# TalShor/SciLMM

Hardware: NVIDIA B200
Metric: reml_iter_time (lower is better)
Workload: dtype f64

## Files before the change

### include/scilmm_b200.h

```cpp
#ifndef SCILMM_B200_H
#define SCILMM_B200_H

#include <stdint.h>

#ifdef __cplusplus
extern "C" {
#endif

#define SLMM_OK 0
#define SLMM_ERR_INVALID 1
#define SLMM_ERR_CUDA 2
#define SLMM_ERR_NOT_POSDEF 3
#define SLMM_ERR_INTERNAL 4

#define SLMM_ORDER_NATURAL 0
#define SLMM_ORDER_GIVEN 1
#define SLMM_ORDER_METIS 2
#define SLMM_ORDER_MINDEG 3
#define SLMM_ORDER_METIS_FAST 4

typedef struct slmm_chol slmm_chol_t;
typedef struct slmm_matset slmm_matset_t;

const char* slmm_last_error(void);
int slmm_version(void);
int slmm_device_count(int* out);

int slmm_matset_create(int32_t n, int32_t K, slmm_matset_t** out);
int slmm_matset_destroy(slmm_matset_t* ms);
int slmm_matset_upload(slmm_matset_t* ms, int32_t k, const int32_t* h_indptr, const int32_t* h_indices,
                       const double* h_data);
int slmm_matset_bind_device(slmm_matset_t* ms, int32_t k, const int32_t* d_indptr, const int32_t* d_indices,
                            const double* d_data, int64_t nnz, int32_t same_as);
int slmm_matset_set_row_range(slmm_matset_t* ms, int32_t row_begin, int32_t row_end);
int slmm_matset_symmetry_hash(slmm_matset_t* ms, int32_t k, uint64_t* h_out2);
int slmm_matset_set_symmetric(slmm_matset_t* ms, int32_t k, int32_t flag);
int slmm_upload_h2d(void* d_dst, const void* h_src, int64_t nbytes, int32_t threads);
int slmm_upload_h2d_2d(void* d_dst, int64_t dst_pitch, const void* h_src, int64_t src_pitch, int64_t width_bytes,
                       int64_t rows);
int slmm_matset_nnz(const slmm_matset_t* ms, int32_t k, int64_t* out);
int slmm_matset_values(const slmm_matset_t* ms, int32_t k, const double** d_data_out);

int slmm_he_moments(slmm_matset_t* ms, const double* d_y, int32_t row_begin, int32_t row_end, double* d_out);
int slmm_he_moments_host(slmm_matset_t* ms, const double* h_y, double* h_out);

int slmm_spmm(slmm_matset_t* ms, int32_t k, const double* d_X, int32_t ncols, double* d_out);
int slmm_spmm_coldot(slmm_matset_t* ms, int32_t k, const double* d_X, int32_t ncols, int32_t row_begin,
                     int32_t row_end, double* d_out);

int slmm_spmm_coldot_multi(slmm_matset_t* ms, int32_t nk, const int32_t* ks, const double* d_X, int32_t ncols,
                           int32_t store_from, double* d_store, int32_t row_begin, int32_t row_end, double* d_dots);
int slmm_quadform_multi(slmm_matset_t* ms, int32_t nk, const int32_t* ks, const double* d_X, int32_t ncols,
                        int32_t row_begin, int32_t row_end, double* d_dots);
int slmm_quadform_gram_multi(slmm_matset_t* ms, int32_t nk, const int32_t* ks, const double* d_X, int32_t ncols,
                             const double* d_XB, int32_t nb, int32_t row_begin, int32_t row_end, double* d_dots,
                             double* d_gram_half);
int slmm_matset_validate(slmm_matset_t* ms, int32_t k, int32_t* flags_out);
int slmm_device_arrays_equal_i32(const int32_t* d_a, const int32_t* d_b, int64_t count, int32_t* out);
int slmm_matset_is_symmetric(slmm_matset_t* ms, int32_t k, int32_t* out);
int slmm_matset_pattern_id(const slmm_matset_t* ms, int32_t k, int32_t* out);

int slmm_matset_build_tiles(slmm_matset_t* ms, int32_t k, const int32_t* d_perm, const int32_t* d_iperm);
int slmm_matset_tile_stats(const slmm_matset_t* ms, int32_t k, int64_t* out4);
int slmm_matset_tile_cta_profile(const slmm_matset_t* ms, int32_t k, int64_t* out, int32_t ncta);
int slmm_quadform_tiled(slmm_matset_t* ms, int32_t nk, const int32_t* ks, const double* d_X, int32_t ncols, int32_t nb,
                        double* d_dots, double* d_gram_half);
int slmm_device_csr_is_symmetric(const int32_t* d_indptr, const int32_t* d_indices, const double* d_data, int32_t n,
                                 int32_t* out);
int slmm_device_pattern_subset(const int32_t* d_indptr_a, const int32_t* d_indices_a, const int32_t* d_indptr_b,
                               const int32_t* d_indices_b, int32_t n, int32_t* out);

int slmm_chol_analyze(int32_t n, const int32_t* h_indptr, const int32_t* h_indices, int32_t ordering,
                      const int32_t* h_user_perm, slmm_chol_t** out);
int slmm_chol_destroy(slmm_chol_t* h);
int slmm_chol_stats(const slmm_chol_t* h, int64_t* i_out, double* d_out);
int slmm_chol_perm(const slmm_chol_t* h, int32_t* h_perm);
int slmm_chol_device_perm(const slmm_chol_t* h, const int32_t** d_perm, const int32_t** d_iperm);

int slmm_chol_register_pattern(slmm_chol_t* h, const int32_t* h_indptr, const int32_t* h_indices, int32_t* map_id);
int slmm_chol_register_pattern_tri(slmm_chol_t* h, const int32_t* h_indptr, const int32_t* h_indices, int32_t tri,
                                   int32_t* map_id);
int slmm_chol_register_pattern_device(slmm_chol_t* h, const int32_t* d_indptr, const int32_t* d_indices, int64_t nnz,
                                      int32_t tri, int32_t* map_id);
int slmm_chol_add_values(slmm_chol_t* h, int32_t map_id, const double* d_values, double sigma, int32_t first);
int slmm_chol_add_values2(slmm_chol_t* h, int32_t map_id, const double* d_values0, double sigma0,
                          const double* d_values1, double sigma1, int32_t first);
int slmm_chol_factorize(slmm_chol_t* h, int32_t* fail_col);
int slmm_chol_logdet(slmm_chol_t* h, double* h_out);
int slmm_chol_solve(slmm_chol_t* h, double* d_B, int32_t nrhs, int32_t mode);
int slmm_chol_lmul(slmm_chol_t* h, const double* d_Z, double* d_out, int32_t nrhs);
int slmm_probe_normals(double* d_out, int64_t n, int32_t ncols, int32_t col_begin, uint64_t seed, uint64_t stream);
int slmm_chol_export_L(slmm_chol_t* h, int64_t* h_colptr, int32_t* h_rowidx, double* h_values);

int slmm_chol_aux_begin(slmm_chol_t* h);
int slmm_chol_aux_end(slmm_chol_t* h);
int slmm_chol_aux_join(slmm_chol_t* h);
int slmm_chol_copy_panels(slmm_chol_t* h, double* host_out);
int slmm_launch_count(int64_t* out, int32_t reset);
int slmm_chol_set_profiling(slmm_chol_t* h, int32_t on);
int slmm_chol_get_profile(const slmm_chol_t* h, double* ms6, double* flops6, int64_t* n6);
int slmm_chol_get_profile_ex(const slmm_chol_t* h, int32_t nkinds, double* ms, double* flops, int64_t* n);
int slmm_chol_set_timeline(slmm_chol_t* h, int32_t on);
int slmm_chol_get_timeline(slmm_chol_t* h, int32_t max_n, int32_t* n_out, float* ms, int32_t* stream);
int slmm_chol_get_launch_timeline(slmm_chol_t* h, int32_t max_n, int32_t* n_out, float* end_ms, int32_t* stream,
                                  int32_t* kind, int32_t* grid, double* flops);
int slmm_chol_get_launch_profile(const slmm_chol_t* h, int64_t max_n, int64_t* n_out, float* ms, double* flops,
                                 int32_t* kind, int32_t* grid);

typedef struct slmm_symbolic slmm_symbolic_t;
int slmm_symbolic_create(int32_t n, const int32_t* h_indptr, const int32_t* h_indices, int32_t ordering,
                         const int32_t* h_user_perm, slmm_symbolic_t** out);
int slmm_symbolic_destroy(slmm_symbolic_t* s);
int slmm_symbolic_stats(const slmm_symbolic_t* s, int64_t* i_out, double* d_out);
int slmm_symbolic_arrays(const slmm_symbolic_t* s, int32_t* perm, int32_t* parent, int32_t* colcount,
                         int32_t* sn_first, int32_t* sn_nrow, int32_t* sn_parent, int64_t* sn_rowptr,
                         int64_t* sn_lptr, int32_t* rows, int32_t* rel, int32_t* level_ptr, int32_t* level_sn);
int slmm_symbolic_entry_map(const slmm_symbolic_t* s, const int32_t* h_indptr, const int32_t* h_indices,
                            int64_t* h_target);
int slmm_symbolic_entry_map_tri(const slmm_symbolic_t* s, const int32_t* h_indptr, const int32_t* h_indices,
                                int32_t tri, int64_t* h_target);

typedef struct slmm_ibd slmm_ibd_t;
int slmm_ibd_build(int32_t n, const int32_t* h_rel_indptr, const int32_t* h_rel_indices, slmm_ibd_t** out);
int slmm_ibd_sizes(const slmm_ibd_t* h, int64_t* nnz_L, int64_t* nnz_A, int32_t* nlevels);
int slmm_ibd_copy_L(const slmm_ibd_t* h, int32_t* h_indptr, int32_t* h_indices, double* h_data);
int slmm_ibd_copy_DF(const slmm_ibd_t* h, double* h_D, double* h_F);
int slmm_ibd_copy_A(const slmm_ibd_t* h, int32_t* h_indptr, int32_t* h_indices, double* h_data);
int slmm_ibd_destroy(slmm_ibd_t* h);

int slmm_gemm_selftest(int32_t M, int32_t N, int32_t K, const double* d_A, const double* d_B, double* d_C,
                       int32_t lower, int32_t reps, float* ms_out);

int slmm_gemm_selftest_ex(int32_t M, int32_t N, int32_t K, const double* d_A, int64_t lda, const double* d_B, int64_t ldb,
                          double* d_C, int64_t ldc, int32_t flags, int32_t copies);

#ifdef __cplusplus
}
#endif
#endif
```

### scilmm_b200/_lib.py

```python
import ctypes as C
import os

_HERE = os.path.dirname(os.path.abspath(__file__))
LIB_PATH = os.path.join(_HERE, "libscilmm_b200.so")

i32, i64, f64 = C.c_int32, C.c_int64, C.c_double
vp = C.c_void_p
pp = C.POINTER(C.c_void_p)


class SlmmError(RuntimeError):
    def __init__(self, code, msg):
        RuntimeError.__init__(self, "scilmm_b200 error %d: %s" % (code, msg))
        self.code = code


class NotPositiveDefiniteError(SlmmError):

    def __init__(self, code, msg, column=-1):
        SlmmError.__init__(self, code, msg)
        self.column = column


SIGNATURES = {
    "slmm_last_error": (C.c_char_p, []),
    "slmm_version": (C.c_int, []),
    "slmm_device_count": (C.c_int, [C.POINTER(C.c_int)]),
    "slmm_matset_create": (C.c_int, [i32, i32, pp]),
    "slmm_matset_destroy": (C.c_int, [vp]),
    "slmm_matset_upload": (C.c_int, [vp, i32, vp, vp, vp]),
    "slmm_matset_bind_device": (C.c_int, [vp, i32, vp, vp, vp, i64, i32]),
    "slmm_matset_build_tiles": (C.c_int, [vp, i32, vp, vp]),
    "slmm_matset_tile_stats": (C.c_int, [vp, i32, vp]),
    "slmm_matset_tile_cta_profile": (C.c_int, [vp, i32, vp, i32]),
    "slmm_quadform_tiled": (C.c_int, [vp, i32, vp, vp, i32, i32, vp, vp]),
    "slmm_chol_device_perm": (C.c_int, [vp, pp, pp]),
    "slmm_matset_set_row_range": (C.c_int, [vp, i32, i32]),
    "slmm_matset_symmetry_hash": (C.c_int, [vp, i32, vp]),
    "slmm_matset_set_symmetric": (C.c_int, [vp, i32, i32]),
    "slmm_upload_h2d": (C.c_int, [vp, vp, i64, i32]),
    "slmm_upload_h2d_2d": (C.c_int, [vp, i64, vp, i64, i64, i64]),
    "slmm_matset_nnz": (C.c_int, [vp, i32, C.POINTER(i64)]),
    "slmm_matset_values": (C.c_int, [vp, i32, pp]),
    "slmm_he_moments": (C.c_int, [vp, vp, i32, i32, vp]),
    "slmm_he_moments_host": (C.c_int, [vp, vp, vp]),
    "slmm_spmm": (C.c_int, [vp, i32, vp, i32, vp]),
    "slmm_spmm_coldot": (C.c_int, [vp, i32, vp, i32, i32, i32, vp]),
    "slmm_spmm_coldot_multi": (C.c_int, [vp, i32, vp, vp, i32, i32, vp, i32, i32, vp]),
    "slmm_matset_pattern_id": (C.c_int, [vp, i32, C.POINTER(i32)]),
    "slmm_quadform_multi": (C.c_int, [vp, i32, vp, vp, i32, i32, i32, vp]),
    "slmm_matset_is_symmetric": (C.c_int, [vp, i32, C.POINTER(i32)]),
    "slmm_matset_validate": (C.c_int, [vp, i32, C.POINTER(i32)]),
    "slmm_device_arrays_equal_i32": (C.c_int, [vp, vp, i64, C.POINTER(i32)]),
    "slmm_quadform_gram_multi": (C.c_int, [vp, i32, vp, vp, i32, vp, i32, i32, i32, vp, vp]),
    "slmm_chol_analyze": (C.c_int, [i32, vp, vp, i32, vp, pp]),
    "slmm_chol_destroy": (C.c_int, [vp]),
    "slmm_chol_stats": (C.c_int, [vp, vp, vp]),
    "slmm_chol_perm": (C.c_int, [vp, vp]),
    "slmm_chol_register_pattern": (C.c_int, [vp, vp, vp, C.POINTER(i32)]),
    "slmm_chol_register_pattern_tri": (C.c_int, [vp, vp, vp, i32, C.POINTER(i32)]),
    "slmm_chol_register_pattern_device": (C.c_int, [vp, vp, vp, i64, i32, C.POINTER(i32)]),
    "slmm_device_csr_is_symmetric": (C.c_int, [vp, vp, vp, i32, C.POINTER(i32)]),
    "slmm_device_pattern_subset": (C.c_int, [vp, vp, vp, vp, i32, C.POINTER(i32)]),
    "slmm_symbolic_entry_map_tri": (C.c_int, [vp, vp, vp, i32, vp]),
    "slmm_chol_add_values": (C.c_int, [vp, i32, vp, f64, i32]),
    "slmm_chol_add_values2": (C.c_int, [vp, i32, vp, f64, vp, f64, i32]),
    "slmm_chol_factorize": (C.c_int, [vp, C.POINTER(i32)]),
    "slmm_chol_logdet": (C.c_int, [vp, C.POINTER(f64)]),
    "slmm_chol_solve": (C.c_int, [vp, vp, i32, i32]),
    "slmm_chol_lmul": (C.c_int, [vp, vp, vp, i32]),
    "slmm_probe_normals": (C.c_int, [vp, i64, i32, i32, C.c_uint64, C.c_uint64]),
    "slmm_chol_export_L": (C.c_int, [vp, vp, vp, vp]),
    "slmm_chol_copy_panels": (C.c_int, [vp, vp]),
    "slmm_chol_aux_begin": (C.c_int, [vp]),
    "slmm_chol_aux_end": (C.c_int, [vp]),
    "slmm_chol_aux_join": (C.c_int, [vp]),
    "slmm_launch_count": (C.c_int, [C.POINTER(i64), i32]),
    "slmm_chol_set_profiling": (C.c_int, [vp, i32]),
    "slmm_chol_set_timeline": (C.c_int, [vp, i32]),
    "slmm_chol_get_timeline": (C.c_int, [vp, i32, C.POINTER(i32), vp, vp]),
    "slmm_chol_get_profile_ex": (C.c_int, [vp, i32, vp, vp, vp]),
    "slmm_chol_get_launch_timeline": (C.c_int, [vp, i32, C.POINTER(i32), vp, vp, vp, vp, vp]),
    "slmm_chol_get_profile": (C.c_int, [vp, vp, vp, vp]),
    "slmm_chol_get_launch_profile": (C.c_int, [vp, i64, C.POINTER(i64), vp, vp, vp, vp]),
    "slmm_symbolic_create": (C.c_int, [i32, vp, vp, i32, vp, pp]),
    "slmm_symbolic_destroy": (C.c_int, [vp]),
    "slmm_symbolic_stats": (C.c_int, [vp, vp, vp]),
    "slmm_symbolic_arrays": (C.c_int, [vp] + [vp] * 12),
    "slmm_symbolic_entry_map": (C.c_int, [vp, vp, vp, vp]),
    "slmm_ibd_build": (C.c_int, [i32, vp, vp, pp]),
    "slmm_ibd_sizes": (C.c_int, [vp, C.POINTER(i64), C.POINTER(i64), C.POINTER(i32)]),
    "slmm_ibd_copy_L": (C.c_int, [vp, vp, vp, vp]),
    "slmm_ibd_copy_DF": (C.c_int, [vp, vp, vp]),
    "slmm_ibd_copy_A": (C.c_int, [vp, vp, vp, vp]),
    "slmm_ibd_destroy": (C.c_int, [vp]),
    "slmm_gemm_selftest_ex": (C.c_int, [i32, i32, i32, vp, i64, vp, i64, vp, i64, i32, i32]),
    "slmm_gemm_selftest": (C.c_int, [i32, i32, i32, vp, vp, vp, i32, i32, C.POINTER(C.c_float)]),
}

_lib = None


def lib():
    global _lib
    if _lib is None:
        if not os.path.exists(LIB_PATH):
            raise ImportError("%s is missing: run `python -c 'import __graft_entry__ as g; g.build()'` "
                              "(nvcc, sm_100a). There is no CPU fallback." % LIB_PATH)
        h = C.CDLL(LIB_PATH)
        for name, (res, args) in SIGNATURES.items():
            fn = getattr(h, name)
            fn.restype = res
            fn.argtypes = args
        _lib = h
    return _lib


def check(code, column=None):
    if code == 0:
        return
    msg = lib().slmm_last_error().decode("utf-8", "replace")
    if code == 3:
        raise NotPositiveDefiniteError(code, msg, -1 if column is None else column)
    raise SlmmError(code, msg)


def np_ptr(a):
    return a.ctypes.data_as(C.c_void_p)
```

### scilmm_b200/csrc/build.py

```python
import os
import subprocess
import sys

HERE = os.path.dirname(os.path.abspath(__file__))
PKG = os.path.dirname(HERE)
LIB = os.path.join(PKG, "libscilmm_b200.so")
CUDA_HOME = os.environ.get("CUDA_HOME", "/usr/local/cuda")
NVCC = os.path.join(CUDA_HOME, "bin", "nvcc")
METIS = os.path.join(CUDA_HOME, "lib64", "libmetis_static.a")
SOURCES_CU = ["chol.cu", "sparse_ops.cu", "ibd.cu", "quadform_tiled.cu"]
SOURCES_CPP = ["symbolic.cpp"]
HEADERS = ["common.h", "dense_tiles.cuh", "potrf_block.cuh", "symbolic.h", "skinny_ops.cuh", "matset.h", "dense_tiles_tma.cuh"]


def _stale():
    if not os.path.exists(LIB):
        return True
    t = os.path.getmtime(LIB)
    for f in SOURCES_CU + SOURCES_CPP + HEADERS + ["build.py"]:
        if os.path.getmtime(os.path.join(HERE, f)) > t:
            return True
    return False


def build(force=False, verbose=False):
    if not force and not _stale():
        return LIB
    if not os.path.exists(NVCC):
        raise RuntimeError("nvcc not found at %s" % NVCC)
    objs = []
    for src in SOURCES_CPP:
        obj = os.path.join(HERE, src.replace(".cpp", ".o"))
        cmd = ["g++", "-O2", "-fPIC", "-std=c++17", "-c", os.path.join(HERE, src), "-o", obj]
        subprocess.check_call(cmd)
        objs.append(obj)
    cmd = [NVCC, "-gencode", "arch=compute_100a,code=sm_100a", "-lineinfo", "-O3", "-std=c++17",
           "-Xcompiler", "-fPIC", "-shared"]
    if verbose:
        cmd += ["-Xptxas", "-v"]
    cmd += [os.path.join(HERE, s) for s in SOURCES_CU] + objs + [METIS, "-o", LIB]
    out = subprocess.run(cmd, stdout=subprocess.PIPE, stderr=subprocess.STDOUT, text=True)
    if verbose or out.returncode != 0:
        sys.stderr.write(out.stdout)
    if out.returncode != 0:
        raise RuntimeError("nvcc failed")
    return LIB


if __name__ == "__main__":
    print(build(force="--force" in sys.argv, verbose="-v" in sys.argv))
```

### scilmm_b200/csrc/chol.cu

```cuda
#include <algorithm>
#include <cmath>
#include <cstring>
#include <map>
#include <memory>
#include <vector>

#include "common.h"
#include "dense_tiles.cuh"
#include "dense_tiles_tma.cuh"
#include "potrf_block.cuh"
#include "skinny_ops.cuh"
#include "symbolic.h"

namespace slmm {

static thread_local std::string g_last_error;
void set_last_error(const std::string& msg) { g_last_error = msg; }
const std::string& last_error() { return g_last_error; }
int64_t g_launch_count = 0;

constexpr int NBO = 1024;

struct PullItem { int32_t p, c0, c1, e0, e1; };
struct PullEntry { int64_t rel_off, src_off; int32_t rsc, ta, tb, pad; };

struct DevSym {
  const int32_t *sn_first, *sn_nrow, *rows, *rel, *child_ptr, *child_idx;
  const int64_t *sn_rowptr, *sn_lptr, *sn_uptr;
};

__global__ void scatter_axpy_kernel(const int64_t* __restrict__ map, const double* __restrict__ vals, double sigma,
                                    double* __restrict__ Lx, int64_t nnz) {
  int64_t e = blockIdx.x * (int64_t)blockDim.x + threadIdx.x;
  const int64_t stride = (int64_t)gridDim.x * blockDim.x;
  for (; e < nnz; e += stride) {
    const int64_t tgt = map[e];
    if (tgt >= 0) Lx[tgt] = __dadd_rn(Lx[tgt], __dmul_rn(sigma, vals[e]));
  }
}

__global__ void scatter_axpy2_kernel(const int64_t* __restrict__ map, const double* __restrict__ v0, double s0,
                                     const double* __restrict__ v1, double s1, double* __restrict__ Lx, int64_t nnz) {
  int64_t e = blockIdx.x * (int64_t)blockDim.x + threadIdx.x;
  const int64_t stride = (int64_t)gridDim.x * blockDim.x;
  for (; e < nnz; e += stride) {
    const int64_t tgt = map[e];
    if (tgt >= 0) Lx[tgt] = __dadd_rn(__dadd_rn(Lx[tgt], __dmul_rn(s0, v0[e])), __dmul_rn(s1, v1[e]));
  }
}

__device__ __forceinline__ int lower_bound_dev(const int32_t* a, int n, int v) {
  int lo = 0, hi = n;
  while (lo < hi) { int mid = (lo + hi) >> 1; if (a[mid] < v) lo = mid + 1; else hi = mid; }
  return lo;
}

template <int TPI>
__global__ void __launch_bounds__(TPI < 128 ? 128 : TPI) extend_add_kernel(const PullItem* __restrict__ items, int nitems,
                                                                         const PullEntry* __restrict__ entries,
                                                                         DevSym S, double* __restrict__ Lx,
                                                                         const double* __restrict__ arena_child,
                                                                         double* __restrict__ arena_parent) {
  constexpr int GROUPS = (TPI < 128 ? 128 : TPI) / TPI;
  const int w = blockIdx.x * GROUPS + threadIdx.x / TPI, lane = threadIdx.x % TPI;
  if (w >= nitems) return;
  const PullItem it = items[w];
  const int p = it.p;
  const int nsp = S.sn_first[p + 1] - S.sn_first[p], msp = S.sn_nrow[p], rsp = msp - nsp;
  double* panel = Lx + S.sn_lptr[p];
  double* Up = arena_parent + S.sn_uptr[p];
  for (int q = it.e0; q < it.e1; q++) {
    const PullEntry en = entries[q];
    const int rsc = en.rsc;
    const int32_t* __restrict__ relc = S.rel + en.rel_off;
    const double* Uc = arena_child + en.src_off;
    for (int tt = en.ta; tt < en.tb; tt++) {
      const int pc = relc[tt];
      const double* __restrict__ src = Uc + (int64_t)tt * rsc;
      double* dst = pc < nsp ? panel + (int64_t)pc * ((msp + 1) & ~1) : Up + (int64_t)(pc - nsp) * rsp - nsp;
      int u = tt + lane;
      for (; u + 3 * TPI < rsc; u += 4 * TPI) {
        const int r0 = relc[u], r1 = relc[u + TPI], r2 = relc[u + 2 * TPI], r3 = relc[u + 3 * TPI];
        const double v0 = src[u], v1 = src[u + TPI], v2 = src[u + 2 * TPI], v3 = src[u + 3 * TPI];
        const double d0 = dst[r0], d1 = dst[r1], d2 = dst[r2], d3 = dst[r3];
        dst[r0] = d0 + v0; dst[r1] = d1 + v1; dst[r2] = d2 + v2; dst[r3] = d3 + v3;
      }
      for (; u < rsc; u += TPI) dst[relc[u]] += src[u];
    }
    if (TPI >= 128) __syncthreads(); else __syncwarp();
  }
}

__global__ void vec_pull_kernel(const PullItem* __restrict__ items, int nitems, const PullEntry* __restrict__ entries,
                                DevSym S, double* __restrict__ X, const double* __restrict__ arena_child,
                                double* __restrict__ arena_parent, const int64_t* __restrict__ vptr, int nrhs) {
  const int w = (blockIdx.x * blockDim.x + threadIdx.x) >> 5, lane = threadIdx.x & 31;
  if (w >= nitems) return;
  const PullItem it = items[w];
  const int p = it.p;
  const int fp = S.sn_first[p], nsp = S.sn_first[p + 1] - fp;
  double* Vp = arena_parent + vptr[p];
  for (int q = it.e0; q < it.e1; q++) {
    const PullEntry en = entries[q];
    const int32_t* relc = S.rel + en.rel_off;
    const double* Vc = arena_child + en.src_off;
    for (int tt = en.ta; tt < en.tb; tt++) {
      const int pr = relc[tt];
      const double* src = Vc + (int64_t)tt * nrhs;
      double* dst = pr < nsp ? X + (int64_t)(fp + pr) * nrhs : Vp + (int64_t)(pr - nsp) * nrhs;
      for (int j = lane; j < nrhs; j += 32) dst[j] += src[j];
    }
  }
}

__global__ void gather_rows_kernel(const double* __restrict__ src, double* __restrict__ dst,
                                   const int32_t* __restrict__ perm, int n, int nrhs, int scatter) {
  const int64_t total = (int64_t)n * nrhs;
  for (int64_t q = blockIdx.x * (int64_t)blockDim.x + threadIdx.x; q < total; q += (int64_t)gridDim.x * blockDim.x) {
    const int i = (int)(q / nrhs), j = (int)(q % nrhs);
    const int64_t o = (int64_t)perm[i] * nrhs + j;
    if (scatter) dst[o] = src[q]; else dst[q] = src[o];
  }
}

__global__ void __launch_bounds__(256) entry_map_kernel(const int32_t* __restrict__ ap, const int32_t* __restrict__ ai,
                                                        int n, const int32_t* __restrict__ iperm,
                                                        const int32_t* __restrict__ col2sn, DevSym S, int tri,
                                                        int64_t* __restrict__ target, int* __restrict__ bad) {
  const int lane = threadIdx.x & 31;
  const int warps = (gridDim.x * blockDim.x) >> 5;
  for (int r = (blockIdx.x * blockDim.x + threadIdx.x) >> 5; r < n; r += warps) {
    const int pr = iperm[r];
    const int b = ap[r], e = ap[r + 1];
    for (int p = b + lane; p < e; p += 32) {
      const int c = ai[p];
      const int pc = iperm[c];
      int ir = pr, ic = pc;
      int64_t out = -1;
      bool take = true;
      if (tri == 0) take = ic <= ir;
      else {
        take = !((tri > 0 && c < r) || (tri < 0 && c > r));
        if (ic > ir) { ir = pc; ic = pr; }
      }
      if (take) {
        const int s = col2sn[ic];
        const int ms = S.sn_nrow[s];
        const int32_t* rows = S.rows + S.sn_rowptr[s];
        const int pos = lower_bound_dev(rows, ms, ir);
        if (pos < ms && rows[pos] == ir) out = S.sn_lptr[s] + (int64_t)(ic - S.sn_first[s]) * ((ms + 1) & ~1) + pos;
        else *bad = 1;
      }
      target[p] = out;
    }
  }
}

__device__ __forceinline__ void philox4x32_10(uint32_t c0, uint32_t c1, uint32_t c2, uint32_t c3, uint32_t k0,
                                              uint32_t k1, uint32_t out[4]) {
#pragma unroll
  for (int r = 0; r < 10; r++) {
    const uint32_t hi0 = __umulhi(0xD2511F53u, c0), lo0 = 0xD2511F53u * c0;
    const uint32_t hi1 = __umulhi(0xCD9E8D57u, c2), lo1 = 0xCD9E8D57u * c2;
    const uint32_t n0 = hi1 ^ c1 ^ k0, n2 = hi0 ^ c3 ^ k1;
    c0 = n0; c1 = lo1; c2 = n2; c3 = lo0;
    k0 += 0x9E3779B9u; k1 += 0xBB67AE85u;
  }
  out[0] = c0; out[1] = c1; out[2] = c2; out[3] = c3;
}

__global__ void __launch_bounds__(256) probe_normals_kernel(double* __restrict__ out, int64_t n, int ncols, int col_begin,
                                                            uint64_t seed, uint64_t stream) {
  const int64_t total = n * ncols;
  for (int64_t q = blockIdx.x * (int64_t)blockDim.x + threadIdx.x; q < total; q += (int64_t)gridDim.x * blockDim.x) {
    const int64_t i = q / ncols;
    const int c = (int)(q - i * ncols) + col_begin;
    uint32_t x[4];
    philox4x32_10((uint32_t)i, (uint32_t)c, (uint32_t)stream, (uint32_t)(stream >> 32) ^ (uint32_t)(i >> 32),
                  (uint32_t)seed, (uint32_t)(seed >> 32), x);
    const uint64_t a = (((uint64_t)x[0] << 32) | x[1]) >> 11, b = (((uint64_t)x[2] << 32) | x[3]) >> 11;
    const double u1 = ((double)a + 0.5) * 0x1.0p-53, u2 = ((double)b + 0.5) * 0x1.0p-53;
    out[q] = sqrt(-2.0 * log(u1)) * cospi(2.0 * u2);
  }
}

struct WBlock { int64_t off; int32_t n, pad; };

__global__ void init_identity_kernel(const WBlock* __restrict__ blocks, double* __restrict__ W) {
  const WBlock b = blocks[blockIdx.x];
  double* w = W + b.off;
  const int64_t total = (int64_t)b.n * b.n;
  for (int64_t q = threadIdx.x; q < total; q += blockDim.x) w[q] = (q % b.n == q / b.n) ? 1.0 : 0.0;
}

__global__ void logdet_kernel(const double* __restrict__ Lx, const int32_t* __restrict__ col2sn,
                              const int32_t* __restrict__ sn_first, const int32_t* __restrict__ sn_nrow,
                              const int64_t* __restrict__ sn_lptr, int n, double* __restrict__ partial) {
  __shared__ double sh[256];
  double acc = 0.0;
  for (int j = blockIdx.x * blockDim.x + threadIdx.x; j < n; j += gridDim.x * blockDim.x) {
    const int s = col2sn[j], c = j - sn_first[s];
    acc += log(Lx[sn_lptr[s] + (int64_t)c * ((sn_nrow[s] + 1) & ~1) + c]);
  }
  sh[threadIdx.x] = acc;
  __syncthreads();
  for (int o = 128; o > 0; o >>= 1) {
    if (threadIdx.x < o) sh[threadIdx.x] += sh[threadIdx.x + o];
    __syncthreads();
  }
  if (threadIdx.x == 0) partial[blockIdx.x] = sh[0];
}

struct Launch {
  enum Kind { POTRF, GEMM_BIG, GEMM_SMALL, PULL_MAT, PULL_VEC, PULL_MAT_BIG, INIT_W, REDUCE, EV_RECORD, EV_WAIT,
              SKINNY_F1, SKINNY_F2 ,
              GEMM_TMA  } kind;
  int64_t off;
  int32_t count;
  int32_t grid;
  int32_t child_parity;
  double flops;
  int64_t tile_off;
  int32_t stream;
  int64_t aux_off = 0;
};

static CUtensorMap encode_tmap(const double* base, uint64_t rows, uint64_t cols, uint64_t ld) {
  typedef CUresult (*EncodeFn)(CUtensorMap*, CUtensorMapDataType, cuuint32_t, void*, const cuuint64_t*, const cuuint64_t*,
                               const cuuint32_t*, const cuuint32_t*, CUtensorMapInterleave, CUtensorMapSwizzle,
                               CUtensorMapL2promotion, CUtensorMapFloatOOBfill);
  static EncodeFn fn = nullptr;
  if (!fn) {
    void* p = nullptr;
    cudaDriverEntryPointQueryResult q;
    CUDA_OK(cudaGetDriverEntryPoint("cuTensorMapEncodeTiled", &p, cudaEnableDefault, &q));
    if (!p || q != cudaDriverEntryPointSuccess) throw std::runtime_error("cuTensorMapEncodeTiled is not available");
    fn = (EncodeFn)p;
  }
  CUtensorMap m;
  const cuuint64_t gdim[2] = {rows, cols};
  const cuuint64_t gstride[1] = {ld * sizeof(double)};
  const cuuint32_t box[2] = {16, (cuuint32_t)TMA_KS};
  const cuuint32_t estr[2] = {1, 1};
  const CUresult rc = fn(&m, CU_TENSOR_MAP_DATA_TYPE_FLOAT64, 2, (void*)base, gdim, gstride, box, estr, CU_TENSOR_MAP_INTERLEAVE_NONE,
                         CU_TENSOR_MAP_SWIZZLE_128B, CU_TENSOR_MAP_L2_PROMOTION_L2_128B, CU_TENSOR_MAP_FLOAT_OOB_FILL_NONE);
  if (rc != CUDA_SUCCESS) throw std::runtime_error("cuTensorMapEncodeTiled failed (" + std::to_string((int)rc) + ")");
  return m;
}

constexpr int BIG_STAGES = 4, SMALL_STAGES = 4;
constexpr int BIG_SMEM = BIG_STAGES * 16 * (128 + 4) * 2 * 8 + 2 * BIG_STAGES * 8;
constexpr int SMALL_SMEM = SMALL_STAGES * 16 * (64 + 4) * 2 * 8 + 2 * SMALL_STAGES * 8;
constexpr int BIG_THREADS = 32 * (2 * 4 + NPW), SMALL_THREADS = 32 * (2 * 2 + NPW);

struct Schedule {
  std::vector<Launch> launches;
  std::vector<GemmOp> gemm;
  std::vector<PotrfOp> potrf;
  std::vector<PullItem> pull;
  std::vector<PullEntry> pull_entries;
  PullEntry* d_pull_entries = nullptr;
  std::vector<ReduceOp> reduce;
  std::vector<CUtensorMap> tmaps;
  CUtensorMap* d_tmaps = nullptr;
  std::vector<int32_t> tile_op;
  int32_t* d_tile_op = nullptr;
  int nevents = 0;
  int64_t ws_size = 0;
  int64_t ws2_size = 0;
  double* d_ws = nullptr;
  double* d_ws2 = nullptr;
  ReduceOp* d_reduce = nullptr;
  GemmOp* d_gemm = nullptr;
  PotrfOp* d_potrf = nullptr;
  PullItem* d_pull = nullptr;
  double flops = 0;
  cudaGraphExec_t gexec[2] = {nullptr, nullptr};
  bool graph_failed = false;
  void upload() {
    if (ws_size > 0 || ws2_size > 0) {
      d_ws = dev_alloc<double>(ws_size);
      d_ws2 = dev_alloc<double>(ws2_size);
      for (GemmOp& op : gemm) {
        if (op.flags & GF_WS) { op.C = d_ws + (int64_t)(intptr_t)op.C; op.flags &= ~GF_WS; }
        if (op.flags & GF_WS2) { op.C = d_ws2 + (int64_t)(intptr_t)op.C; op.flags &= ~GF_WS2; }
      }
      for (ReduceOp& r : reduce) {
        r.ws = ((r.flags & GF_WS2) ? d_ws2 : d_ws) + (int64_t)(intptr_t)r.ws;
        r.flags &= ~GF_WS2;
      }
    }
    d_reduce = dev_upload(reduce.data(), reduce.size());
    d_gemm = dev_upload(gemm.data(), gemm.size());
    d_potrf = dev_upload(potrf.data(), potrf.size());
    d_pull = dev_upload(pull.data(), pull.size());
    d_tile_op = dev_upload(tile_op.data(), tile_op.size());
    d_tmaps = dev_upload(tmaps.data(), tmaps.size());
    d_pull_entries = dev_upload(pull_entries.data(), pull_entries.size());
  }
  void release() {
    for (int q = 0; q < 2; q++) if (gexec[q]) { cudaGraphExecDestroy(gexec[q]); gexec[q] = nullptr; }
    dev_free(d_gemm); dev_free(d_potrf); dev_free(d_pull); dev_free(d_ws); dev_free(d_ws2); dev_free(d_reduce); dev_free(d_tile_op); dev_free(d_pull_entries);
    d_ws2 = nullptr;
    dev_free(d_tmaps); d_tmaps = nullptr;
    d_tile_op = nullptr; d_pull_entries = nullptr;
    d_gemm = nullptr; d_potrf = nullptr; d_pull = nullptr; d_ws = nullptr; d_reduce = nullptr;
  }
  size_t device_bytes() const {
    return gemm.size() * sizeof(GemmOp) + potrf.size() * sizeof(PotrfOp) + pull.size() * sizeof(PullItem) +
           reduce.size() * sizeof(ReduceOp) + (size_t)(ws_size + ws2_size) * 8 + tile_op.size() * 4 + pull_entries.size() * sizeof(PullEntry);
  }
};

struct PhaseBuilder {
  std::vector<GemmOp> big, small, sk1, sk2;
  std::vector<GemmOp> tma;
  int skinny_mt = 0;
  int ws_id = 0;
  std::vector<PotrfOp> potrf;
  std::vector<ReduceOp> reduces;
  int64_t ws_used = 0;
  bool allow_split = true;
  static bool tma_ok(const GemmOp& op) {
    return op.a_si == 1 && op.b_sj == 1 && op.a_kidx == nullptr && !(op.flags & GF_TRIL_B) &&
           (op.a_sk % 2) == 0 && (op.b_sk % 2) == 0 && op.a_sk > 0 && op.b_sk > 0 && op.K >= 64;
  }
  void push(const GemmOp& op, bool small_tiles) {
    const bool tma_splits_inplace = op.C == op.A && op.N + (int)(((uintptr_t)op.B >> 3) & 1) > 128;
    if (small_tiles) small.push_back(op);
    else if (tma_ok(op) && !tma_splits_inplace) tma.push_back(op);
    else big.push_back(op);
  }
  template <typename Push>
  void split_k(const GemmOp& op, int S, int kc, Push push) {
    const int64_t mn = (int64_t)op.M * op.N;
    ReduceOp r;
    memset(&r, 0, sizeof(r));
    r.C = op.C; r.c_si = op.c_si; r.c_sj = op.c_sj; r.M = op.M; r.N = op.N; r.S = S;
    r.flags = (op.flags & (GF_ACCUM | GF_NEG)) | (ws_id ? GF_WS2 : 0);
    r.ws = (const double*)(intptr_t)ws_used;
    reduces.push_back(r);
    for (int c = 0; c < S; c++) {
      GemmOp part = op;
      const int k0 = c * kc;
      part.K = std::min(kc, op.K - k0);
      if (op.a_kidx) part.a_kidx = op.a_kidx + k0; else part.A = op.A + (int64_t)k0 * op.a_sk;
      part.B = op.B + (int64_t)k0 * op.b_sk;
      part.C = (double*)(intptr_t)(ws_used + (int64_t)c * mn);
      part.c_si = 1; part.c_sj = op.M;
      part.flags = (ws_id ? GF_WS2 : GF_WS) | (op.flags & GF_TRIL_B);
      part.pad = k0;
      push(part);
    }
    ws_used += (int64_t)S * mn;
  }
  bool add_skinny(const GemmOp& op) {
    if (skinny_mt <= 0 || op.M > skinny_mt || op.a_si != 1 || op.c_si != 1 || (op.flags & (GF_LOWER | GF_BIGTILE))) return false;
    const bool f1 = op.b_sj == 1 && op.a_kidx == nullptr;
    if (!f1 && op.b_sk != 1) return false;
    if (!f1 && (op.flags & GF_TRIL_B)) return false;
    std::vector<GemmOp>& dst = f1 ? sk1 : sk2;
    const int cols = f1 ? SK_F1_COLS : SK_F2_COLS, kmin = 64;
    const int64_t nj = (op.N + cols - 1) / cols;
    int S = 1;
    const int64_t target = f1 ? 148 * 8 : 148 * 4;
    const bool can_split = allow_split && op.C != op.A;
    if (can_split && nj < target) S = (int)std::min<int64_t>((target + nj - 1) / nj, std::max(1, op.K / kmin));
    if (!f1 && skinny_mt < 8) S = std::max(S, (op.K + SK_F2_KMAX - 1) / SK_F2_KMAX);
    if (S > 1 && !can_split) return false;
    int kc = op.K;
    if (S > 1) {
      kc = (((op.K + S - 1) / S) + 15) / 16 * 16;
      if (!f1 && skinny_mt < 8) kc = std::min(kc, SK_F2_KMAX);
      S = (op.K + kc - 1) / kc;
    }
    if (S <= 1) { GemmOp o = op; o.pad = 0; dst.push_back(o); }
    else split_k(op, S, kc, [&](const GemmOp& part) { dst.push_back(part); });
    return true;
  }
  void add(GemmOp op) {
    if (op.M <= 0 || op.N <= 0 || op.K <= 0) return;
    if (add_skinny(op)) return;
    const bool lower = op.flags & GF_LOWER;
    const int64_t tb = (int64_t)((op.M + 127) / 128) * ((op.N + 127) / 128);
    const int64_t ts = (int64_t)((op.M + 63) / 64) * ((op.N + 63) / 64);
    const bool force_big = op.flags & GF_BIGTILE;
    op.flags &= ~GF_BIGTILE;
    const bool small_tiles = !force_big && (!(op.M > 64 && op.N > 64) || (!lower && tb < 40 && op.K >= 128) ||
                                            (lower && tb <= 64));
    const int64_t tiles = small_tiles ? ts : tb;
    if (allow_split && !lower && (op.flags & GF_TRIL_B) && op.K >= 4096 && op.C != op.A && !small_tiles) {
      const int kc = 2048;
      const int S = (op.K + kc - 1) / kc;
      split_k(op, S, kc, [&](GemmOp part) { part.flags = (ws_id ? GF_WS2 : GF_WS) | GF_TRIL_B; push(part, false); });
      return;
    }
    if (allow_split && !lower && !(op.flags & GF_TRIL_B) && tiles <= 148 && op.K >= 256 && op.C != op.A) {
      int S = (int)std::min<int64_t>(std::min<int64_t>(64, op.K / 64), std::max<int64_t>(1, 148 / tiles));
      const int kc = S > 0 ? (((op.K + S - 1) / S) + 15) / 16 * 16 : op.K;
      S = (op.K + kc - 1) / kc;
      if (S >= 2) {
        op.flags &= ~GF_TRIL_B;
        split_k(op, S, kc, [&](GemmOp part) { part.pad = 0; part.flags = ws_id ? GF_WS2 : GF_WS; push(part, small_tiles); });
        return;
      }
    }
    push(op, small_tiles);
  }
  void flush(Schedule& sch, int stream = 0) {
    const size_t first_launch = sch.launches.size();
    if (!potrf.empty()) {
      double pf = 0;
      for (const PotrfOp& o : potrf) pf += 2.0 * o.nb * o.nb * o.nb / 3.0;
      sch.launches.push_back({Launch::POTRF, (int64_t)sch.potrf.size(), (int32_t)potrf.size(), (int32_t)potrf.size(), 0, pf});
      sch.potrf.insert(sch.potrf.end(), potrf.begin(), potrf.end());
    }
    for (int pass = 0; pass < 3; pass++) {
      std::vector<GemmOp>& v = pass == 0 ? tma : pass == 1 ? big : small;
      if (v.empty()) continue;
      const int T = pass == 2 ? 64 : 128;
      int64_t tiles = 0;
      double lf = 0;
      for (GemmOp& op : v) {
        int em = 0, en = 0;
        if (pass == 0) {
          em = (int)(((uintptr_t)op.A >> 3) & 1);
          en = (int)(((uintptr_t)op.B >> 3) & 1);
          op.pad = em | (en << 1);
        }
        op.tiles_m = (op.M + em + T - 1) / T;
        op.tiles_n = (op.N + en + T - 1) / T;
        op.tile_start = (int32_t)tiles;
        tiles += (int64_t)op.tiles_m * op.tiles_n;
        double f = 2.0 * op.M * op.N * op.K;
        if (op.flags & GF_TRIL_B) f = (double)op.M * op.N * op.K;
        if (op.flags & GF_LOWER) {
          const double nn = std::min(op.M, op.N);
          f = 2.0 * op.K * ((double)op.M * op.N - nn * (nn - 1) / 2.0);
        }
        sch.flops += f;
        lf += f;
      }
      if (tiles > 2000000000LL) throw std::runtime_error("too many tiles in one phase");
      const int64_t tile_off = (int64_t)sch.tile_op.size();
      sch.tile_op.resize(tile_off + tiles);
      for (size_t q = 0; q < v.size(); q++)
        std::fill(sch.tile_op.begin() + tile_off + v[q].tile_start,
                  sch.tile_op.begin() + tile_off + v[q].tile_start + (int64_t)v[q].tiles_m * v[q].tiles_n, (int32_t)q);
      if (pass == 0) {
        for (GemmOp& op : v) {
          const int sa = op.pad & 1, sb = (op.pad >> 1) & 1;
          sch.tmaps.push_back(encode_tmap(op.A - sa, (uint64_t)op.M + sa, (uint64_t)op.K, (uint64_t)op.a_sk));
          sch.tmaps.push_back(encode_tmap(op.B - sb, (uint64_t)op.N + sb, (uint64_t)op.K, (uint64_t)op.b_sk));
        }
      }
      Launch L{pass == 0 ? Launch::GEMM_TMA : pass == 1 ? Launch::GEMM_BIG : Launch::GEMM_SMALL, (int64_t)sch.gemm.size(),
               (int32_t)v.size(), (int32_t)tiles, 0, lf, tile_off};
      if (pass == 0) L.aux_off = (int64_t)sch.tmaps.size() - 2 * (int64_t)v.size();
      sch.launches.push_back(L);
      sch.gemm.insert(sch.gemm.end(), v.begin(), v.end());
    }
    for (int pass = 0; pass < 2; pass++) {
      std::vector<GemmOp>& v = pass == 0 ? sk1 : sk2;
      if (v.empty()) continue;
      const int T = pass == 0 ? SK_F1_COLS : SK_F2_COLS;
      int64_t tiles = 0;
      double lf = 0;
      for (GemmOp& op : v) {
        op.tiles_m = 1;
        op.tiles_n = (op.N + T - 1) / T;
        op.tile_start = (int32_t)tiles;
        tiles += op.tiles_n;
        const double f = (op.flags & GF_TRIL_B) ? (double)op.M * op.N * op.K : 2.0 * op.M * op.N * op.K;
        sch.flops += f;
        lf += f;
      }
      if (tiles > 2000000000LL) throw std::runtime_error("too many tiles in one phase");
      const int64_t tile_off = (int64_t)sch.tile_op.size();
      sch.tile_op.resize(tile_off + tiles);
      for (size_t q = 0; q < v.size(); q++)
        std::fill(sch.tile_op.begin() + tile_off + v[q].tile_start,
                  sch.tile_op.begin() + tile_off + v[q].tile_start + v[q].tiles_n, (int32_t)q);
      sch.launches.push_back({pass == 0 ? Launch::SKINNY_F1 : Launch::SKINNY_F2, (int64_t)sch.gemm.size(),
                              (int32_t)v.size(), (int32_t)tiles, skinny_mt, lf, tile_off});
      sch.gemm.insert(sch.gemm.end(), v.begin(), v.end());
    }
    if (!reduces.empty()) {
      int64_t blocks = 0;
      for (ReduceOp& r : reduces) {
        r.block_start = (int32_t)blocks;
        blocks += ((int64_t)r.M * r.N + 255) / 256;
      }
      sch.launches.push_back({Launch::REDUCE, (int64_t)sch.reduce.size(), (int32_t)reduces.size(), (int32_t)blocks, 0, 0.0});
      sch.reduce.insert(sch.reduce.end(), reduces.begin(), reduces.end());
      if (ws_id) sch.ws2_size = std::max(sch.ws2_size, ws_used); else sch.ws_size = std::max(sch.ws_size, ws_used);
    }
    for (size_t q = first_launch; q < sch.launches.size(); q++) sch.launches[q].stream = stream;
    big.clear(); small.clear(); tma.clear(); sk1.clear(); sk2.clear(); potrf.clear(); reduces.clear();
    ws_used = 0;
  }
  bool empty() const { return big.empty() && small.empty() && tma.empty() && sk1.empty() && sk2.empty() && potrf.empty(); }
};

static GemmOp make_op(double* C, int64_t c_si, int64_t c_sj, const double* A, int64_t a_si, int64_t a_sk,
                      const double* B, int64_t b_sj, int64_t b_sk, int M, int N, int K, int flags,
                      const int32_t* kidx = nullptr) {
  GemmOp op;
  memset(&op, 0, sizeof(op));
  op.C = C; op.A = A; op.B = B; op.a_kidx = kidx;
  op.c_si = c_si; op.c_sj = c_sj; op.a_si = a_si; op.a_sk = a_sk; op.b_sj = b_sj; op.b_sk = b_sk;
  op.M = M; op.N = N; op.K = K; op.flags = flags;
  return op;
}

struct SolvePlan {
  int nrhs = 0;
  double *X = nullptr, *X2 = nullptr;
  double* arena[2] = {nullptr, nullptr};
  int64_t* d_vptr = nullptr;
  Schedule fwd, bwd, lmul;
  size_t bytes = 0;
  void release() {
    dev_free(X); dev_free(X2); dev_free(arena[0]); dev_free(arena[1]); dev_free(d_vptr);
    fwd.release(); bwd.release(); lmul.release();
  }
};

struct EntryMap { int64_t* d_map = nullptr; int64_t nnz = 0; };

}

using namespace slmm;

struct slmm_chol {
  Symbolic S;
  int32_t *d_sn_first = nullptr, *d_sn_nrow = nullptr, *d_rows = nullptr, *d_rel = nullptr, *d_child_ptr = nullptr,
          *d_child_idx = nullptr, *d_col2sn = nullptr, *d_perm = nullptr, *d_iperm = nullptr;
  int64_t *d_sn_rowptr = nullptr, *d_sn_lptr = nullptr, *d_sn_uptr = nullptr;
  std::vector<int64_t> uptr, invptr;
  std::vector<int64_t> wptr;
  std::vector<WBlock> wblocks;
  WBlock* d_wblocks = nullptr;
  double* Lx = nullptr;
  double* inv = nullptr;
  double* W = nullptr;
  double* wscratch = nullptr;
  std::vector<int64_t> wscratch_off;
  double* arena[2] = {nullptr, nullptr};
  int64_t arena_size[2] = {0, 0};
  int* d_info = nullptr;
  double* d_partial = nullptr;
  Schedule fact;
  std::vector<EntryMap> maps;
  std::map<int, std::unique_ptr<SolvePlan>> plans;
  cudaStream_t s_main = nullptr, s_bulk = nullptr;
  cudaStream_t s_aux = nullptr;
  cudaStream_t cur = nullptr;
  cudaEvent_t ev_aux = nullptr;
  cudaEvent_t ev_fork = nullptr, ev_join = nullptr;
  std::vector<cudaEvent_t> events;
  bool factored = false;
  bool profiling = false;
  bool timeline = false;
  std::vector<cudaEvent_t> tl_events;
  std::vector<cudaEvent_t> tl_launch;
  int tl_count = 0;
  double prof_ms[16] = {};
  double prof_flops[16] = {};
  int64_t prof_n[16] = {};
  std::vector<float> prof_launch_ms;
  std::vector<double> prof_launch_flops;
  std::vector<int32_t> prof_launch_kind, prof_launch_grid;
  size_t bytes = 0;
  int64_t exported_nnz = 0;

  DevSym devsym() const {
    return DevSym{d_sn_first, d_sn_nrow, d_rows, d_rel, d_child_ptr, d_child_idx, d_sn_rowptr, d_sn_lptr, d_sn_uptr};
  }
};

namespace slmm {

static void init_kernel_attributes() {
  static bool done = false;
  if (done) return;
  CUDA_OK(cudaFuncSetAttribute(gemm_tiles_kernel<128, 128, 2, 4, BIG_STAGES>, cudaFuncAttributeMaxDynamicSharedMemorySize, BIG_SMEM));
  CUDA_OK(cudaFuncSetAttribute(gemm_tiles_kernel<64, 64, 2, 2, SMALL_STAGES>, cudaFuncAttributeMaxDynamicSharedMemorySize, SMALL_SMEM));
  CUDA_OK(cudaFuncSetAttribute(potrf_inv_kernel_v4, cudaFuncAttributeMaxDynamicSharedMemorySize, POTRF4_SMEM));
  CUDA_OK(cudaFuncSetAttribute(gemm_tiles_tma_kernel, cudaFuncAttributeMaxDynamicSharedMemorySize, TMA_SMEM));
#define SKD_ATTR(NMT)                                                                                                         \
  CUDA_OK(cudaFuncSetAttribute(skinny_f2_dmma_kernel<NMT>, cudaFuncAttributeMaxDynamicSharedMemorySize, SkDmma<NMT>::SMEM));   \
  CUDA_OK(cudaFuncSetAttribute(skinny_f1_dmma_kernel<NMT>, cudaFuncAttributeMaxDynamicSharedMemorySize, SkDmma<NMT>::F1_SMEM));
  SKD_ATTR(1) SKD_ATTR(2) SKD_ATTR(4)
#undef SKD_ATTR
  done = true;
}

static void launch_one(slmm_chol* h, const Schedule& sch, const Launch& L, const DevSym& ds, double* X,
                       double* const* vec_arena, const int64_t* d_vptr, int nrhs, cudaStream_t st) {
  switch (L.kind) {
    case Launch::POTRF:
      potrf_inv_kernel_v4<<<L.grid, 256, POTRF4_SMEM, st>>>(sch.d_potrf + L.off, h->d_info);
      break;
    case Launch::GEMM_BIG:
      gemm_tiles_kernel<128, 128, 2, 4, BIG_STAGES><<<L.grid, BIG_THREADS, BIG_SMEM, st>>>(sch.d_gemm + L.off, sch.d_tile_op + L.tile_off);
      break;
    case Launch::GEMM_TMA:
      gemm_tiles_tma_kernel<<<L.grid, TMA_THREADS, TMA_SMEM, st>>>(sch.d_gemm + L.off, sch.d_tile_op + L.tile_off, sch.d_tmaps + L.aux_off);
      break;
    case Launch::GEMM_SMALL:
      gemm_tiles_kernel<64, 64, 2, 2, SMALL_STAGES><<<L.grid, SMALL_THREADS, SMALL_SMEM, st>>>(sch.d_gemm + L.off, sch.d_tile_op + L.tile_off);
      break;
    case Launch::PULL_MAT:
      extend_add_kernel<32><<<(L.count + 3) / 4, 128, 0, st>>>(sch.d_pull + L.off, L.count, sch.d_pull_entries, ds, h->Lx,
                                                               h->arena[L.child_parity], h->arena[L.child_parity ^ 1]);
      break;
    case Launch::PULL_MAT_BIG:
      extend_add_kernel<256><<<L.count, 256, 0, st>>>(sch.d_pull + L.off, L.count, sch.d_pull_entries, ds, h->Lx,
                                                      h->arena[L.child_parity], h->arena[L.child_parity ^ 1]);
      break;
    case Launch::PULL_VEC:
      vec_pull_kernel<<<(L.count + 3) / 4, 128, 0, st>>>(sch.d_pull + L.off, L.count, sch.d_pull_entries, ds, X,
                                                         vec_arena[L.child_parity], vec_arena[L.child_parity ^ 1], d_vptr, nrhs);
      break;
    case Launch::REDUCE:
      splitk_reduce_kernel<<<L.grid, 256, 0, st>>>(sch.d_reduce + L.off, L.count);
      break;
    case Launch::SKINNY_F1:
    case Launch::SKINNY_F2: {
      const GemmOp* ops = sch.d_gemm + L.off;
      const int32_t* top = sch.d_tile_op + L.tile_off;
      const bool f1 = L.kind == Launch::SKINNY_F1;
#define SKD_CASE(NMT)                                                                          \
  if (f1) skinny_f1_dmma_kernel<NMT><<<L.grid, 256, SkDmma<NMT>::F1_SMEM, st>>>(ops, top);  \
  else skinny_f2_dmma_kernel<NMT><<<L.grid, 256, SkDmma<NMT>::SMEM, st>>>(ops, top);
#define SK_CASE(MT)                                                                        \
  if (f1) skinny_f1_kernel<MT><<<L.grid, SK_F1_COLS, 0, st>>>(ops, top);                   \
  else skinny_f2_kernel<MT><<<L.grid, 256, SK_F2_KMAX * MT * sizeof(double), st>>>(ops, top);
      switch (L.child_parity) {
        case 1: SK_CASE(1) break;
        case 2: SK_CASE(2) break;
        case 4: SK_CASE(4) break;
        case 8: SKD_CASE(1) break;
        case 16: SKD_CASE(2) break;
        default: SKD_CASE(4) break;
      }
#undef SK_CASE
#undef SKD_CASE
      break;
    }
    case Launch::INIT_W:
      init_identity_kernel<<<L.count, 256, 0, st>>>(h->d_wblocks, h->W);
      break;
    default:
      break;
  }
}

static bool is_kernel(const Launch& L) { return L.kind != Launch::EV_RECORD && L.kind != Launch::EV_WAIT; }

static void issue_schedule(slmm_chol* h, const Schedule& sch, double* X, double* const* vec_arena,
                           const int64_t* d_vptr, int nrhs, bool two, cudaStream_t one,
                           std::vector<cudaEvent_t>* per_launch = nullptr) {
  const DevSym ds = h->devsym();
  size_t nk = 0;
  for (const Launch& L : sch.launches) {
    cudaStream_t st = two ? (L.stream ? h->s_bulk : h->s_main) : one;
    if (L.kind == Launch::EV_RECORD) { if (two) CUDA_OK(cudaEventRecord(h->events[L.count], st)); continue; }
    if (L.kind == Launch::EV_WAIT) { if (two) CUDA_OK(cudaStreamWaitEvent(st, h->events[L.count], 0)); continue; }
    launch_one(h, sch, L, ds, X, vec_arena, d_vptr, nrhs, st);
    if (per_launch) {
      if (nk >= per_launch->size()) { cudaEvent_t e; CUDA_OK(cudaEventCreate(&e)); per_launch->push_back(e); }
      CUDA_OK(cudaEventRecord((*per_launch)[nk], st));
    }
    nk++;
  }
}

static cudaGraphExec_t capture_schedule(slmm_chol* h, const Schedule& sch, double* X, double* const* vec_arena,
                                        const int64_t* d_vptr, int nrhs, bool two) {
  cudaStream_t origin = h->s_main;
  cudaGraph_t graph = nullptr;
  cudaGraphExec_t exec = nullptr;
  CUDA_OK(cudaStreamBeginCapture(origin, cudaStreamCaptureModeRelaxed));
  try {
    if (two) {
      CUDA_OK(cudaEventRecord(h->ev_fork, origin));
      CUDA_OK(cudaStreamWaitEvent(h->s_bulk, h->ev_fork, 0));
    }
    issue_schedule(h, sch, X, vec_arena, d_vptr, nrhs, two, origin);
    if (two) {
      CUDA_OK(cudaEventRecord(h->ev_join, h->s_bulk));
      CUDA_OK(cudaStreamWaitEvent(origin, h->ev_join, 0));
    }
    CUDA_OK(cudaGetLastError());
  } catch (...) {
    cudaStreamEndCapture(origin, &graph);
    if (graph) cudaGraphDestroy(graph);
    cudaGetLastError();
    throw;
  }
  CUDA_OK(cudaStreamEndCapture(origin, &graph));
  const cudaError_t e = cudaGraphInstantiate(&exec, graph, 0);
  cudaGraphDestroy(graph);
  CUDA_OK(e);
  return exec;
}

static void run_schedule(slmm_chol* h, Schedule& sch, double* X, double* const* vec_arena, const int64_t* d_vptr,
                         int nrhs) {
  int64_t nk = 0;
  for (const Launch& L : sch.launches) nk += is_kernel(L) ? 1 : 0;
  if (nk == 0) return;
  if (!h->profiling) {
    const bool two = sch.nevents > 0 && h->s_main != nullptr && h->cur == nullptr;
    while ((int)h->events.size() < sch.nevents) {
      cudaEvent_t e;
      CUDA_OK(cudaEventCreateWithFlags(&e, cudaEventDisableTiming));
      h->events.push_back(e);
    }
    const int gi = two ? 0 : 1;
    if (h->timeline && two) {
      while ((int)h->tl_events.size() < sch.nevents + 2) {
        cudaEvent_t e;
        CUDA_OK(cudaEventCreate(&e));
        h->tl_events.push_back(e);
      }
      std::vector<cudaEvent_t> saved = h->events;
      for (int q = 0; q < sch.nevents; q++) h->events[q] = h->tl_events[q + 2];
      CUDA_OK(cudaEventRecord(h->tl_events[0], 0));
      CUDA_OK(cudaStreamWaitEvent(h->s_main, h->tl_events[0], 0));
      CUDA_OK(cudaStreamWaitEvent(h->s_bulk, h->tl_events[0], 0));
      issue_schedule(h, sch, X, vec_arena, d_vptr, nrhs, true, nullptr, &h->tl_launch);
      CUDA_OK(cudaEventRecord(h->ev_join, h->s_bulk));
      CUDA_OK(cudaStreamWaitEvent(h->s_main, h->ev_join, 0));
      CUDA_OK(cudaEventRecord(h->tl_events[1], h->s_main));
      CUDA_OK(cudaStreamWaitEvent(0, h->tl_events[1], 0));
      CUDA_OK(cudaEventSynchronize(h->tl_events[1]));
      h->events = saved;
      h->tl_count = sch.nevents + 2;
      g_launch_count += nk;
      return;
    }
    const bool use_graph = !two && h->s_main != nullptr && !sch.graph_failed;
    if (use_graph && sch.gexec[gi] == nullptr) {
      try {
        sch.gexec[gi] = capture_schedule(h, sch, X, vec_arena, d_vptr, nrhs, two);
      } catch (const std::exception&) {
        sch.graph_failed = true;
        sch.gexec[gi] = nullptr;
      }
    }
    cudaGraphExec_t exec = (use_graph && !sch.graph_failed) ? sch.gexec[gi] : nullptr;
    if (exec != nullptr && h->cur != nullptr) {
      CUDA_OK(cudaGraphLaunch(exec, h->cur));
    } else if (exec != nullptr || two) {
      CUDA_OK(cudaEventRecord(h->ev_fork, 0));
      CUDA_OK(cudaStreamWaitEvent(h->s_main, h->ev_fork, 0));
      if (exec != nullptr) {
        CUDA_OK(cudaGraphLaunch(exec, h->s_main));
      } else {
        CUDA_OK(cudaStreamWaitEvent(h->s_bulk, h->ev_fork, 0));
        issue_schedule(h, sch, X, vec_arena, d_vptr, nrhs, true, nullptr);
        CUDA_OK(cudaEventRecord(h->ev_join, h->s_bulk));
        CUDA_OK(cudaStreamWaitEvent(h->s_main, h->ev_join, 0));
      }
      CUDA_OK(cudaEventRecord(h->ev_join, h->s_main));
      CUDA_OK(cudaStreamWaitEvent(0, h->ev_join, 0));
    } else {
      issue_schedule(h, sch, X, vec_arena, d_vptr, nrhs, false, h->cur);
    }
  } else {
    const DevSym ds = h->devsym();
    cudaStream_t st = h->cur;
    std::vector<const Launch*> ks;
    for (const Launch& L : sch.launches) if (is_kernel(L)) ks.push_back(&L);
    const size_t nl = ks.size();
    std::vector<cudaEvent_t> ev(nl + 1);
    for (auto& e : ev) CUDA_OK(cudaEventCreate(&e));
    CUDA_OK(cudaEventRecord(ev[0], st));
    for (size_t i = 0; i < nl; i++) {
      launch_one(h, sch, *ks[i], ds, X, vec_arena, d_vptr, nrhs, st);
      CUDA_OK(cudaEventRecord(ev[i + 1], st));
    }
    CUDA_OK(cudaEventSynchronize(ev[nl]));
    for (size_t i = 0; i < nl; i++) {
      float ms = 0;
      CUDA_OK(cudaEventElapsedTime(&ms, ev[i], ev[i + 1]));
      const int k = (int)ks[i]->kind;
      h->prof_ms[k] += ms;
      h->prof_flops[k] += ks[i]->flops;
      h->prof_n[k] += 1;
      h->prof_launch_ms.push_back(ms);
      h->prof_launch_flops.push_back(ks[i]->flops);
      h->prof_launch_kind.push_back(k);
      h->prof_launch_grid.push_back((ks[i]->kind <= Launch::GEMM_SMALL || ks[i]->kind >= Launch::SKINNY_F1) ? ks[i]->grid : ks[i]->count);
    }
    for (auto& e : ev) cudaEventDestroy(e);
  }
  g_launch_count += nk;
  CUDA_OK(cudaGetLastError());
}

static void add_pull_items(Schedule& sch, const Symbolic& S, const std::vector<int64_t>& src_ptr, int level,
                           int lo_kind, Launch::Kind kind, int chunk, int min_rows = 0, int max_rows = 1 << 30) {
  const int64_t off = (int64_t)sch.pull.size();
  std::vector<std::vector<PullEntry>> per_item;
  for (int q = S.level_ptr[level]; q < S.level_ptr[level + 1]; q++) {
    const int p = S.level_sn[q];
    if (S.child_ptr[p + 1] == S.child_ptr[p]) continue;
    const int ns = S.sn_first[p + 1] - S.sn_first[p], ms = S.sn_nrow[p];
    if (ms < min_rows || ms >= max_rows) continue;
    const int a = lo_kind == 1 ? ns : 0, b = lo_kind == 0 ? ns : ms;
    std::vector<int> starts;
    for (int c0 = a; c0 < b;) {
      int c1 = std::min(b, c0 + chunk);
      if (c0 < ns && c1 > ns) c1 = ns;
      starts.push_back(c0);
      c0 = c1;
    }
    if (starts.empty()) continue;
    starts.push_back(b);
    const int nit = (int)starts.size() - 1;
    per_item.assign(nit, std::vector<PullEntry>());
    for (int cq = S.child_ptr[p]; cq < S.child_ptr[p + 1]; cq++) {
      const int c = S.child_idx[cq];
      const int nsc = S.sn_first[c + 1] - S.sn_first[c], rsc = S.sn_nrow[c] - nsc;
      if (rsc == 0) continue;
      const int64_t rel_off = S.sn_rowptr[c] + nsc;
      const int32_t* relc = S.rel.data() + rel_off;
      int t = (int)(std::lower_bound(relc, relc + rsc, a) - relc);
      int item = 0;
      while (t < rsc && relc[t] < b) {
        while (starts[item + 1] <= relc[t]) item++;
        int tb = t;
        while (tb < rsc && relc[tb] < starts[item + 1]) tb++;
        per_item[item].push_back({rel_off, src_ptr[c], rsc, t, tb, 0});
        t = tb;
      }
    }
    for (int i = 0; i < nit; i++) {
      if (per_item[i].empty()) continue;
      const int32_t e0 = (int32_t)sch.pull_entries.size();
      sch.pull_entries.insert(sch.pull_entries.end(), per_item[i].begin(), per_item[i].end());
      sch.pull.push_back({p, starts[i], starts[i + 1], e0, (int32_t)sch.pull_entries.size()});
    }
  }
  const int cnt = (int)(sch.pull.size() - off);
  if (cnt > 0) sch.launches.push_back({kind, off, cnt, 0, (level + 1) & 1, 0.0});
}

struct OuterBlock { int o0, nbo, ldw; double* winv; };
static int num_outer(int ns) { return (ns + NBO - 1) / NBO; }
static OuterBlock outer_block(const slmm_chol* h, int s, int ob) {
  const Symbolic& S = h->S;
  const int ns = S.sn_first[s + 1] - S.sn_first[s];
  OuterBlock b;
  b.o0 = ob * NBO;
  b.nbo = std::min(ns, b.o0 + NBO) - b.o0;
  if (b.nbo <= NBI) {
    b.winv = h->inv + h->invptr[s] + (int64_t)(b.o0 / NBI) * NBI * NBI;
    b.ldw = NBI;
  } else {
    int64_t off = h->wptr[s];
    for (int q = 0; q < ob; q++) off += (int64_t)NBO * NBO;
    b.winv = h->W + off;
    b.ldw = b.nbo;
  }
  return b;
}

struct FStep {
  enum Kind { POTRF, TRSM, UPD, WINV1, WINV2, CPANEL, OUTER, SCHUR } kind;
  int a, b;
};

static void build_factor_schedule(slmm_chol* h) {
  const Symbolic& S = h->S;
  Schedule& sch = h->fact;
  PhaseBuilder pb, pb_rest, pb_unrest;
  pb_rest.allow_split = pb_unrest.allow_split = false;
  int last_bulk_ev = -1, unrest_ev = -1;
  std::vector<std::vector<FStep>> prog;
  for (int d = S.nlevels - 1; d >= 0; d--) {
    add_pull_items(sch, S, h->uptr, d, 0, Launch::PULL_MAT, 8, 0, 512);
    add_pull_items(sch, S, h->uptr, d, 0, Launch::PULL_MAT_BIG, 4, 512);
    const int nl = S.level_ptr[d + 1] - S.level_ptr[d];
    prog.assign(nl, std::vector<FStep>());
    size_t max_steps = 0;
    for (int q = 0; q < nl; q++) {
      const int s = S.level_sn[S.level_ptr[d] + q];
      const int ns = S.sn_first[s + 1] - S.sn_first[s], ms = S.sn_nrow[s], rs = ms - ns;
      std::vector<FStep>& pr = prog[q];
      if (ns <= NBO) {
        const int nib = (ns + NBI - 1) / NBI;
        for (int ib = 0; ib < nib; ib++) {
          pr.push_back({FStep::POTRF, ib, 0});
          pr.push_back({FStep::TRSM, ib, 0});
          if (ib + 1 < nib) pr.push_back({FStep::UPD, ib, 0});
        }
        if (rs > 0) pr.push_back({FStep::SCHUR, 0, 0});
      } else {
        for (int ob = 0; ob < num_outer(ns); ob++) {
          const int o0 = ob * NBO, o1 = std::min(ns, o0 + NBO), w = o1 - o0;
          for (int c0 = o0; c0 < o1; c0 += NBI) {
            const int ib = c0 / NBI;
            pr.push_back({FStep::POTRF, ib, 0});
            if (std::min(o1, c0 + NBI) < o1) { pr.push_back({FStep::TRSM, ib, 0}); pr.push_back({FStep::UPD, ib, 0}); }
          }
          for (int m = NBI; m < w; m *= 2) { pr.push_back({FStep::WINV1, ob, m}); pr.push_back({FStep::WINV2, ob, m}); }
          if (ms > o1)
            for (int j = (w + 127) / 128 - 1; j >= 0; j--) pr.push_back({FStep::CPANEL, ob, j});
          if (o1 < ns) pr.push_back({FStep::OUTER, ob, 0});
          else if (rs > 0) pr.push_back({FStep::SCHUR, 0, 0});
        }
      }
      max_steps = std::max(max_steps, pr.size());
    }
    for (size_t ph = 0; ph < max_steps; ph++) {
      bool outer_done = false, needs_below = false;
      for (int q = 0; q < nl; q++) {
        if (ph >= prog[q].size()) continue;
        const FStep st = prog[q][ph];
        if (st.kind == FStep::CPANEL || st.kind == FStep::SCHUR) needs_below = true;
        const int s = S.level_sn[S.level_ptr[d] + q];
        const int f = S.sn_first[s], ns = S.sn_first[s + 1] - f, ms = S.sn_nrow[s], rs = ms - ns;
        const bool wide = ns > NBO;
        double* P = h->Lx + S.sn_lptr[s];
        const int64_t ld = panel_ld(ms);
        if (st.kind == FStep::POTRF || st.kind == FStep::TRSM || st.kind == FStep::UPD) {
          const int ib = st.a, c0 = ib * NBI, c1 = std::min(ns, c0 + NBI), nb = c1 - c0;
          const int ob = c0 / NBO, ob0 = ob * NBO, ob_end = std::min(ns, ob0 + NBO);
          double* inv = h->inv + h->invptr[s] + (int64_t)ib * NBI * NBI;
          int64_t inv_ld = NBI;
          if (wide) {
            const OuterBlock wb = outer_block(h, s, ob);
            if (wb.nbo > NBI) { inv = wb.winv + (c0 - ob0) + (int64_t)(c0 - ob0) * wb.ldw; inv_ld = wb.ldw; }
          }
          const int row_end = wide ? ob_end : ms;
          if (st.kind == FStep::POTRF) {
            pb.potrf.push_back({P + c0 + c0 * ld, inv, (int32_t)ld, nb, f + c0, (int32_t)inv_ld});
            sch.flops += (double)nb * nb * nb / 3.0;
          } else if (st.kind == FStep::TRSM) {
            pb.add(make_op(P + c1 + c0 * ld, 1, ld, P + c1 + c0 * ld, 1, ld, inv, 1, inv_ld, row_end - c1, nb, nb, 0));
          } else {
            pb.add(make_op(P + c1 + c1 * ld, 1, ld, P + c1 + c0 * ld, 1, ld, P + c1 + c0 * ld, 1, ld, row_end - c1,
                           ob_end - c1, nb, GF_LOWER | GF_ACCUM | GF_NEG));
          }
        } else if (st.kind == FStep::WINV1 || st.kind == FStep::WINV2) {
          const OuterBlock wb = outer_block(h, s, st.a);
          const int m = st.b, o0 = wb.o0;
          double* T = h->wscratch + h->wscratch_off[s];
          int pair = 0;
          for (int lo = 0; lo + m < wb.nbo; lo += 2 * m, pair++) {
            const int m2 = std::min(m, wb.nbo - lo - m);
            double* Tp = T + (int64_t)pair * m * m;
            double* Ainv = wb.winv + lo + (int64_t)lo * wb.ldw;
            double* Binv = wb.winv + (lo + m) + (int64_t)(lo + m) * wb.ldw;
            double* X21 = wb.winv + (lo + m) + (int64_t)lo * wb.ldw;
            if (st.kind == FStep::WINV1)
              pb.add(make_op(Tp, 1, m2, P + (o0 + lo + m) + (int64_t)(o0 + lo) * ld, 1, ld, Ainv, wb.ldw, 1, m2, m, m, 0));
            else
              pb.add(make_op(X21, 1, wb.ldw, Binv, 1, wb.ldw, Tp, m2, 1, m2, m, m2, GF_NEG));
          }
        } else if (st.kind == FStep::CPANEL) {
          const OuterBlock wb = outer_block(h, s, st.a);
          const int o0 = wb.o0, o1 = o0 + wb.nbo, j0 = 128 * st.b, nj = std::min(128, wb.nbo - j0);
          const int K = std::min(wb.nbo, j0 + 128);
          pb.add(make_op(P + o1 + (int64_t)(o0 + j0) * ld, 1, ld, P + o1 + (int64_t)o0 * ld, 1, ld, wb.winv + j0, 1, wb.ldw,
                         ms - o1, nj, K, GF_BIGTILE));
        } else if (st.kind == FStep::OUTER) {
          const int ob0 = st.a * NBO, c1 = std::min(ns, ob0 + NBO);
          outer_done = true;
          const int nx = std::min(ns, c1 + NBO);
          const bool split = (ns - nx) >= NBO;
          const int ncols = split ? nx - c1 : ns - c1;
          const int below = ms - c1 - ncols;
          pb.add(make_op(P + c1 + c1 * ld, 1, ld, P + c1 + ob0 * ld, 1, ld, P + c1 + ob0 * ld, 1, ld, ncols,
                         ncols, c1 - ob0, GF_LOWER | GF_ACCUM | GF_NEG));
          if (below > 0)
            pb_unrest.add(make_op(P + (c1 + ncols) + c1 * ld, 1, ld, P + (c1 + ncols) + ob0 * ld, 1, ld, P + c1 + ob0 * ld, 1, ld,
                                  below, ncols, c1 - ob0, GF_ACCUM | GF_NEG));
          if (split)
            pb_rest.add(make_op(P + nx + nx * ld, 1, ld, P + nx + ob0 * ld, 1, ld, P + nx + ob0 * ld, 1, ld, ms - nx,
                                ns - nx, c1 - ob0, GF_LOWER | GF_ACCUM | GF_NEG));
        } else {
          double* U = h->arena[d & 1] + h->uptr[s];
          pb.add(make_op(U, 1, rs, P + ns, 1, ld, P + ns, 1, ld, rs, rs, ns, GF_LOWER | GF_NEG));
        }
      }
      const bool side = !pb_rest.empty() || !pb_unrest.empty();
      int ev_panel = -1;
      if (side) {
        ev_panel = sch.nevents++;
        sch.launches.push_back({Launch::EV_RECORD, 0, ev_panel, 0, 0, 0.0, 0, 0});
      }
      if (outer_done && last_bulk_ev >= 0) {
        sch.launches.push_back({Launch::EV_WAIT, 0, last_bulk_ev, 0, 0, 0.0, 0, 0});
        last_bulk_ev = -1;
      }
      if (needs_below && unrest_ev >= 0) {
        sch.launches.push_back({Launch::EV_WAIT, 0, unrest_ev, 0, 0, 0.0, 0, 0});
        unrest_ev = -1;
      }
      pb.flush(sch, 0);
      if (side) {
        sch.launches.push_back({Launch::EV_WAIT, 0, ev_panel, 0, 0, 0.0, 0, 1});
        if (!pb_unrest.empty()) {
          pb_unrest.flush(sch, 1);
          unrest_ev = sch.nevents++;
          sch.launches.push_back({Launch::EV_RECORD, 0, unrest_ev, 0, 0, 0.0, 0, 1});
          last_bulk_ev = unrest_ev;
        }
        if (!pb_rest.empty()) {
          pb_rest.flush(sch, 1);
          last_bulk_ev = sch.nevents++;
          sch.launches.push_back({Launch::EV_RECORD, 0, last_bulk_ev, 0, 0, 0.0, 0, 1});
        }
      }
    }
    if (last_bulk_ev >= 0) sch.launches.push_back({Launch::EV_WAIT, 0, last_bulk_ev, 0, 0, 0.0, 0, 0});
    last_bulk_ev = unrest_ev = -1;
    add_pull_items(sch, S, h->uptr, d, 1, Launch::PULL_MAT, 8, 0, 512);
    add_pull_items(sch, S, h->uptr, d, 1, Launch::PULL_MAT_BIG, 4, 512);
  }
  if (!h->wblocks.empty()) {
    sch.launches.push_back({Launch::INIT_W, 0, (int32_t)h->wblocks.size(), (int32_t)h->wblocks.size(), 0, 0.0});
    for (int t = 0; t < NBO / NBI; t++) {
      for (int half = 0; half < 2; half++) {
        for (int s2 = 0; s2 < S.nsuper; s2++) {
          const int ns = S.sn_first[s2 + 1] - S.sn_first[s2];
          if (ns <= NBI || ns > NBO) continue;
          double* P = h->Lx + S.sn_lptr[s2];
          const int64_t ldp = panel_ld(S.sn_nrow[s2]);
          for (int ob = 0; ob < num_outer(ns); ob++) {
            const OuterBlock b = outer_block(h, s2, ob);
            if (b.nbo <= NBI || t * NBI >= b.nbo) continue;
            const int r0 = t * NBI, nbt = std::min(NBI, b.nbo - r0), ncols = std::min(b.nbo, r0 + NBI);
            double* inv64 = h->inv + h->invptr[s2] + (int64_t)((b.o0 + r0) / NBI) * NBI * NBI;
            if (half == 0) {
              pb.add(make_op(b.winv + r0, 1, b.ldw, inv64, 1, NBI, b.winv + r0, b.ldw, 1, nbt, ncols, nbt, 0));
            } else if (r0 + nbt < b.nbo) {
              pb.add(make_op(b.winv + r0 + nbt, 1, b.ldw, P + (b.o0 + r0 + nbt) + (int64_t)(b.o0 + r0) * ldp, 1, ldp,
                             b.winv + r0, b.ldw, 1, b.nbo - r0 - nbt, ncols, nbt, GF_ACCUM | GF_NEG));
            }
          }
        }
        pb.flush(sch);
      }
    }
  }
  sch.upload();
}

static SolvePlan* get_plan(slmm_chol* h, int nrhs) {
  const int key = nrhs * 2 + (h->cur != nullptr ? 1 : 0);
  auto it = h->plans.find(key);
  if (it != h->plans.end()) return it->second.get();
  if (h->plans.size() >= 6) {
    CUDA_OK(cudaDeviceSynchronize());
    for (auto& kv : h->plans) kv.second->release();
    h->plans.clear();
  }
  const Symbolic& S = h->S;
  std::unique_ptr<SolvePlan> pl(new SolvePlan());
  pl->nrhs = nrhs;
  const int n = S.n;
  pl->X = dev_alloc<double>((size_t)n * nrhs);
  pl->X2 = dev_alloc<double>((size_t)n * nrhs);
  std::vector<int64_t> vptr(S.nsuper, 0);
  int64_t asz[2] = {0, 0};
  for (int d = 0; d < S.nlevels; d++) {
    int64_t off = 0;
    for (int q = S.level_ptr[d]; q < S.level_ptr[d + 1]; q++) {
      const int s = S.level_sn[q];
      vptr[s] = off;
      off += (int64_t)(S.sn_nrow[s] - (S.sn_first[s + 1] - S.sn_first[s])) * nrhs;
    }
    asz[d & 1] = std::max(asz[d & 1], off);
  }
  pl->arena[0] = dev_alloc<double>(asz[0]);
  pl->arena[1] = dev_alloc<double>(asz[1]);
  pl->d_vptr = dev_upload(vptr.data(), vptr.size());
  pl->bytes = ((size_t)2 * n * nrhs + asz[0] + asz[1]) * 8;
  const int64_t R = nrhs;
  PhaseBuilder pb, pb_rest;
  pb_rest.ws_id = 1;
  if (nrhs <= 32) pb.skinny_mt = nrhs <= 1 ? 1 : nrhs <= 2 ? 2 : nrhs <= 4 ? 4 : nrhs <= 8 ? 8 : nrhs <= 16 ? 16 : 32;
  const bool lookahead = nrhs >= 64;
  int last_bulk_ev = -1;
  auto flush_pair = [&](Schedule& sch, bool updated) {
    int ev_diag = -1;
    if (!pb_rest.empty()) {
      ev_diag = sch.nevents++;
      sch.launches.push_back({Launch::EV_RECORD, 0, ev_diag, 0, 0, 0.0, 0, 0});
    }
    if (updated && last_bulk_ev >= 0) {
      sch.launches.push_back({Launch::EV_WAIT, 0, last_bulk_ev, 0, 0, 0.0, 0, 0});
      last_bulk_ev = -1;
    }
    pb.flush(sch, 0);
    if (ev_diag >= 0) {
      sch.launches.push_back({Launch::EV_WAIT, 0, ev_diag, 0, 0, 0.0, 0, 1});
      pb_rest.flush(sch, 1);
      last_bulk_ev = sch.nevents++;
      sch.launches.push_back({Launch::EV_RECORD, 0, last_bulk_ev, 0, 0, 0.0, 0, 1});
    }
  };
  for (int d = S.nlevels - 1; d >= 0; d--) {
    add_pull_items(pl->fwd, S, vptr, d, 0, Launch::PULL_VEC, 4);
    int max_nob = 0;
    for (int q = S.level_ptr[d]; q < S.level_ptr[d + 1]; q++) {
      const int s = S.level_sn[q];
      max_nob = std::max(max_nob, num_outer(S.sn_first[s + 1] - S.sn_first[s]));
    }
    for (int ph = 0; ph < 2 * max_nob + 1; ph++) {
      bool updated = false;
      for (int q = S.level_ptr[d]; q < S.level_ptr[d + 1]; q++) {
        const int s = S.level_sn[q];
        const int f = S.sn_first[s], ns = S.sn_first[s + 1] - f, ms = S.sn_nrow[s], rs = ms - ns;
        const int nob = num_outer(ns);
        double* P = h->Lx + S.sn_lptr[s];
        const int64_t ld = panel_ld(ms);
        double* Xs = pl->X + (int64_t)f * R;
        double* Ys = pl->X2 + (int64_t)f * R;
        if (ph == 2 * nob) {
          if (rs > 0)
            pb.add(make_op(pl->arena[d & 1] + vptr[s], 1, R, Ys, 1, R, P + ns, 1, ld, nrhs, rs, ns, GF_NEG));
          continue;
        }
        if (ph > 2 * nob) continue;
        const OuterBlock b = outer_block(h, s, ph / 2);
        const int o1 = b.o0 + b.nbo;
        if (ph % 2 == 0) {
          pb.add(make_op(Ys + (int64_t)b.o0 * R, 1, R, Xs + (int64_t)b.o0 * R, 1, R, b.winv, 1, b.ldw, nrhs, b.nbo,
                         b.nbo, 0));
        } else if (o1 < ns) {
          updated = true;
          const int nx = std::min(ns, o1 + NBO);
          const bool split = lookahead && (ns - nx) >= NBO;
          pb.add(make_op(Xs + (int64_t)o1 * R, 1, R, Ys + (int64_t)b.o0 * R, 1, R, P + o1 + (int64_t)b.o0 * ld, 1, ld,
                         nrhs, (split ? nx : ns) - o1, b.nbo, GF_ACCUM | GF_NEG));
          if (split)
            pb_rest.add(make_op(Xs + (int64_t)nx * R, 1, R, Ys + (int64_t)b.o0 * R, 1, R, P + nx + (int64_t)b.o0 * ld, 1, ld,
                                nrhs, ns - nx, b.nbo, GF_ACCUM | GF_NEG));
        }
      }
      flush_pair(pl->fwd, updated);
    }
    if (last_bulk_ev >= 0) { pl->fwd.launches.push_back({Launch::EV_WAIT, 0, last_bulk_ev, 0, 0, 0.0, 0, 0}); last_bulk_ev = -1; }
    add_pull_items(pl->fwd, S, vptr, d, 1, Launch::PULL_VEC, 4);
  }
  for (int d = 0; d < S.nlevels; d++) {
    int max_nob = 0;
    for (int q = S.level_ptr[d]; q < S.level_ptr[d + 1]; q++) {
      const int s = S.level_sn[q];
      max_nob = std::max(max_nob, num_outer(S.sn_first[s + 1] - S.sn_first[s]));
    }
    for (int ph = 0; ph < 2 * max_nob + 1; ph++) {
      bool updated = false;
      for (int q = S.level_ptr[d]; q < S.level_ptr[d + 1]; q++) {
        const int s = S.level_sn[q];
        const int f = S.sn_first[s], ns = S.sn_first[s + 1] - f, ms = S.sn_nrow[s], rs = ms - ns;
        const int nob = num_outer(ns);
        double* P = h->Lx + S.sn_lptr[s];
        const int64_t ld = panel_ld(ms);
        double* Xs = pl->X + (int64_t)f * R;
        double* Ys = pl->X2 + (int64_t)f * R;
        if (ph == 0) {
          if (rs > 0)
            pb.add(make_op(Ys, 1, R, pl->X, 1, R, P + ns, ld, 1, nrhs, ns, rs, GF_ACCUM | GF_NEG,
                           h->d_rows + S.sn_rowptr[s] + ns));
          continue;
        }
        const int step = ph - 1, r = step / 2;
        if (r >= nob) continue;
        const OuterBlock b = outer_block(h, s, nob - 1 - r);
        if (step % 2 == 0) {
          pb.add(make_op(Xs + (int64_t)b.o0 * R, 1, R, Ys + (int64_t)b.o0 * R, 1, R, b.winv, b.ldw, 1, nrhs, b.nbo,
                         b.nbo, 0));
        } else if (b.o0 > 0) {
          updated = true;
          const int p0 = b.o0 - NBO;
          const bool split = lookahead && p0 >= NBO;
          const int lo = split ? p0 : 0;
          pb.add(make_op(Ys + (int64_t)lo * R, 1, R, Xs + (int64_t)b.o0 * R, 1, R, P + b.o0 + (int64_t)lo * ld, ld, 1, nrhs,
                         b.o0 - lo, b.nbo, GF_ACCUM | GF_NEG));
          if (split)
            pb_rest.add(make_op(Ys, 1, R, Xs + (int64_t)b.o0 * R, 1, R, P + b.o0, ld, 1, nrhs, p0, b.nbo,
                                GF_ACCUM | GF_NEG));
        }
      }
      flush_pair(pl->bwd, updated);
    }
    if (last_bulk_ev >= 0) { pl->bwd.launches.push_back({Launch::EV_WAIT, 0, last_bulk_ev, 0, 0, 0.0, 0, 0}); last_bulk_ev = -1; }
  }
  for (int d = S.nlevels - 1; d >= 0; d--) {
    for (int q = S.level_ptr[d]; q < S.level_ptr[d + 1]; q++) {
      const int s = S.level_sn[q];
      const int f = S.sn_first[s], ns = S.sn_first[s + 1] - f, ms = S.sn_nrow[s], rs = ms - ns;
      double* P = h->Lx + S.sn_lptr[s];
      const int64_t ld = panel_ld(ms);
      pb.add(make_op(pl->X2 + (int64_t)f * R, 1, R, pl->X + (int64_t)f * R, 1, R, P, 1, ld, nrhs, ns, ns, GF_TRIL_B));
      if (rs > 0)
        pb.add(make_op(pl->arena[d & 1] + vptr[s], 1, R, pl->X + (int64_t)f * R, 1, R, P + ns, 1, ld, nrhs, rs, ns, 0));
    }
    pb.flush(pl->lmul);
    add_pull_items(pl->lmul, S, vptr, d, 2, Launch::PULL_VEC, 4);
  }
  pl->fwd.upload();
  pl->bwd.upload();
  pl->lmul.upload();
  pl->bytes += pl->fwd.device_bytes() + pl->bwd.device_bytes() + pl->lmul.device_bytes();
  SolvePlan* raw = pl.get();
  h->plans[key] = std::move(pl);
  return raw;
}

}

template <typename T>
static void copy_out(T* dst, const std::vector<T>& v) { if (dst && !v.empty()) memcpy(dst, v.data(), v.size() * sizeof(T)); }

extern "C" {

const char* slmm_last_error(void) { return slmm::last_error().c_str(); }
int slmm_version(void) { return 100; }
int slmm_device_count(int* out) {
  int c = 0;
  cudaError_t e = cudaGetDeviceCount(&c);
  if (e != cudaSuccess) { c = 0; cudaGetLastError(); }
  *out = c;
  return SLMM_OK;
}

int slmm_chol_analyze(int32_t n, const int32_t* indptr, const int32_t* indices, int32_t ordering,
                      const int32_t* user_perm, slmm_chol_t** out) {
  SLMM_TRY
  if (n <= 0 || !indptr || !indices || !out) throw std::invalid_argument("slmm_chol_analyze: bad arguments");
  std::unique_ptr<slmm_chol> h(new slmm_chol());
  SymbolicOptions opt;
  opt.ordering = ordering;
  analyze(n, indptr, indices, user_perm, opt, h->S);
  const Symbolic& S = h->S;
  init_kernel_attributes();
  h->uptr.assign(S.nsuper, 0);
  h->invptr.assign(S.nsuper + 1, 0);
  for (int d = 0; d < S.nlevels; d++) {
    int64_t off = 0;
    for (int q = S.level_ptr[d]; q < S.level_ptr[d + 1]; q++) {
      const int s = S.level_sn[q];
      const int64_t rs = S.sn_nrow[s] - (S.sn_first[s + 1] - S.sn_first[s]);
      h->uptr[s] = off;
      off += rs * rs;
    }
    h->arena_size[d & 1] = std::max(h->arena_size[d & 1], off);
  }
  h->exported_nnz = 0;
  h->wptr.assign(S.nsuper + 1, 0);
  h->wscratch_off.assign(S.nsuper, 0);
  int64_t wscratch_total = 0;
  for (int s = 0; s < S.nsuper; s++) {
    const int64_t ns = S.sn_first[s + 1] - S.sn_first[s], ms = S.sn_nrow[s];
    h->invptr[s + 1] = h->invptr[s] + ((ns + NBI - 1) / NBI) * NBI * NBI;
    h->exported_nnz += ns * ms - ns * (ns - 1) / 2;
    int64_t w = 0;
    for (int ob = 0; ob < num_outer((int)ns); ob++) {
      const int nbo = (int)std::min<int64_t>(ns, (int64_t)(ob + 1) * NBO) - ob * NBO;
      if (nbo > NBI) {
        if (ns <= NBO) h->wblocks.push_back({h->wptr[s] + w, nbo, 0});
        w += ((int64_t)nbo * nbo + 1) & ~(int64_t)1;
      }
    }
    h->wptr[s + 1] = h->wptr[s] + w;
    h->wscratch_off[s] = wscratch_total;
    if (ns > NBO) wscratch_total += (int64_t)(NBO / 2) * (NBO / 2);
  }
  h->d_sn_first = dev_upload(S.sn_first.data(), S.sn_first.size());
  h->d_sn_nrow = dev_upload(S.sn_nrow.data(), S.sn_nrow.size());
  h->d_rows = dev_upload(S.rows.data(), S.rows.size());
  h->d_rel = dev_upload(S.rel.data(), S.rel.size());
  h->d_child_ptr = dev_upload(S.child_ptr.data(), S.child_ptr.size());
  h->d_child_idx = dev_upload(S.child_idx.data(), S.child_idx.size());
  h->d_col2sn = dev_upload(S.col2sn.data(), S.col2sn.size());
  h->d_perm = dev_upload(S.perm.data(), S.perm.size());
  h->d_iperm = dev_upload(S.iperm.data(), S.iperm.size());
  h->d_sn_rowptr = dev_upload(S.sn_rowptr.data(), S.sn_rowptr.size());
  h->d_sn_lptr = dev_upload(S.sn_lptr.data(), S.sn_lptr.size());
  h->d_sn_uptr = dev_upload(h->uptr.data(), h->uptr.size());
  h->Lx = dev_alloc<double>(S.lsize);
  h->inv = dev_alloc<double>(h->invptr[S.nsuper]);
  h->W = dev_alloc<double>(h->wptr[S.nsuper]);
  CUDA_OK(cudaMemset(h->W, 0, std::max<int64_t>(1, h->wptr[S.nsuper]) * sizeof(double)));
  h->wscratch = dev_alloc<double>(wscratch_total);
  h->d_wblocks = dev_upload(h->wblocks.data(), h->wblocks.size());
  h->arena[0] = dev_alloc<double>(h->arena_size[0]);
  h->arena[1] = dev_alloc<double>(h->arena_size[1]);
  h->d_info = dev_alloc<int>(1);
  h->d_partial = dev_alloc<double>(1024);
  {
    int least = 0, greatest = 0;
    CUDA_OK(cudaDeviceGetStreamPriorityRange(&least, &greatest));
    CUDA_OK(cudaStreamCreateWithPriority(&h->s_main, cudaStreamNonBlocking, greatest));
    CUDA_OK(cudaStreamCreateWithPriority(&h->s_bulk, cudaStreamNonBlocking, least));
    CUDA_OK(cudaStreamCreateWithPriority(&h->s_aux, cudaStreamNonBlocking, least));
    CUDA_OK(cudaEventCreateWithFlags(&h->ev_aux, cudaEventDisableTiming));
    CUDA_OK(cudaEventCreateWithFlags(&h->ev_fork, cudaEventDisableTiming));
    CUDA_OK(cudaEventCreateWithFlags(&h->ev_join, cudaEventDisableTiming));
  }
  CUDA_OK(cudaMemset(h->Lx, 0, S.lsize * sizeof(double)));
  build_factor_schedule(h.get());
  h->bytes = (S.lsize + h->invptr[S.nsuper] + h->wptr[S.nsuper] + h->arena_size[0] + h->arena_size[1]) * 8 +
             (S.rows.size() * 2 + S.sn_first.size() * 8) * 4 + h->fact.device_bytes();
  CUDA_OK(cudaDeviceSynchronize());
  *out = h.release();
  return SLMM_OK;
  SLMM_CATCH
}

int slmm_chol_destroy(slmm_chol_t* h) {
  if (!h) return SLMM_OK;
  dev_free(h->d_sn_first); dev_free(h->d_sn_nrow); dev_free(h->d_rows); dev_free(h->d_rel);
  dev_free(h->d_child_ptr); dev_free(h->d_child_idx); dev_free(h->d_col2sn); dev_free(h->d_perm); dev_free(h->d_iperm);
  dev_free(h->d_sn_rowptr); dev_free(h->d_sn_lptr); dev_free(h->d_sn_uptr);
  dev_free(h->Lx); dev_free(h->inv); dev_free(h->W); dev_free(h->wscratch); dev_free(h->d_wblocks); dev_free(h->arena[0]); dev_free(h->arena[1]);
  dev_free(h->d_info); dev_free(h->d_partial);
  for (cudaEvent_t e : h->events) cudaEventDestroy(e);
  for (cudaEvent_t e : h->tl_events) cudaEventDestroy(e);
  for (cudaEvent_t e : h->tl_launch) cudaEventDestroy(e);
  if (h->ev_fork) cudaEventDestroy(h->ev_fork);
  if (h->ev_join) cudaEventDestroy(h->ev_join);
  if (h->s_main) cudaStreamDestroy(h->s_main);
  if (h->s_bulk) cudaStreamDestroy(h->s_bulk);
  if (h->s_aux) cudaStreamDestroy(h->s_aux);
  if (h->ev_aux) cudaEventDestroy(h->ev_aux);
  h->fact.release();
  for (auto& m : h->maps) dev_free(m.d_map);
  for (auto& kv : h->plans) kv.second->release();
  delete h;
  return SLMM_OK;
}

int slmm_chol_stats(const slmm_chol_t* h, int64_t* i, double* d) {
  SLMM_TRY
  if (!h) throw std::invalid_argument("null handle");
  const Symbolic& S = h->S;
  if (i) {
    i[0] = S.n; i[1] = S.nsuper; i[2] = S.nlevels; i[3] = S.nnzL; i[4] = S.lsize; i[5] = h->exported_nnz;
    i[6] = S.max_front_rows; i[7] = S.max_super_cols; i[8] = S.ncomponents;
    i[9] = (int64_t)h->fact.launches.size();
    size_t b = h->bytes;
    for (auto& kv : h->plans) b += kv.second->bytes;
    for (auto& m : h->maps) b += m.nnz * 8;
    i[10] = (int64_t)b;
  }
  if (d) { d[0] = S.flops; d[1] = S.t_order; d[2] = S.t_symbolic; d[3] = h->fact.flops; }
  return SLMM_OK;
  SLMM_CATCH
}

int slmm_chol_perm(const slmm_chol_t* h, int32_t* perm) {
  SLMM_TRY
  if (!h || !perm) throw std::invalid_argument("null argument");
  memcpy(perm, h->S.perm.data(), sizeof(int32_t) * h->S.n);
  return SLMM_OK;
  SLMM_CATCH
}

int slmm_chol_device_perm(const slmm_chol_t* h, const int32_t** d_perm, const int32_t** d_iperm) {
  if (!h || !d_perm || !d_iperm) return SLMM_ERR_INVALID;
  *d_perm = h->d_perm;
  *d_iperm = h->d_iperm;
  return SLMM_OK;
}

int slmm_chol_register_pattern_tri(slmm_chol_t* h, const int32_t* indptr, const int32_t* indices, int32_t tri,
                                   int32_t* map_id) {
  SLMM_TRY
  if (!h || !indptr || !indices || !map_id) throw std::invalid_argument("null argument");
  const int64_t nnz = indptr[h->S.n];
  std::vector<int64_t> tgt(nnz);
  entry_map(h->S, indptr, indices, tgt.data(), tri);
  EntryMap m;
  m.nnz = nnz;
  m.d_map = dev_upload(tgt.data(), tgt.size());
  CUDA_OK(cudaDeviceSynchronize());
  h->maps.push_back(m);
  *map_id = (int32_t)h->maps.size() - 1;
  return SLMM_OK;
  SLMM_CATCH
}

int slmm_chol_register_pattern(slmm_chol_t* h, const int32_t* indptr, const int32_t* indices, int32_t* map_id) {
  return slmm_chol_register_pattern_tri(h, indptr, indices, 0, map_id);
}

int slmm_chol_register_pattern_device(slmm_chol_t* h, const int32_t* d_indptr, const int32_t* d_indices, int64_t nnz,
                                      int32_t tri, int32_t* map_id) {
  SLMM_TRY
  if (!h || !d_indptr || !d_indices || !map_id || nnz < 0) throw std::invalid_argument("bad arguments");
  EntryMap m;
  m.nnz = nnz;
  m.d_map = dev_alloc<int64_t>((size_t)nnz);
  int* d_bad = dev_alloc<int>(1);
  CUDA_OK(cudaMemsetAsync(d_bad, 0, sizeof(int), 0));
  const int n = h->S.n;
  entry_map_kernel<<<std::max(1, std::min(148 * 8, (n + 7) / 8)), 256>>>(d_indptr, d_indices, n, h->d_iperm, h->d_col2sn,
                                                                       h->devsym(), tri, m.d_map, d_bad);
  g_launch_count++;
  int bad = 0;
  const cudaError_t e = cudaMemcpy(&bad, d_bad, sizeof(int), cudaMemcpyDeviceToHost);
  dev_free(d_bad);
  if (e != cudaSuccess || bad) {
    dev_free(m.d_map);
    CUDA_OK(e);
    throw std::invalid_argument("matrix entry outside the analysed pattern");
  }
  h->maps.push_back(m);
  *map_id = (int32_t)h->maps.size() - 1;
  return SLMM_OK;
  SLMM_CATCH
}

int slmm_chol_add_values(slmm_chol_t* h, int32_t map_id, const double* d_values, double sigma, int32_t first) {
  SLMM_TRY
  if (!h || map_id < 0 || map_id >= (int)h->maps.size()) throw std::invalid_argument("bad map id");
  if (first) CUDA_OK(cudaMemsetAsync(h->Lx, 0, h->S.lsize * sizeof(double), 0));
  const EntryMap& m = h->maps[map_id];
  if (m.nnz > 0) {
    const int grid = (int)std::min<int64_t>((m.nnz + 255) / 256, 148 * 16);
    scatter_axpy_kernel<<<grid, 256>>>(m.d_map, d_values, sigma, h->Lx, m.nnz);
    g_launch_count++;
  }
  CUDA_OK(cudaGetLastError());
  h->factored = false;
  return SLMM_OK;
  SLMM_CATCH
}

int slmm_chol_add_values2(slmm_chol_t* h, int32_t map_id, const double* d_values0, double sigma0,
                          const double* d_values1, double sigma1, int32_t first) {
  SLMM_TRY
  if (!h || map_id < 0 || map_id >= (int)h->maps.size() || !d_values0 || !d_values1) throw std::invalid_argument("bad arguments");
  if (first) CUDA_OK(cudaMemsetAsync(h->Lx, 0, h->S.lsize * sizeof(double), 0));
  const EntryMap& m = h->maps[map_id];
  if (m.nnz > 0) {
    const int grid = (int)std::min<int64_t>((m.nnz + 255) / 256, 148 * 16);
    scatter_axpy2_kernel<<<grid, 256>>>(m.d_map, d_values0, sigma0, d_values1, sigma1, h->Lx, m.nnz);
    g_launch_count++;
  }
  CUDA_OK(cudaGetLastError());
  h->factored = false;
  return SLMM_OK;
  SLMM_CATCH
}

int slmm_chol_factorize(slmm_chol_t* h, int32_t* fail_col) {
  SLMM_TRY
  if (!h) throw std::invalid_argument("null handle");
  const int big = 0x7fffffff;
  CUDA_OK(cudaMemcpyAsync(h->d_info, &big, sizeof(int), cudaMemcpyHostToDevice, 0));
  run_schedule(h, h->fact, nullptr, nullptr, nullptr, 0);
  int info = 0;
  CUDA_OK(cudaMemcpy(&info, h->d_info, sizeof(int), cudaMemcpyDeviceToHost));
  if (info != big) {
    if (fail_col) *fail_col = info - 1;
    set_last_error("matrix is not positive definite (non-positive pivot at permuted column " + std::to_string(info - 1) + ")");
    return SLMM_ERR_NOT_POSDEF;
  }
  if (fail_col) *fail_col = -1;
  h->factored = true;
  return SLMM_OK;
  SLMM_CATCH
}

int slmm_chol_logdet(slmm_chol_t* h, double* out) {
  SLMM_TRY
  if (!h || !out) throw std::invalid_argument("null argument");
  if (!h->factored) throw std::invalid_argument("factorize first");
  const int grid = std::min(1024, (h->S.n + 255) / 256);
  logdet_kernel<<<grid, 256>>>(h->Lx, h->d_col2sn, h->d_sn_first, h->d_sn_nrow, h->d_sn_lptr, h->S.n, h->d_partial);
  g_launch_count++;
  std::vector<double> part(grid);
  CUDA_OK(cudaMemcpy(part.data(), h->d_partial, grid * sizeof(double), cudaMemcpyDeviceToHost));
  double s = 0;
  for (double v : part) s += v;
  *out = 2.0 * s;
  return SLMM_OK;
  SLMM_CATCH
}

int slmm_chol_solve(slmm_chol_t* h, double* d_B, int32_t nrhs, int32_t mode) {
  SLMM_TRY
  if (!h || !d_B || nrhs <= 0) throw std::invalid_argument("bad arguments");
  if (!h->factored) throw std::invalid_argument("factorize first");
  SolvePlan* pl = get_plan(h, nrhs);
  const int n = h->S.n;
  const int64_t total = (int64_t)n * nrhs;
  const int grid = (int)std::min<int64_t>((total + 255) / 256, 148 * 32);
  gather_rows_kernel<<<grid, 256, 0, h->cur>>>(d_B, mode == 2 ? pl->X2 : pl->X, h->d_perm, n, nrhs, 0);
  if (mode == 0 || mode == 1) run_schedule(h, pl->fwd, pl->X, pl->arena, pl->d_vptr, nrhs);
  if (mode == 0 || mode == 2) run_schedule(h, pl->bwd, pl->X, pl->arena, pl->d_vptr, nrhs);
  gather_rows_kernel<<<grid, 256, 0, h->cur>>>(mode == 1 ? pl->X2 : pl->X, d_B, h->d_perm, n, nrhs, 1);
  g_launch_count += 2;
  CUDA_OK(cudaGetLastError());
  return SLMM_OK;
  SLMM_CATCH
}

int slmm_chol_lmul(slmm_chol_t* h, const double* d_Z, double* d_out, int32_t nrhs) {
  SLMM_TRY
  if (!h || !d_Z || !d_out || nrhs <= 0) throw std::invalid_argument("bad arguments");
  if (!h->factored) throw std::invalid_argument("factorize first");
  SolvePlan* pl = get_plan(h, nrhs);
  const int n = h->S.n;
  const int64_t total = (int64_t)n * nrhs;
  CUDA_OK(cudaMemcpyAsync(pl->X, d_Z, total * sizeof(double), cudaMemcpyDeviceToDevice, h->cur));
  run_schedule(h, pl->lmul, pl->X2, pl->arena, pl->d_vptr, nrhs);
  const int grid = (int)std::min<int64_t>((total + 255) / 256, 148 * 32);
  gather_rows_kernel<<<grid, 256, 0, h->cur>>>(pl->X2, d_out, h->d_perm, n, nrhs, 1);
  g_launch_count++;
  CUDA_OK(cudaGetLastError());
  return SLMM_OK;
  SLMM_CATCH
}

int slmm_probe_normals(double* d_out, int64_t n, int32_t ncols, int32_t col_begin, uint64_t seed, uint64_t stream) {
  SLMM_TRY
  if (!d_out || n <= 0 || ncols <= 0 || col_begin < 0) throw std::invalid_argument("bad arguments");
  const int64_t total = n * ncols;
  const int grid = (int)std::min<int64_t>((total + 255) / 256, 148 * 16);
  probe_normals_kernel<<<grid, 256>>>(d_out, n, ncols, col_begin, seed, stream);
  g_launch_count++;
  CUDA_OK(cudaGetLastError());
  return SLMM_OK;
  SLMM_CATCH
}

int slmm_chol_export_L(slmm_chol_t* h, int64_t* colptr, int32_t* rowidx, double* values) {
  SLMM_TRY
  if (!h || !colptr || !rowidx || !values) throw std::invalid_argument("null argument");
  if (!h->factored) throw std::invalid_argument("factorize first");
  const Symbolic& S = h->S;
  std::vector<double> Lh(S.lsize);
  CUDA_OK(cudaMemcpy(Lh.data(), h->Lx, S.lsize * sizeof(double), cudaMemcpyDeviceToHost));
  int64_t q = 0;
  for (int s = 0; s < S.nsuper; s++) {
    const int f = S.sn_first[s], ns = S.sn_first[s + 1] - f, ms = S.sn_nrow[s];
    const int32_t* rows = S.rows.data() + S.sn_rowptr[s];
    const double* P = Lh.data() + S.sn_lptr[s];
    for (int c = 0; c < ns; c++) {
      colptr[f + c] = q;
      for (int r = c; r < ms; r++) { rowidx[q] = rows[r]; values[q] = P[r + (int64_t)c * panel_ld(ms)]; q++; }
    }
  }
  colptr[S.n] = q;
  return SLMM_OK;
  SLMM_CATCH
}

int slmm_chol_aux_begin(slmm_chol_t* h) {
  SLMM_TRY
  if (!h || !h->s_aux) throw std::invalid_argument("null handle");
  if (h->cur != nullptr) throw std::invalid_argument("auxiliary section already open");
  CUDA_OK(cudaEventRecord(h->ev_aux, 0));
  CUDA_OK(cudaStreamWaitEvent(h->s_aux, h->ev_aux, 0));
  h->cur = h->s_aux;
  return SLMM_OK;
  SLMM_CATCH
}

int slmm_chol_aux_end(slmm_chol_t* h) {
  if (!h) return SLMM_ERR_INVALID;
  h->cur = nullptr;
  return SLMM_OK;
}

int slmm_chol_aux_join(slmm_chol_t* h) {
  SLMM_TRY
  if (!h || !h->s_aux) throw std::invalid_argument("null handle");
  CUDA_OK(cudaEventRecord(h->ev_aux, h->s_aux));
  CUDA_OK(cudaStreamWaitEvent(0, h->ev_aux, 0));
  return SLMM_OK;
  SLMM_CATCH
}

int slmm_chol_copy_panels(slmm_chol_t* h, double* host_out) {
  SLMM_TRY
  if (!h || !host_out) throw std::invalid_argument("null argument");
  CUDA_OK(cudaMemcpy(host_out, h->Lx, h->S.lsize * sizeof(double), cudaMemcpyDeviceToHost));
  return SLMM_OK;
  SLMM_CATCH
}

int slmm_launch_count(int64_t* out, int32_t reset) {
  if (out) *out = g_launch_count;
  if (reset) g_launch_count = 0;
  return SLMM_OK;
}

int slmm_chol_set_profiling(slmm_chol_t* h, int32_t on) {
  if (!h) return SLMM_ERR_INVALID;
  h->profiling = on != 0;
  for (int k = 0; k < 16; k++) { h->prof_ms[k] = 0; h->prof_flops[k] = 0; h->prof_n[k] = 0; }
  h->prof_launch_ms.clear(); h->prof_launch_flops.clear(); h->prof_launch_kind.clear(); h->prof_launch_grid.clear();
  return SLMM_OK;
}

int slmm_chol_set_timeline(slmm_chol_t* h, int32_t on) {
  if (!h) return SLMM_ERR_INVALID;
  h->timeline = on != 0;
  return SLMM_OK;
}

int slmm_chol_get_timeline(slmm_chol_t* h, int32_t max_n, int32_t* n_out, float* ms, int32_t* stream) {
  SLMM_TRY
  if (!h || !n_out) throw std::invalid_argument("null argument");
  const int n = h->tl_count;
  *n_out = n;
  if (ms) {
    std::vector<int> rec_stream(std::max(0, n - 2), 0);
    for (const Launch& L : h->fact.launches)
      if (L.kind == Launch::EV_RECORD && L.count + 2 < n) rec_stream[L.count] = L.stream;
    for (int q = 0; q < n && q < max_n; q++) {
      float v = 0.f;
      if (q > 0) CUDA_OK(cudaEventElapsedTime(&v, h->tl_events[0], h->tl_events[q]));
      ms[q] = v;
      if (stream) stream[q] = q >= 2 ? rec_stream[q - 2] : 0;
    }
  }
  return SLMM_OK;
  SLMM_CATCH
}

int slmm_chol_get_launch_timeline(slmm_chol_t* h, int32_t max_n, int32_t* n_out, float* end_ms, int32_t* stream,
                                  int32_t* kind, int32_t* grid, double* flops) {
  SLMM_TRY
  if (!h || !n_out) throw std::invalid_argument("null argument");
  std::vector<const Launch*> ks;
  for (const Launch& L : h->fact.launches) if (is_kernel(L)) ks.push_back(&L);
  const int n = (int)std::min(ks.size(), h->tl_launch.size());
  *n_out = n;
  for (int q = 0; q < n && q < max_n; q++) {
    if (end_ms) { float v = 0.f; CUDA_OK(cudaEventElapsedTime(&v, h->tl_events[0], h->tl_launch[q])); end_ms[q] = v; }
    if (stream) stream[q] = ks[q]->stream;
    if (kind) kind[q] = (int)ks[q]->kind;
    if (grid) grid[q] = (ks[q]->kind <= Launch::GEMM_SMALL || ks[q]->kind >= Launch::SKINNY_F1) ? ks[q]->grid : ks[q]->count;
    if (flops) flops[q] = ks[q]->flops;
  }
  return SLMM_OK;
  SLMM_CATCH
}

int slmm_chol_get_profile(const slmm_chol_t* h, double* ms6, double* flops6, int64_t* n6) {
  if (!h || !ms6 || !flops6 || !n6) return SLMM_ERR_INVALID;
  for (int k = 0; k < 6; k++) { ms6[k] = h->prof_ms[k]; flops6[k] = h->prof_flops[k]; n6[k] = h->prof_n[k]; }
  return SLMM_OK;
}

int slmm_chol_get_profile_ex(const slmm_chol_t* h, int32_t nkinds, double* ms, double* flops, int64_t* n) {
  if (!h || !ms || !flops || !n || nkinds < 0 || nkinds > 16) return SLMM_ERR_INVALID;
  for (int k = 0; k < nkinds; k++) { ms[k] = h->prof_ms[k]; flops[k] = h->prof_flops[k]; n[k] = h->prof_n[k]; }
  return SLMM_OK;
}

int slmm_chol_get_launch_profile(const slmm_chol_t* h, int64_t max_n, int64_t* n_out, float* ms, double* flops,
                                 int32_t* kind, int32_t* grid) {
  if (!h || !n_out) return SLMM_ERR_INVALID;
  const int64_t n = (int64_t)h->prof_launch_ms.size();
  *n_out = n;
  for (int64_t i = 0; i < n && i < max_n; i++) {
    if (ms) ms[i] = h->prof_launch_ms[i];
    if (flops) flops[i] = h->prof_launch_flops[i];
    if (kind) kind[i] = h->prof_launch_kind[i];
    if (grid) grid[i] = h->prof_launch_grid[i];
  }
  return SLMM_OK;
}

struct slmm_symbolic { Symbolic S; };

int slmm_symbolic_create(int32_t n, const int32_t* indptr, const int32_t* indices, int32_t ordering,
                         const int32_t* user_perm, slmm_symbolic_t** out) {
  SLMM_TRY
  if (n <= 0 || !indptr || !indices || !out) throw std::invalid_argument("slmm_symbolic_create: bad arguments");
  std::unique_ptr<slmm_symbolic> h(new slmm_symbolic());
  SymbolicOptions opt;
  opt.ordering = ordering;
  analyze(n, indptr, indices, user_perm, opt, h->S);
  *out = h.release();
  return SLMM_OK;
  SLMM_CATCH
}

int slmm_symbolic_destroy(slmm_symbolic_t* s) { delete s; return SLMM_OK; }

int slmm_symbolic_stats(const slmm_symbolic_t* h, int64_t* i, double* d) {
  SLMM_TRY
  if (!h) throw std::invalid_argument("null handle");
  const Symbolic& S = h->S;
  if (i) {
    int64_t exported = 0;
    for (int s = 0; s < S.nsuper; s++) {
      const int64_t ns = S.sn_first[s + 1] - S.sn_first[s], ms = S.sn_nrow[s];
      exported += ns * ms - ns * (ns - 1) / 2;
    }
    i[0] = S.n; i[1] = S.nsuper; i[2] = S.nlevels; i[3] = S.nnzL; i[4] = S.lsize; i[5] = exported;
    i[6] = S.max_front_rows; i[7] = S.max_super_cols; i[8] = S.ncomponents; i[9] = (int64_t)S.rows.size();
  }
  if (d) { d[0] = S.flops; d[1] = S.t_order; d[2] = S.t_symbolic; d[3] = 0; }
  return SLMM_OK;
  SLMM_CATCH
}

int slmm_symbolic_arrays(const slmm_symbolic_t* h, int32_t* perm, int32_t* parent, int32_t* colcount,
                         int32_t* sn_first, int32_t* sn_nrow, int32_t* sn_parent, int64_t* sn_rowptr,
                         int64_t* sn_lptr, int32_t* rows, int32_t* rel, int32_t* level_ptr, int32_t* level_sn) {
  SLMM_TRY
  if (!h) throw std::invalid_argument("null handle");
  const Symbolic& S = h->S;
  copy_out(perm, S.perm); copy_out(parent, S.parent); copy_out(colcount, S.colcount);
  copy_out(sn_first, S.sn_first); copy_out(sn_nrow, S.sn_nrow); copy_out(sn_parent, S.sn_parent);
  copy_out(sn_rowptr, S.sn_rowptr); copy_out(sn_lptr, S.sn_lptr); copy_out(rows, S.rows); copy_out(rel, S.rel);
  copy_out(level_ptr, S.level_ptr); copy_out(level_sn, S.level_sn);
  return SLMM_OK;
  SLMM_CATCH
}

int slmm_symbolic_entry_map_tri(const slmm_symbolic_t* h, const int32_t* indptr, const int32_t* indices, int32_t tri,
                                int64_t* target) {
  SLMM_TRY
  if (!h || !indptr || !indices || !target) throw std::invalid_argument("null argument");
  entry_map(h->S, indptr, indices, target, tri);
  return SLMM_OK;
  SLMM_CATCH
}

int slmm_symbolic_entry_map(const slmm_symbolic_t* h, const int32_t* indptr, const int32_t* indices, int64_t* target) {
  SLMM_TRY
  if (!h || !indptr || !indices || !target) throw std::invalid_argument("null argument");
  entry_map(h->S, indptr, indices, target);
  return SLMM_OK;
  SLMM_CATCH
}

int slmm_gemm_selftest_ex(int32_t M, int32_t N, int32_t K, const double* d_A, int64_t lda, const double* d_B, int64_t ldb,
                          double* d_C, int64_t ldc, int32_t flags, int32_t copies) {
  SLMM_TRY
  init_kernel_attributes();
  Schedule sch;
  PhaseBuilder pb;
  pb.allow_split = false;
  for (int c = 0; c < copies; c++)
    pb.add(make_op(d_C + (int64_t)c * ldc * N, 1, ldc, d_A, 1, lda, d_B, 1, ldb, M, N, K, flags & (GF_LOWER | GF_ACCUM | GF_NEG)));
  pb.flush(sch);
  sch.upload();
  slmm_chol dummy;
  run_schedule(&dummy, sch, nullptr, nullptr, nullptr, 0);
  CUDA_OK(cudaDeviceSynchronize());
  sch.release();
  return SLMM_OK;
  SLMM_CATCH
}

int slmm_gemm_selftest(int32_t M, int32_t N, int32_t K, const double* d_A, const double* d_B, double* d_C,
                       int32_t lower, int32_t reps, float* ms_out) {
  SLMM_TRY
  init_kernel_attributes();
  Schedule sch;
  PhaseBuilder pb;
  pb.add(make_op(d_C, 1, M, d_A, 1, M, d_B, 1, N, M, N, K, lower ? GF_LOWER : 0));
  pb.flush(sch);
  sch.upload();
  cudaEvent_t e0, e1;
  CUDA_OK(cudaEventCreate(&e0));
  CUDA_OK(cudaEventCreate(&e1));
  slmm_chol dummy;
  run_schedule(&dummy, sch, nullptr, nullptr, nullptr, 0);
  CUDA_OK(cudaEventRecord(e0, 0));
  for (int r = 0; r < reps; r++) run_schedule(&dummy, sch, nullptr, nullptr, nullptr, 0);
  CUDA_OK(cudaEventRecord(e1, 0));
  CUDA_OK(cudaEventSynchronize(e1));
  float ms = 0;
  CUDA_OK(cudaEventElapsedTime(&ms, e0, e1));
  if (ms_out) *ms_out = reps > 0 ? ms / reps : 0.f;
  cudaEventDestroy(e0);
  cudaEventDestroy(e1);
  sch.release();
  return SLMM_OK;
  SLMM_CATCH
}

}
```

### scilmm_b200/csrc/dense_tiles.cuh

```cuda
#pragma once
#include <cuda_runtime.h>

#include <cstdint>

namespace slmm {

constexpr int NBI = 64;

enum GemmFlags { GF_LOWER = 1, GF_ACCUM = 2, GF_NEG = 4, GF_WS = 8 ,
                 GF_BIGTILE = 16 ,
                 GF_TRIL_B = 32 ,
                 GF_WS2 = 64  };

struct GemmOp {
  double* C;
  const double* A;
  const double* B;
  const int32_t* a_kidx;
  int64_t c_si, c_sj, a_si, a_sk, b_sj, b_sk;
  int32_t M, N, K;
  int32_t flags;
  int32_t tile_start, tiles_m, tiles_n, pad;
};

struct ReduceOp {
  double* C;
  const double* ws;
  int64_t c_si, c_sj;
  int32_t M, N, S, flags;
  int32_t block_start, pad;
};

struct PotrfOp {
  double* blk;
  double* inv;
  int32_t ld, nb;
  int32_t colbase;
  int32_t inv_ld;
};

__device__ __forceinline__ void dmma884(double& c0, double& c1, double a, double b) {
  asm volatile("mma.sync.aligned.m8n8k4.row.col.f64.f64.f64.f64 {%0,%1}, {%2}, {%3}, {%0,%1};\n"
               : "+d"(c0), "+d"(c1)
               : "d"(a), "d"(b));
}

__device__ __forceinline__ void cp_async8(double* smem_dst, const double* gsrc, int src_bytes) {
  const unsigned d = (unsigned)__cvta_generic_to_shared(smem_dst);
  asm volatile("cp.async.ca.shared.global [%0], [%1], 8, %2;\n" ::"r"(d), "l"(gsrc), "r"(src_bytes) : "memory");
}
__device__ __forceinline__ void mbar_init(uint64_t* bar, int count) {
  asm volatile("mbarrier.init.shared::cta.b64 [%0], %1;\n" ::"r"((unsigned)__cvta_generic_to_shared(bar)), "r"(count) : "memory");
}
__device__ __forceinline__ void mbar_arrive(uint64_t* bar) {
  asm volatile("{\n.reg .b64 st;\nmbarrier.arrive.shared::cta.b64 st, [%0];\n}\n" ::"r"((unsigned)__cvta_generic_to_shared(bar)) : "memory");
}
__device__ __forceinline__ void mbar_cp_async_arrive(uint64_t* bar) {
  asm volatile("cp.async.mbarrier.arrive.noinc.shared::cta.b64 [%0];\n" ::"r"((unsigned)__cvta_generic_to_shared(bar)) : "memory");
}
__device__ __forceinline__ void mbar_wait(uint64_t* bar, int parity) {
  const unsigned a = (unsigned)__cvta_generic_to_shared(bar);
  unsigned done = 0;
  while (!done) {
    asm volatile("{\n.reg .pred p;\nmbarrier.try_wait.parity.shared::cta.b64 p, [%1], %2;\nselp.u32 %0, 1, 0, p;\n}\n"
                 : "=r"(done) : "r"(a), "r"(parity) : "memory");
  }
}

constexpr int NPW = 4;

template <int REGS>
__device__ __forceinline__ void reg_dealloc() { asm volatile("setmaxnreg.dec.sync.aligned.u32 %0;\n" ::"n"(REGS)); }
template <int REGS>
__device__ __forceinline__ void reg_alloc() { asm volatile("setmaxnreg.inc.sync.aligned.u32 %0;\n" ::"n"(REGS)); }

template <int T, int LD>
__device__ __noinline__ void produce_operand(double* __restrict__ sm, const double* __restrict__ base, int64_t s_i,
                                                int64_t s_k, const int32_t* __restrict__ kidx, bool kcontig, int rem,
                                                int k0, int K, int pw, int lane) {
  constexpr int KS = 16;
  if (!kcontig) {
    const int64_t lane_off = (int64_t)lane * s_i, chunk = 32 * s_i;
#pragma unroll
    for (int kq = 0; kq < KS / NPW; kq++) {
      const int k = pw * (KS / NPW) + kq;
      const bool kok = k0 + k < K;
      int64_t gk = k0 + k;
      if (kidx != nullptr) gk = kok ? kidx[k0 + k] : 0;
      const double* src = base + gk * s_k + lane_off;
      double* dst = sm + k * LD + lane;
#pragma unroll
      for (int c = 0; c < T / 32; c++) {
        const bool ok = kok && (lane + 32 * c < rem);
        cp_async8(dst + 32 * c, ok ? src + c * chunk : base, ok ? 8 : 0);
      }
    }
  } else {
    const int k = lane & 15, r = lane >> 4;
    const bool kok = k0 + k < K;
    const double* src = base + (k0 + k);
    double* dst = sm + k * LD;
#pragma unroll
    for (int c = 0; c < T / 2 / NPW; c++) {
      const int i = 2 * (pw * (T / 2 / NPW) + c) + r;
      const bool ok = kok && i < rem;
      cp_async8(dst + i, ok ? src + (int64_t)i * s_i : base, ok ? 8 : 0);
    }
  }
}

template <int TM, int TN, int NWM, int NWN, int STAGES>
__global__ void __launch_bounds__(32 * (NWM * NWN + NPW), 1) gemm_tiles_kernel(const GemmOp* __restrict__ ops,
                                                                                const int32_t* __restrict__ tile_op) {
  constexpr int NCW = NWM * NWN;
  constexpr int KS = 16;
  constexpr int WM = TM / NWM, WN = TN / NWN;
  constexpr int MI = WM / 8, NI = WN / 8;
  constexpr int LDA = TM + 4, LDB = TN + 4;
  constexpr bool REBALANCE = (NCW == 8);
  static_assert(TM % 32 == 0 && TN % 32 == 0 && NCW % 4 == 0, "producer mapping / warpgroup layout");
  extern __shared__ double smem[];
  double* As = smem;
  double* Bs = smem + STAGES * KS * LDA;
  uint64_t* full_bar = reinterpret_cast<uint64_t*>(Bs + STAGES * KS * LDB);
  uint64_t* empty_bar = full_bar + STAGES;

  const int tile = blockIdx.x;
  const GemmOp& op = ops[tile_op[tile]];
  const int local = tile - op.tile_start;
  const int tiles_m = op.tiles_m;
  const int tm0 = (local % tiles_m) * TM, tn0 = (local / tiles_m) * TN;
  const int flags = op.flags;
  if ((flags & GF_LOWER) && tm0 + TM <= tn0) return;

  const int tid = threadIdx.x, lane = tid & 31, warp = tid >> 5;
  const int M = op.M, N = op.N;
  const int K = (flags & GF_TRIL_B) ? min(op.K, max(0, tn0 + TN - op.pad)) : op.K;
  const int nslab = (K + KS - 1) / KS;
  if (tid == 0) {
    for (int s = 0; s < STAGES; s++) { mbar_init(full_bar + s, 32 * NPW); mbar_init(empty_bar + s, NCW); }
    asm volatile("fence.mbarrier_init.release.cluster;\n" ::: "memory");
  }
  __syncthreads();

  if (warp >= NCW) {
    if (REBALANCE) reg_dealloc<56>();
    const int pw = warp - NCW;
    const int Mrem = M - tm0, Nrem = N - tn0;
    const int64_t a_si = op.a_si, a_sk = op.a_sk, b_sj = op.b_sj, b_sk = op.b_sk;
    const int32_t* kidx = op.a_kidx;
    const bool a_kcontig = (a_sk == 1 && kidx == nullptr && a_si != 1);
    const bool b_kcontig = (b_sk == 1 && b_sj != 1);
    const double* Abase = op.A + (int64_t)tm0 * a_si;
    const double* Bbase = op.B + (int64_t)tn0 * b_sj;
    if ((flags & GF_ACCUM) && op.c_si == 1) {
      const int pt = pw * 32 + lane;
      if (pt < TN && tn0 + pt < N) {
        const double* ccol = op.C + (int64_t)tm0 + (int64_t)(tn0 + pt) * op.c_sj;
        const int rows = min(TM, M - tm0);
        const int r_first = (flags & GF_LOWER) ? max(0, tn0 + pt - tm0) : 0;
        for (int r = (r_first / 16) * 16; r < rows; r += 16)
          asm volatile("prefetch.global.L2 [%0];\n" ::"l"(ccol + r));
      }
    }
    for (int s = 0; s < nslab; s++) {
      const int stage = s % STAGES, use = s / STAGES;
      if (use > 0) mbar_wait(empty_bar + stage, (use - 1) & 1);
      const int k0 = s * KS;
      produce_operand<TM, LDA>(As + stage * KS * LDA, Abase, a_si, a_sk, kidx, a_kcontig, Mrem, k0, K, pw, lane);
      produce_operand<TN, LDB>(Bs + stage * KS * LDB, Bbase, b_sj, b_sk, nullptr, b_kcontig, Nrem, k0, K, pw, lane);
      mbar_cp_async_arrive(full_bar + stage);
    }
    return;
  }
  if (REBALANCE) reg_alloc<224>();

  const int g = lane >> 2, t = lane & 3;
  const int wm0 = (warp % NWM) * WM, wn0 = (warp / NWM) * WN;
  double acc[MI][NI][2];
#pragma unroll
  for (int mi = 0; mi < MI; mi++)
#pragma unroll
    for (int ni = 0; ni < NI; ni++) acc[mi][ni][0] = acc[mi][ni][1] = 0.0;

  for (int s = 0; s < nslab; s++) {
    const int stage = s % STAGES;
    mbar_wait(full_bar + stage, (s / STAGES) & 1);
    const double* as = As + stage * KS * LDA + wm0 + g;
    const double* bs = Bs + stage * KS * LDB + wn0 + g;
#pragma unroll
    for (int kk = 0; kk < KS; kk += 4) {
      double af[MI], bf[NI];
#pragma unroll
      for (int mi = 0; mi < MI; mi++) af[mi] = as[(kk + t) * LDA + mi * 8];
#pragma unroll
      for (int ni = 0; ni < NI; ni++) bf[ni] = bs[(kk + t) * LDB + ni * 8];
#pragma unroll
      for (int mi = 0; mi < MI; mi++)
#pragma unroll
        for (int ni = 0; ni < NI; ni++) dmma884(acc[mi][ni][0], acc[mi][ni][1], af[mi], bf[ni]);
    }
    __syncwarp();
    if (lane == 0) mbar_arrive(empty_bar + stage);
  }

  const bool accum = flags & GF_ACCUM, neg = flags & GF_NEG, lower = flags & GF_LOWER;
  double* Cb = op.C;
  const int64_t c_si = op.c_si, c_sj = op.c_sj;
  constexpr int MB = 1;
#pragma unroll
  for (int mb = 0; mb < MI; mb += MB) {
    double old[MB][NI][2];
    bool ok[MB][NI][2];
#pragma unroll
    for (int m2 = 0; m2 < MB; m2++) {
      const int i = tm0 + wm0 + (mb + m2) * 8 + g;
#pragma unroll
      for (int ni = 0; ni < NI; ni++)
#pragma unroll
        for (int h = 0; h < 2; h++) {
          const int j = tn0 + wn0 + ni * 8 + 2 * t + h;
          ok[m2][ni][h] = (i < M) && (j < N) && !(lower && i < j);
          old[m2][ni][h] = 0.0;
        }
    }
    if (accum) {
#pragma unroll
      for (int m2 = 0; m2 < MB; m2++) {
        const int i = tm0 + wm0 + (mb + m2) * 8 + g;
#pragma unroll
        for (int ni = 0; ni < NI; ni++)
#pragma unroll
          for (int h = 0; h < 2; h++) {
            const int j = tn0 + wn0 + ni * 8 + 2 * t + h;
            if (ok[m2][ni][h]) old[m2][ni][h] = Cb[(int64_t)i * c_si + (int64_t)j * c_sj];
          }
      }
    }
#pragma unroll
    for (int m2 = 0; m2 < MB; m2++) {
      const int i = tm0 + wm0 + (mb + m2) * 8 + g;
#pragma unroll
      for (int ni = 0; ni < NI; ni++)
#pragma unroll
        for (int h = 0; h < 2; h++) {
          const int j = tn0 + wn0 + ni * 8 + 2 * t + h;
          const double a = acc[mb + m2][ni][h];
          if (ok[m2][ni][h]) Cb[(int64_t)i * c_si + (int64_t)j * c_sj] = old[m2][ni][h] + (neg ? -a : a);
        }
    }
  }
}

__global__ void __launch_bounds__(256) splitk_reduce_kernel(const ReduceOp* __restrict__ ops, int nops) {
  int lo = 0, hi = nops - 1;
  const int blk = blockIdx.x;
  while (lo < hi) {
    int mid = (lo + hi + 1) >> 1;
    if (ops[mid].block_start <= blk) lo = mid; else hi = mid - 1;
  }
  const ReduceOp op = ops[lo];
  const int64_t total = (int64_t)op.M * op.N;
  const int64_t e = (int64_t)(blk - op.block_start) * 256 + threadIdx.x;
  if (e >= total) return;
  double sum = 0.0;
  for (int s = 0; s < op.S; s++) sum += op.ws[(int64_t)s * total + e];
  const int i = (int)(e % op.M), j = (int)(e / op.M);
  double* cp = op.C + (int64_t)i * op.c_si + (int64_t)j * op.c_sj;
  const double v = (op.flags & GF_NEG) ? -sum : sum;
  *cp = (op.flags & GF_ACCUM) ? *cp + v : v;
}

}
```

### scilmm_b200/csrc/potrf_block.cuh

```cuda
#pragma once
#include "dense_tiles.cuh"

namespace slmm {

constexpr int PQ = 8;
constexpr int PLD = NBI + 1;
constexpr int POTRF4_SMEM = 3 * NBI * PLD * 8;

#ifdef POTRF_DEBUG
__device__ long long g_potrf_dbg[8];
#define PDBG(i) if (threadIdx.x == 0 && blockIdx.x == 0) g_potrf_dbg[i] = clock64();
#else
#define PDBG(i)
#endif

__device__ __forceinline__ void tile_mma(double& c0, double& c1, const double* a, int lda, const double* b, int ldb, int K,
                                         int g, int t) {
  for (int k = 0; k < K; k += 4) dmma884(c0, c1, a[g * lda + k + t], b[g * ldb + k + t]);
}

__global__ void __launch_bounds__(256) potrf_inv_kernel_v4(const PotrfOp* __restrict__ ops, int* __restrict__ info) {
  extern __shared__ double pb_smem[];
  double (*A)[PLD] = reinterpret_cast<double (*)[PLD]>(pb_smem);
  double (*X)[PLD] = reinterpret_cast<double (*)[PLD]>(pb_smem + NBI * PLD);
  double (*T)[PLD] = reinterpret_cast<double (*)[PLD]>(pb_smem + 2 * NBI * PLD);
  __shared__ int fail;
  PDBG(0)
  const PotrfOp op = ops[blockIdx.x];
  const int nb = op.nb, tid = threadIdx.x, lane = tid & 31, warp = tid >> 5;
  const int g = lane >> 2, t = lane & 3;
  if (tid == 0) fail = 0;
  {
    double v[NBI * NBI / 256];
#pragma unroll
    for (int u = 0; u < NBI * NBI / 256; u++) {
      const int q = tid + 256 * u, i = q % NBI, j = q / NBI;
      v[u] = (i == j) ? 1.0 : 0.0;
      if (i < nb && j < nb) v[u] = (i >= j) ? __ldg(op.blk + i + (int64_t)j * op.ld) : 0.0;
    }
#pragma unroll
    for (int u = 0; u < NBI * NBI / 256; u++) {
      const int q = tid + 256 * u, i = q % NBI, j = q / NBI;
      A[i][j] = v[u];
      X[i][j] = 0.0;
    }
  }
  __syncthreads();
  PDBG(1)
  const int nsteps = (nb + PQ - 1) / PQ;
  for (int kq = 0; kq < NBI / PQ; kq++) {
    const int kb = kq * PQ;
    if (kq >= nsteps) {
      if (tid < PQ) X[kb + tid][kb + tid] = 1.0;
      continue;
    }
    if (warp == 0) {
      const int i = lane & 7;
      double a[PQ];
#pragma unroll
      for (int c = 0; c < PQ; c++) a[c] = A[kb + i][kb + c];
      int bad = 0;
      double ri[PQ];
#pragma unroll
      for (int j = 0; j < PQ; j++) {
        const double d = __shfl_sync(0xffffffffu, a[j], j);
        if (!(d > 0.0) && bad == 0) bad = kb + j + 1;
        const double rinv = rsqrt(d > 0.0 ? d : 1.0);
        ri[j] = rinv;
        const double l = (i == j) ? d * rinv : a[j] * rinv;
        a[j] = l;
#pragma unroll
        for (int k = j + 1; k < PQ; k++) {
          const double lk = __shfl_sync(0xffffffffu, l, k);
          a[k] = fma(-l, lk, a[k]);
        }
      }
      double x[PQ];
      const int c = lane & 7;
#pragma unroll
      for (int r = 0; r < PQ; r++) {
        double s = (r == c) ? 1.0 : 0.0;
#pragma unroll
        for (int k = 0; k < r; k++) {
          const double lrk = __shfl_sync(0xffffffffu, a[k], r);
          s = fma(-lrk, (k >= c) ? x[k] : 0.0, s);
        }
        x[r] = (r >= c) ? s * ri[r] : 0.0;
      }
      if (lane < PQ) {
#pragma unroll
        for (int cc = 0; cc < PQ; cc++) A[kb + i][kb + cc] = (cc <= i) ? a[cc] : 0.0;
#pragma unroll
        for (int r = 0; r < PQ; r++) X[kb + r][kb + c] = x[r];
      }
      if (bad && lane == 0) fail = bad;
    }
    __syncthreads();
    if (fail) break;
    const int r0 = kb + PQ, ntile = (NBI - r0) / PQ;
    if (warp < ntile) {
      const int i0 = r0 + PQ * warp;
      double c0 = 0.0, c1 = 0.0;
      tile_mma(c0, c1, &A[i0][kb], PLD, &X[kb][kb], PLD, PQ, g, t);
      __syncwarp();
      A[i0 + g][kb + 2 * t] = c0;
      A[i0 + g][kb + 2 * t + 1] = c1;
    }
    __syncthreads();
    const int npair = ntile * (ntile + 1) / 2;
    for (int p = warp; p < npair; p += 8) {
      int ti = 0, rem = p;
      while (rem > ti) { rem -= ti + 1; ti++; }
      const int tj = rem;
      const int i0 = r0 + PQ * ti, j0 = r0 + PQ * tj;
      double c0 = 0.0, c1 = 0.0;
      tile_mma(c0, c1, &A[i0][kb], PLD, &A[j0][kb], PLD, PQ, g, t);
      A[i0 + g][j0 + 2 * t] -= c0;
      A[i0 + g][j0 + 2 * t + 1] -= c1;
    }
    __syncthreads();
  }
  __syncthreads();
  PDBG(2)
  if (fail) {
    if (tid == 0) atomicMin(info, op.colbase + fail);
    return;
  }
#pragma unroll 1
  for (int m = PQ; m < NBI; m *= 2) {
    const int tpb = (m / PQ) * (m / PQ);
    const int ntile = (NBI / (2 * m)) * tpb;
    for (int q = warp; q < ntile; q += 8) {
      const int pr = q / tpb, ti = (q % tpb) / (m / PQ), tj = q % (m / PQ);
      const int lo = pr * 2 * m;
      double c0 = 0.0, c1 = 0.0;
      for (int k = 0; k < m; k += 4)
        dmma884(c0, c1, A[lo + m + PQ * ti + g][lo + k + t], X[lo + k + t][lo + PQ * tj + g]);
      T[lo + m + PQ * ti + g][lo + PQ * tj + 2 * t] = c0;
      T[lo + m + PQ * ti + g][lo + PQ * tj + 2 * t + 1] = c1;
    }
    __syncthreads();
    for (int q = warp; q < ntile; q += 8) {
      const int pr = q / tpb, ti = (q % tpb) / (m / PQ), tj = q % (m / PQ);
      const int lo = pr * 2 * m;
      double c0 = 0.0, c1 = 0.0;
      for (int k = 0; k < m; k += 4)
        dmma884(c0, c1, X[lo + m + PQ * ti + g][lo + m + k + t], T[lo + m + k + t][lo + PQ * tj + g]);
      X[lo + m + PQ * ti + g][lo + PQ * tj + 2 * t] = -c0;
      X[lo + m + PQ * ti + g][lo + PQ * tj + 2 * t + 1] = -c1;
    }
    __syncthreads();
  }
  PDBG(3)
  for (int q = tid; q < NBI * NBI; q += 256) {
    const int i = q % NBI, jj = q / NBI;
    if (i < nb && jj < nb && i >= jj) op.blk[i + (int64_t)jj * op.ld] = A[i][jj];
    if (op.inv_ld == NBI || (i < nb && jj < nb)) op.inv[i + (int64_t)jj * op.inv_ld] = (i < nb && jj < nb) ? X[i][jj] : 0.0;
  }
  PDBG(4)
}

}
```

### scilmm_b200/engine.py

```python
import ctypes as C

import numpy as np
import scipy.sparse as sp

from . import _lib
from ._lib import check, lib, np_ptr

ORDERINGS = {"natural": 0, "given": 1, "metis": 2, "nesdis": 2, "default": 2, "amd": 3, "mindeg": 3,
             "nesdis_fast": 4, "metis_fast": 4}


def _torch():
    import torch
    return torch


def require_cuda():
    torch = _torch()
    if not torch.cuda.is_available():
        raise RuntimeError("scilmm_b200 needs a CUDA device (sm_100a); there is no CPU fallback")
    return torch


def device_count():
    c = C.c_int(0)
    check(lib().slmm_device_count(C.byref(c)))
    return c.value


def _as_i32(a):
    return np.ascontiguousarray(a, dtype=np.int32)


def _as_f64(a):
    return np.ascontiguousarray(a, dtype=np.float64)


def canonical_csr(m):
    m = sp.csr_matrix(m)
    if not m.has_sorted_indices:
        m = m.sorted_indices()
    if m.indices.dtype != np.int32 or m.indptr.dtype != np.int32:
        m = sp.csr_matrix((m.data, m.indices.astype(np.int32), m.indptr.astype(np.int32)), shape=m.shape)
    if m.data.dtype != np.float64:
        m = m.astype(np.float64)
    return m


UPLOAD_THREADS = 4


def to_device(a, torch=None):
    torch = torch or require_cuda()
    a = np.ascontiguousarray(a)
    if a.nbytes < (4 << 20):
        return torch.from_numpy(a).to("cuda", non_blocking=False)
    out = torch.empty(a.shape, dtype=torch.from_numpy(a[:0].reshape(-1)).dtype, device="cuda")
    check(lib().slmm_upload_h2d(out.data_ptr(), np_ptr(a), int(a.nbytes), int(UPLOAD_THREADS)))
    return out


def upload_columns(Z, col_begin, col_end, torch=None):
    torch = torch or require_cuda()
    n, s = int(Z.shape[0]), int(Z.shape[1])
    if torch.is_tensor(Z):
        if Z.dtype != torch.float64 or not Z.is_contiguous() or Z.is_cuda:
            raise ValueError("upload_columns needs a contiguous float64 host block")
        src, itemsize = Z.data_ptr(), 8
    else:
        if Z.dtype != np.float64 or not Z.flags.c_contiguous:
            raise ValueError("upload_columns needs a C-ordered float64 host block")
        src, itemsize = Z.ctypes.data, 8
    w = int(col_end) - int(col_begin)
    out = torch.empty(n, w, dtype=torch.float64, device="cuda")
    if n == 0 or w <= 0:
        return out
    check(lib().slmm_upload_h2d_2d(out.data_ptr(), w * itemsize, src + int(col_begin) * itemsize, s * itemsize,
                                   w * itemsize, n))
    return out


class SymbolicView(object):

    def __init__(self, pattern, ordering="metis", perm=None):
        pattern = canonical_csr(pattern)
        n = pattern.shape[0]
        h = C.c_void_p()
        self._perm_in = None if perm is None else _as_i32(perm)
        code = ORDERINGS[ordering] if perm is None else 1
        check(lib().slmm_symbolic_create(n, np_ptr(pattern.indptr), np_ptr(pattern.indices), code,
                                         None if perm is None else np_ptr(self._perm_in), C.byref(h)))
        self._h = h
        self.n = n
        i = np.zeros(16, dtype=np.int64)
        d = np.zeros(8, dtype=np.float64)
        check(lib().slmm_symbolic_stats(h, np_ptr(i), np_ptr(d)))
        self.nsuper, self.nlevels, self.nnzL, self.lsize = int(i[1]), int(i[2]), int(i[3]), int(i[4])
        self.exported_nnz, self.max_front_rows, self.max_super_cols = int(i[5]), int(i[6]), int(i[7])
        self.ncomponents, self.total_rows = int(i[8]), int(i[9])
        self.flops, self.t_order, self.t_symbolic = float(d[0]), float(d[1]), float(d[2])

    def arrays(self):
        n, ns = self.n, self.nsuper
        out = dict(perm=np.zeros(n, np.int32), parent=np.zeros(n, np.int32), colcount=np.zeros(n, np.int32),
                   sn_first=np.zeros(ns + 1, np.int32), sn_nrow=np.zeros(ns, np.int32),
                   sn_parent=np.zeros(ns, np.int32), sn_rowptr=np.zeros(ns + 1, np.int64),
                   sn_lptr=np.zeros(ns + 1, np.int64), rows=np.zeros(self.total_rows, np.int32),
                   rel=np.zeros(self.total_rows, np.int32), level_ptr=np.zeros(self.nlevels + 1, np.int32),
                   level_sn=np.zeros(ns, np.int32))
        order = ["perm", "parent", "colcount", "sn_first", "sn_nrow", "sn_parent", "sn_rowptr", "sn_lptr", "rows",
                 "rel", "level_ptr", "level_sn"]
        check(lib().slmm_symbolic_arrays(self._h, *[np_ptr(out[k]) for k in order]))
        out["sn_ld"] = ((out["sn_nrow"].astype(np.int64) + 1) & ~np.int64(1)).astype(np.int64)
        return out

    def entry_map(self, pattern):
        pattern = canonical_csr(pattern)
        tgt = np.zeros(pattern.nnz, dtype=np.int64)
        check(lib().slmm_symbolic_entry_map(self._h, np_ptr(pattern.indptr), np_ptr(pattern.indices), np_ptr(tgt)))
        return tgt

    def __del__(self):
        try:
            if getattr(self, "_h", None):
                lib().slmm_symbolic_destroy(self._h)
                self._h = None
        except Exception:
            pass


def _csr_arrays(m, row_range=None):
    if not sp.isspmatrix_csr(m):
        m = sp.csr_matrix(m)
    ip, ix, dt = m.indptr, m.indices, m.data
    if row_range is not None and tuple(row_range) != (0, m.shape[0]):
        r0, r1 = row_range
        a, b = int(ip[r0]), int(ip[r1])
        ip = (ip[r0:r1 + 1] - ip[r0]).astype(np.int32)
        ix, dt = ix[a:b], dt[a:b]
    if ip.dtype != np.int32:
        ip = ip.astype(np.int32)
    if ix.dtype != np.int32:
        ix = ix.astype(np.int32)
    if dt.dtype != np.float64:
        dt = dt.astype(np.float64)
    return np.ascontiguousarray(ip), np.ascontiguousarray(ix), np.ascontiguousarray(dt), int(ix.size)


class MatSet(object):

    def __init__(self, mats, row_range=None):
        torch = require_cuda()
        self.n = mats[0].shape[0]
        self.K = len(mats)
        self.row_range = (0, self.n) if row_range is None else (int(row_range[0]), int(row_range[1]))
        h = C.c_void_p()
        check(lib().slmm_matset_create(self.n, self.K, C.byref(h)))
        self._h = h
        if self.row_range != (0, self.n):
            check(lib().slmm_matset_set_row_range(h, self.row_range[0], self.row_range[1]))
        self._sym_known = self.row_range == (0, self.n)
        self._keep = []
        self.nnz = []
        self.h2d_bytes = 0
        patterns = []
        for k, m in enumerate(mats):
            if m.shape != (self.n, self.n):
                raise ValueError("all matrices must be n x n")
            self._bind(k, m, patterns, torch, verified=False)
        self._out = torch.zeros(2 * self.K + 2 * self.K * self.K, dtype=torch.float64, device="cuda")

    def _bind(self, k, m, patterns, torch, verified):
        ip, ix, dt, nnz = _csr_arrays(m, self.row_range)
        dat_t = to_device(dt, torch)
        self.h2d_bytes += dt.nbytes
        same = -1
        ptr_t = idx_t = None
        for (j, ipj, nnzj, ptr_j, idx_j) in patterns:
            if nnzj != nnz or not (ipj is ip or np.array_equal(ipj, ip)):
                continue
            if idx_t is None:
                idx_t = to_device(ix, torch)
                self.h2d_bytes += ix.nbytes
            eq = C.c_int32(0)
            check(lib().slmm_device_arrays_equal_i32(idx_j.data_ptr(), idx_t.data_ptr(), nnz, C.byref(eq)))
            if eq.value:
                same, ptr_t, idx_t = j, ptr_j, idx_j
                break
        if same < 0:
            ptr_t = to_device(ip, torch)
            if idx_t is None:
                idx_t = to_device(ix, torch)
                self.h2d_bytes += ix.nbytes
            self.h2d_bytes += ip.nbytes
        check(lib().slmm_matset_bind_device(self._h, k, ptr_t.data_ptr(), idx_t.data_ptr(), dat_t.data_ptr(), nnz, same))
        if same < 0 and not verified:
            flags = C.c_int32(0)
            check(lib().slmm_matset_validate(self._h, k, C.byref(flags)))
            if flags.value & 2:
                raise ValueError("matrix %d: CSR indices / row pointers out of range" % k)
            if flags.value & 1:
                if self.row_range != (0, self.n):
                    raise ValueError("matrix %d: row-block shards need canonical CSR (sorted rows, no duplicates)" % k)
                mc = sp.csr_matrix(m).copy()
                mc.sum_duplicates()
                return self._bind(k, canonical_csr(mc), patterns, torch, verified=True)
        if same < 0:
            patterns.append((k, ip, nnz, ptr_t, idx_t))
        if len(self._keep) > k:
            self._keep[k] = (ptr_t, idx_t, dat_t)
            self.nnz[k] = nnz
        else:
            self._keep.append((ptr_t, idx_t, dat_t))
            self.nnz.append(nnz)

    def values_ptr(self, k):
        return self._keep[k][2].data_ptr()

    def device_arrays(self, k):
        return self._keep[k]

    def pattern_is_subset(self, k_small, k_big):
        a, b = self._keep[k_small], self._keep[k_big]
        if a[1].data_ptr() == b[1].data_ptr():
            return True
        return device_pattern_subset(a[0], a[1], b[0], b[1], self.n)

    def resolve_symmetry_sharded(self, allreduce_sum_):
        if self._sym_known:
            return
        torch = _torch()
        h = np.zeros(2 * self.K, dtype=np.uint64)
        for k in range(self.K):
            check(lib().slmm_matset_symmetry_hash(self._h, k, np_ptr(h[2 * k:2 * k + 2])))
        t = torch.from_numpy(h.view(np.int64).copy()).to("cuda")
        allreduce_sum_(t)
        tot = t.cpu().numpy()
        for k in range(self.K):
            check(lib().slmm_matset_set_symmetric(self._h, k, 1 if tot[2 * k] == tot[2 * k + 1] else 0))
        self._sym_known = True

    def he_moments_device(self, y_dev, row_begin=None, row_end=None):
        row_begin = self.row_range[0] if row_begin is None else row_begin
        row_end = self.row_range[1] if row_end is None else row_end
        check(lib().slmm_he_moments(self._h, y_dev.data_ptr(), int(row_begin), int(row_end), self._out.data_ptr()))
        return self._out

    @staticmethod
    def split_moments(out, K):
        out = np.asarray(out)
        q_off, q_diag = out[:K], out[K:2 * K]
        S_off = out[2 * K:2 * K + K * K].reshape(K, K)
        S_diag = out[2 * K + K * K:].reshape(K, K)
        S_off = np.tril(S_off) + np.tril(S_off, -1).T
        S_diag = np.tril(S_diag) + np.tril(S_diag, -1).T
        return q_off, q_diag, S_off, S_diag

    def spmm(self, k, X, out=None):
        torch = _torch()
        X2 = X if X.dim() == 2 else X.unsqueeze(1)
        X2 = X2.contiguous()
        ncols = X2.shape[1]
        if out is None:
            out = torch.empty_like(X2)
        for c0 in range(0, ncols, 256):
            c1 = min(ncols, c0 + 256)
            if c0 == 0 and c1 == ncols:
                check(lib().slmm_spmm(self._h, k, X2.data_ptr(), ncols, out.data_ptr()))
            else:
                blk = X2[:, c0:c1].contiguous()
                o = torch.empty_like(blk)
                check(lib().slmm_spmm(self._h, k, blk.data_ptr(), c1 - c0, o.data_ptr()))
                out[:, c0:c1] = o
        return out if X.dim() == 2 else out[:, 0]

    def coldot(self, k, X, row_begin=0, row_end=None):
        torch = _torch()
        X2 = (X if X.dim() == 2 else X.unsqueeze(1)).contiguous()
        ncols = X2.shape[1]
        row_end = self.n if row_end is None else row_end
        out = torch.empty(ncols, dtype=torch.float64, device="cuda")
        for c0 in range(0, ncols, 256):
            c1 = min(ncols, c0 + 256)
            blk = X2 if (c0 == 0 and c1 == ncols) else X2[:, c0:c1].contiguous()
            o = out if (c0 == 0 and c1 == ncols) else torch.empty(c1 - c0, dtype=torch.float64, device="cuda")
            check(lib().slmm_spmm_coldot(self._h, k, blk.data_ptr(), c1 - c0, int(row_begin), int(row_end),
                                         o.data_ptr()))
            if o is not out:
                out[c0:c1] = o
        return out

    def pattern_id(self, k):
        v = C.c_int32(-1)
        check(lib().slmm_matset_pattern_id(self._h, int(k), C.byref(v)))
        return v.value

    def pattern_groups(self, max_group=2):
        groups, out = {}, []
        for k in range(self.K):
            groups.setdefault(self.pattern_id(k), []).append(k)
        for ks in groups.values():
            for i in range(0, len(ks), max_group):
                out.append(ks[i:i + max_group])
        return out

    def coldot_multi(self, ks, X, store_from=None, row_begin=0, row_end=None):
        torch = _torch()
        X2 = X.contiguous()
        n, ncols = X2.shape
        row_end = self.n if row_end is None else row_end
        store_from = ncols if store_from is None else store_from
        ks_arr = np.asarray(ks, dtype=np.int32)
        dots = torch.empty(len(ks), ncols, dtype=torch.float64, device="cuda")
        store = None
        if store_from < ncols:
            store = torch.zeros(len(ks), n, ncols - store_from, dtype=torch.float64, device="cuda")
        check(lib().slmm_spmm_coldot_multi(self._h, len(ks), np_ptr(ks_arr), X2.data_ptr(), int(ncols), int(store_from),
                                           store.data_ptr() if store is not None else None, int(row_begin),
                                           int(row_end), dots.data_ptr()))
        return dots, store

    def quadform_gram_multi(self, ks, X, XB, row_begin=0, row_end=None):
        torch = _torch()
        X2, B2 = X.contiguous(), XB.contiguous()
        ncols, nb = X2.shape[1], B2.shape[1]
        row_end = self.n if row_end is None else row_end
        ks_arr = np.asarray(ks, dtype=np.int32)
        dots = torch.empty(len(ks), ncols, dtype=torch.float64, device="cuda")
        half = torch.empty(len(ks), nb, nb, dtype=torch.float64, device="cuda")
        check(lib().slmm_quadform_gram_multi(self._h, len(ks), np_ptr(ks_arr), X2.data_ptr(), int(ncols),
                                             B2.data_ptr(), int(nb), int(row_begin), int(row_end),
                                             dots.data_ptr(), half.data_ptr()))
        return dots, half + half.transpose(1, 2)

    def build_tiles(self, k, chol_engine):
        dp, di = chol_engine.device_perm()
        check(lib().slmm_matset_build_tiles(self._h, int(k), dp, di))
        self._tiled = getattr(self, "_tiled", set()) | {int(k)}

    def tile_stats(self, k):
        out = np.zeros(4, dtype=np.int64)
        check(lib().slmm_matset_tile_stats(self._h, int(k), np_ptr(out)))
        return dict(tiles=int(out[0]), entries=int(out[1]), distinct=int(out[2]), ctas=int(out[3]))

    def tile_cta_profile(self, k):
        ncta = self.tile_stats(k)["ctas"]
        out = np.zeros((ncta, 4), dtype=np.int64)
        check(lib().slmm_matset_tile_cta_profile(self._h, int(k), np_ptr(out), int(ncta)))
        return out

    def has_tiles(self, ks):
        t = getattr(self, "_tiled", set())
        return all(int(k) in t for k in ks)

    def quadform_tiled(self, ks, X, nb):
        torch = _torch()
        X2 = X.contiguous()
        ncols = X2.shape[1]
        ks_arr = np.asarray(ks, dtype=np.int32)
        dots = torch.empty(len(ks), ncols, dtype=torch.float64, device="cuda")
        half = torch.empty(len(ks), max(nb, 1), max(nb, 1), dtype=torch.float64, device="cuda")
        check(lib().slmm_quadform_tiled(self._h, len(ks), np_ptr(ks_arr), X2.data_ptr(), int(ncols), int(nb),
                                        dots.data_ptr(), half.data_ptr() if nb > 0 else None))
        return dots, (half + half.transpose(1, 2)) if nb > 0 else None

    def is_symmetric(self, k):
        v = C.c_int32(0)
        check(lib().slmm_matset_is_symmetric(self._h, int(k), C.byref(v)))
        return bool(v.value)

    def quadform_multi(self, ks, X, row_begin=0, row_end=None):
        torch = _torch()
        X2 = (X if X.dim() == 2 else X.unsqueeze(1)).contiguous()
        ncols = X2.shape[1]
        row_end = self.n if row_end is None else row_end
        ks_arr = np.asarray(ks, dtype=np.int32)
        dots = torch.empty(len(ks), ncols, dtype=torch.float64, device="cuda")
        for c0 in range(0, ncols, 160):
            c1 = min(ncols, c0 + 160)
            whole = c0 == 0 and c1 == ncols
            blk = X2 if whole else X2[:, c0:c1].contiguous()
            o = dots if whole else torch.empty(len(ks), c1 - c0, dtype=torch.float64, device="cuda")
            check(lib().slmm_quadform_multi(self._h, len(ks), np_ptr(ks_arr), blk.data_ptr(), int(c1 - c0),
                                            int(row_begin), int(row_end), o.data_ptr()))
            if not whole:
                dots[:, c0:c1] = o
        return dots

    def __del__(self):
        try:
            if getattr(self, "_h", None):
                lib().slmm_matset_destroy(self._h)
                self._h = None
        except Exception:
            pass


def device_csr_is_symmetric(ptr_t, idx_t, dat_t, n):
    v = C.c_int32(0)
    check(lib().slmm_device_csr_is_symmetric(ptr_t.data_ptr(), idx_t.data_ptr(), dat_t.data_ptr(), int(n), C.byref(v)))
    return bool(v.value)


def device_pattern_subset(ap_t, ai_t, bp_t, bi_t, n):
    v = C.c_int32(0)
    check(lib().slmm_device_pattern_subset(ap_t.data_ptr(), ai_t.data_ptr(), bp_t.data_ptr(), bi_t.data_ptr(), int(n),
                                           C.byref(v)))
    return bool(v.value)


class CholEngine(object):

    def __init__(self, pattern, ordering="metis", perm=None):
        require_cuda()
        pattern = canonical_csr(pattern)
        self.n = pattern.shape[0]
        h = C.c_void_p()
        self._perm_in = None if perm is None else _as_i32(perm)
        code = ORDERINGS[ordering] if perm is None else 1
        check(lib().slmm_chol_analyze(self.n, np_ptr(pattern.indptr), np_ptr(pattern.indices), code,
                                      None if perm is None else np_ptr(self._perm_in), C.byref(h)))
        self._h = h
        self._perm = None
        self.factorizations = 0

    def stats(self):
        i = np.zeros(16, dtype=np.int64)
        d = np.zeros(8, dtype=np.float64)
        check(lib().slmm_chol_stats(self._h, np_ptr(i), np_ptr(d)))
        return dict(n=int(i[0]), nsuper=int(i[1]), nlevels=int(i[2]), nnzL=int(i[3]), lsize=int(i[4]),
                    exported_nnz=int(i[5]), max_front_rows=int(i[6]), max_super_cols=int(i[7]),
                    ncomponents=int(i[8]), launches=int(i[9]), device_bytes=int(i[10]), flops=float(d[0]),
                    t_order=float(d[1]), t_symbolic=float(d[2]), issued_flops=float(d[3]))

    def perm(self):
        if self._perm is None:
            p = np.zeros(self.n, dtype=np.int32)
            check(lib().slmm_chol_perm(self._h, np_ptr(p)))
            self._perm = p
        return self._perm

    def device_perm(self):
        a, b = C.c_void_p(), C.c_void_p()
        check(lib().slmm_chol_device_perm(self._h, C.byref(a), C.byref(b)))
        return a, b

    def register_pattern(self, pattern, tri=0):
        pattern = canonical_csr(pattern)
        mid = C.c_int32(-1)
        check(lib().slmm_chol_register_pattern_tri(self._h, np_ptr(pattern.indptr), np_ptr(pattern.indices),
                                                   int(tri), C.byref(mid)))
        return mid.value

    def register_pattern_device(self, ptr_t, idx_t, nnz, tri=0):
        mid = C.c_int32(-1)
        check(lib().slmm_chol_register_pattern_device(self._h, ptr_t.data_ptr(), idx_t.data_ptr(), int(nnz),
                                                      int(tri), C.byref(mid)))
        return mid.value

    def add_values(self, map_id, values_ptr, sigma, first):
        check(lib().slmm_chol_add_values(self._h, int(map_id), values_ptr, float(sigma), 1 if first else 0))

    def add_values2(self, map_id, values_ptr0, sigma0, values_ptr1, sigma1, first):
        check(lib().slmm_chol_add_values2(self._h, int(map_id), values_ptr0, float(sigma0), values_ptr1, float(sigma1),
                                          1 if first else 0))

    def factorize(self):
        col = C.c_int32(-1)
        code = lib().slmm_chol_factorize(self._h, C.byref(col))
        check(code, col.value)
        self.factorizations += 1

    def logdet(self):
        v = C.c_double(0.0)
        check(lib().slmm_chol_logdet(self._h, C.byref(v)))
        return v.value

    def solve_(self, B, mode=0):
        if not B.is_contiguous():
            raise ValueError("solve_ needs a contiguous tensor")
        nrhs = 1 if B.dim() == 1 else B.shape[1]
        check(lib().slmm_chol_solve(self._h, B.data_ptr(), int(nrhs), int(mode)))
        return B

    def lmul(self, Z):
        torch = _torch()
        Z2 = (Z if Z.dim() == 2 else Z.unsqueeze(1)).contiguous()
        out = torch.empty_like(Z2)
        check(lib().slmm_chol_lmul(self._h, Z2.data_ptr(), out.data_ptr(), int(Z2.shape[1])))
        return out if Z.dim() == 2 else out[:, 0]

    def probe_normals(self, n, ncols, col_begin, seed, stream):
        torch = _torch()
        out = torch.empty(int(n), int(ncols), dtype=torch.float64, device="cuda")
        check(lib().slmm_probe_normals(out.data_ptr(), int(n), int(ncols), int(col_begin), int(seed) & (2 ** 64 - 1),
                                       int(stream) & (2 ** 64 - 1)))
        return out

    def aux_begin(self):
        check(lib().slmm_chol_aux_begin(self._h))

    def aux_end(self):
        check(lib().slmm_chol_aux_end(self._h))

    def aux_join(self):
        check(lib().slmm_chol_aux_join(self._h))

    def panels(self):
        out = np.zeros(self.stats()["lsize"], dtype=np.float64)
        check(lib().slmm_chol_copy_panels(self._h, np_ptr(out)))
        return out

    def set_profiling(self, on):
        check(lib().slmm_chol_set_profiling(self._h, 1 if on else 0))

    def timeline(self):
        check(lib().slmm_chol_set_timeline(self._h, 1))
        try:
            self.factorize()
        finally:
            check(lib().slmm_chol_set_timeline(self._h, 0))
        n = C.c_int32(0)
        check(lib().slmm_chol_get_timeline(self._h, 0, C.byref(n), None, None))
        ms, st = np.zeros(n.value, np.float32), np.zeros(n.value, np.int32)
        check(lib().slmm_chol_get_timeline(self._h, n.value, C.byref(n), np_ptr(ms), np_ptr(st)))
        return ms, st

    def launch_timeline(self):
        n = C.c_int32(0)
        check(lib().slmm_chol_get_launch_timeline(self._h, 0, C.byref(n), None, None, None, None, None))
        end, fl = np.zeros(n.value, np.float32), np.zeros(n.value)
        st, kind, grid = (np.zeros(n.value, np.int32) for _ in range(3))
        check(lib().slmm_chol_get_launch_timeline(self._h, n.value, C.byref(n), np_ptr(end), np_ptr(st), np_ptr(kind),
                                                  np_ptr(grid), np_ptr(fl)))
        return end, st, kind, grid, fl

    def profile(self):
        ms, fl, n = np.zeros(13), np.zeros(13), np.zeros(13, dtype=np.int64)
        check(lib().slmm_chol_get_profile_ex(self._h, 13, np_ptr(ms), np_ptr(fl), np_ptr(n)))
        names = ["potrf_inv", "gemm_big", "gemm_small", "extend_add", "rhs_pull", "extend_add_big", "init_w",
                 "splitk_reduce", "_ev_record", "_ev_wait", "skinny_f1", "skinny_f2", "gemm_tma"]
        return {names[k]: dict(ms=float(ms[k]), flops=float(fl[k]), launches=int(n[k])) for k in range(13)
                if not names[k].startswith("_")}

    def launch_profile(self):
        n = C.c_int64(0)
        check(lib().slmm_chol_get_launch_profile(self._h, 0, C.byref(n), None, None, None, None))
        ms, fl = np.zeros(n.value, np.float32), np.zeros(n.value)
        kind, grid = np.zeros(n.value, np.int32), np.zeros(n.value, np.int32)
        check(lib().slmm_chol_get_launch_profile(self._h, n.value, C.byref(n), np_ptr(ms), np_ptr(fl), np_ptr(kind),
                                                 np_ptr(grid)))
        return ms, fl, kind, grid

    def export_L(self):
        st = self.stats()
        nnz = st["exported_nnz"]
        colptr = np.zeros(self.n + 1, dtype=np.int64)
        rowidx = np.zeros(nnz, dtype=np.int32)
        vals = np.zeros(nnz, dtype=np.float64)
        check(lib().slmm_chol_export_L(self._h, np_ptr(colptr), np_ptr(rowidx), np_ptr(vals)))
        return sp.csc_matrix((vals, rowidx, colptr), shape=(self.n, self.n))

    def __del__(self):
        try:
            if getattr(self, "_h", None):
                lib().slmm_chol_destroy(self._h)
                self._h = None
        except Exception:
            pass


def launch_count(reset=False):
    v = C.c_int64(0)
    check(lib().slmm_launch_count(C.byref(v), 1 if reset else 0))
    return v.value


def gemm_selftest(M, N, K, lower=False, reps=5, seed=0):
    torch = require_cuda()
    g = torch.Generator(device="cuda").manual_seed(seed)
    A = torch.randn(K, M, generator=g, dtype=torch.float64, device="cuda")
    B = torch.randn(K, N, generator=g, dtype=torch.float64, device="cuda")
    Cm = torch.zeros(N, M, dtype=torch.float64, device="cuda")
    ms = C.c_float(0)
    check(lib().slmm_gemm_selftest(M, N, K, A.data_ptr(), B.data_ptr(), Cm.data_ptr(), 1 if lower else 0, reps,
                                   C.byref(ms)))
    ref = (A.t() @ B).t()
    got = Cm
    if lower:
        mask = torch.tril(torch.ones(M, N, dtype=torch.bool, device="cuda")).t()
        err = ((got - ref) * mask).abs().max().item()
        flops = M * N * K
    else:
        err = (got - ref).abs().max().item()
        flops = 2.0 * M * N * K
    return err, ms.value, flops / (ms.value * 1e-3) / 1e12 if ms.value > 0 else 0.0
```

Before: 0.1946.

## Fuse wide-supernode inner block Cholesky into one persistent dataflow kernel

Replaces the per-inner-block sequence of POTRF, TRSM and update launches inside each outer panel of a wide supernode with a single persistent kernel. CTAs grab work items from an atomic ticket and wait on per-tile acquire/release counters. The goal is to remove kernel launch overhead and the global barriers between small dependent steps of the dense factorization. In exchange it limits the work to 32 CTAs with spin-waiting, adds a counter memset per factorization, and adds launch start-time profiling plumbing.

```diff
diff --git a/include/scilmm_b200.h b/include/scilmm_b200.h
--- a/include/scilmm_b200.h
+++ b/include/scilmm_b200.h
@@ -24,6 +24,7 @@
 
 const char* slmm_last_error(void);
 int slmm_version(void);
+int slmm_chain_order_check(int32_t w);
 int slmm_device_count(int* out);
 
 int slmm_matset_create(int32_t n, int32_t K, slmm_matset_t** out);
@@ -102,8 +103,8 @@
 int slmm_chol_get_profile_ex(const slmm_chol_t* h, int32_t nkinds, double* ms, double* flops, int64_t* n);
 int slmm_chol_set_timeline(slmm_chol_t* h, int32_t on);
 int slmm_chol_get_timeline(slmm_chol_t* h, int32_t max_n, int32_t* n_out, float* ms, int32_t* stream);
-int slmm_chol_get_launch_timeline(slmm_chol_t* h, int32_t max_n, int32_t* n_out, float* end_ms, int32_t* stream,
-                                  int32_t* kind, int32_t* grid, double* flops);
+int slmm_chol_get_launch_timeline(slmm_chol_t* h, int32_t max_n, int32_t* n_out, float* start_ms, float* end_ms,
+                                  int32_t* stream, int32_t* kind, int32_t* grid, double* flops);
 int slmm_chol_get_launch_profile(const slmm_chol_t* h, int64_t max_n, int64_t* n_out, float* ms, double* flops,
                                  int32_t* kind, int32_t* grid);
 
diff --git a/scilmm_b200/_lib.py b/scilmm_b200/_lib.py
--- a/scilmm_b200/_lib.py
+++ b/scilmm_b200/_lib.py
@@ -25,6 +25,7 @@
 SIGNATURES = {
     "slmm_last_error": (C.c_char_p, []),
     "slmm_version": (C.c_int, []),
+    "slmm_chain_order_check": (C.c_int, [i32]),
     "slmm_device_count": (C.c_int, [C.POINTER(C.c_int)]),
     "slmm_matset_create": (C.c_int, [i32, i32, pp]),
     "slmm_matset_destroy": (C.c_int, [vp]),
@@ -80,7 +81,7 @@
     "slmm_chol_set_timeline": (C.c_int, [vp, i32]),
     "slmm_chol_get_timeline": (C.c_int, [vp, i32, C.POINTER(i32), vp, vp]),
     "slmm_chol_get_profile_ex": (C.c_int, [vp, i32, vp, vp, vp]),
-    "slmm_chol_get_launch_timeline": (C.c_int, [vp, i32, C.POINTER(i32), vp, vp, vp, vp, vp]),
+    "slmm_chol_get_launch_timeline": (C.c_int, [vp, i32, C.POINTER(i32), vp, vp, vp, vp, vp, vp]),
     "slmm_chol_get_profile": (C.c_int, [vp, vp, vp, vp]),
     "slmm_chol_get_launch_profile": (C.c_int, [vp, i64, C.POINTER(i64), vp, vp, vp, vp]),
     "slmm_symbolic_create": (C.c_int, [i32, vp, vp, i32, vp, pp]),
diff --git a/scilmm_b200/csrc/build.py b/scilmm_b200/csrc/build.py
--- a/scilmm_b200/csrc/build.py
+++ b/scilmm_b200/csrc/build.py
@@ -10,7 +10,7 @@
 METIS = os.path.join(CUDA_HOME, "lib64", "libmetis_static.a")
 SOURCES_CU = ["chol.cu", "sparse_ops.cu", "ibd.cu", "quadform_tiled.cu"]
 SOURCES_CPP = ["symbolic.cpp"]
-HEADERS = ["common.h", "dense_tiles.cuh", "potrf_block.cuh", "symbolic.h", "skinny_ops.cuh", "matset.h", "dense_tiles_tma.cuh"]
+HEADERS = ["common.h", "dense_tiles.cuh", "potrf_block.cuh", "symbolic.h", "skinny_ops.cuh", "matset.h", "dense_tiles_tma.cuh", "chain_block.cuh"]
 
 
 def _stale():
diff --git a/scilmm_b200/csrc/chain_block.cuh b/scilmm_b200/csrc/chain_block.cuh
--- /dev/null
+++ b/scilmm_b200/csrc/chain_block.cuh
@@ -0,0 +1,150 @@
+#pragma once
+#include "dense_tiles.cuh"
+#include "potrf_block.cuh"
+
+namespace slmm {
+
+struct ChainOp {
+  double* P;
+  double* winv;
+  int32_t ld, w, ldw, colbase;
+  int32_t item_start;
+  int32_t ctr_off;
+};
+
+struct ChainItem {
+  enum Kind { POTRF, TRSM, UPD } kind;
+  int k, i, j;
+};
+
+constexpr int CHAIN_CTAS = 32;
+constexpr int CHAIN_SMEM = POTRF4_SMEM > 4 * 16 * (64 + 4) * 2 * 8 + 2 * 4 * 8 ? POTRF4_SMEM : 4 * 16 * (64 + 4) * 2 * 8 + 2 * 4 * 8;
+
+__host__ __device__ inline int chain_nib(int w) { return (w + NBI - 1) / NBI; }
+
+__host__ __device__ inline int chain_iter_items(int nib, int k) {
+  const int m = nib - 1 - k;
+  return 1 + m + (k >= 1 ? m * (m + 1) / 2 : 0) + m;
+}
+
+__host__ __device__ inline int chain_items(int w) {
+  const int nib = chain_nib(w);
+  int n = 0;
+  for (int k = 0; k < nib; k++) n += chain_iter_items(nib, k);
+  return n;
+}
+
+__host__ __device__ inline ChainItem chain_item(int w, int t) {
+  const int nib = chain_nib(w);
+  int k = 0;
+  while (t >= chain_iter_items(nib, k)) { t -= chain_iter_items(nib, k); k++; }
+  const int m = nib - 1 - k;
+  if (t == 0) return {ChainItem::POTRF, k, k, k};
+  t -= 1;
+  if (t < m) return {ChainItem::TRSM, k, k + 1 + t, k};
+  t -= m;
+  if (k >= 1) {
+    for (int j = k + 1; j < nib; j++) {
+      if (t < nib - j) return {ChainItem::UPD, k - 1, j + t, j};
+      t -= nib - j;
+    }
+  }
+  return {ChainItem::UPD, k, k + 1 + t, k + 1};
+}
+
+__host__ __device__ inline int chain_tile(int i, int j) { return i * (i + 1) / 2 + j; }
+
+__device__ __forceinline__ int ld_acquire(const int* p) {
+  int v;
+  asm volatile("ld.acquire.gpu.global.s32 %0, [%1];\n" : "=r"(v) : "l"(p) : "memory");
+  return v;
+}
+__device__ __forceinline__ void st_release(int* p, int v) {
+  asm volatile("st.release.gpu.global.s32 [%0], %1;\n" ::"l"(p), "r"(v) : "memory");
+}
+__device__ __forceinline__ void wait_at_least(const int* p, int v) {
+  while (ld_acquire(p) < v) {}
+}
+
+__device__ __forceinline__ GemmOp chain_gemm_op(const ChainOp& c, bool upd, int k) {
+  const int c0 = k * NBI, c1 = c0 + NBI;
+  GemmOp op;
+  op.a_kidx = nullptr;
+  op.c_si = 1; op.c_sj = c.ld; op.a_si = 1; op.a_sk = c.ld;
+  op.A = c.P + c1 + (int64_t)c0 * c.ld;
+  op.M = c.w - c1; op.K = NBI;
+  op.tile_start = 0; op.pad = 0;
+  if (upd) {
+    op.C = c.P + c1 + (int64_t)c1 * c.ld;
+    op.B = op.A; op.b_sj = 1; op.b_sk = c.ld;
+    op.N = c.w - c1;
+    op.flags = GF_LOWER | GF_ACCUM | GF_NEG;
+  } else {
+    op.C = c.P + c1 + (int64_t)c0 * c.ld;
+    op.B = c.winv + c0 + (int64_t)c0 * c.ldw; op.b_sj = 1; op.b_sk = c.ldw;
+    op.N = NBI;
+    op.flags = 0;
+  }
+  op.tiles_m = (op.M + 63) / 64;
+  op.tiles_n = (op.N + 63) / 64;
+  return op;
+}
+
+__device__ __forceinline__ void mbar_inval(uint64_t* bar) {
+  asm volatile("mbarrier.inval.shared::cta.b64 [%0];\n" ::"r"((unsigned)__cvta_generic_to_shared(bar)) : "memory");
+}
+
+__global__ void __launch_bounds__(256, 1) wide_chain_kernel(const ChainOp* __restrict__ ops, int nops, int total,
+                                                            int* __restrict__ ticket, int* __restrict__ ctr,
+                                                            int* __restrict__ info) {
+  extern __shared__ double smem[];
+  __shared__ int s_t;
+  constexpr int STAGES = 4, LD = 64 + 4;
+  uint64_t* bars = reinterpret_cast<uint64_t*>(smem + 2 * STAGES * 16 * LD);
+  for (;;) {
+    if (threadIdx.x == 0) s_t = atomicAdd(ticket, 1);
+    __syncthreads();
+    const int t = s_t;
+    if (t >= total) return;
+    int q = 0;
+    while (q + 1 < nops && ops[q + 1].item_start <= t) q++;
+    const ChainOp c = ops[q];
+    const ChainItem it = chain_item(c.w, t - c.item_start);
+    int* tc = ctr + c.ctr_off;
+    if (threadIdx.x == 0) {
+      if (it.kind == ChainItem::POTRF) {
+        wait_at_least(tc + chain_tile(it.k, it.k), it.k);
+      } else if (it.kind == ChainItem::TRSM) {
+        wait_at_least(tc + chain_tile(it.k, it.k), it.k + 1);
+        wait_at_least(tc + chain_tile(it.i, it.k), it.k);
+      } else {
+        wait_at_least(tc + chain_tile(it.i, it.k), it.k + 1);
+        wait_at_least(tc + chain_tile(it.j, it.k), it.k + 1);
+        wait_at_least(tc + chain_tile(it.i, it.j), it.k);
+      }
+    }
+    __syncthreads();
+    if (it.kind == ChainItem::POTRF) {
+      const int c0 = it.k * NBI;
+      PotrfOp po;
+      po.blk = c.P + c0 + (int64_t)c0 * c.ld;
+      po.inv = c.winv + c0 + (int64_t)c0 * c.ldw;
+      po.ld = c.ld; po.nb = min(NBI, c.w - c0); po.colbase = c.colbase + c0; po.inv_ld = c.ldw;
+      potrf_inv_block<false>(po, info, smem);
+    } else {
+      const bool upd = it.kind == ChainItem::UPD;
+      const GemmOp op = chain_gemm_op(c, upd, it.k);
+      const int local = (it.i - it.k - 1) + (upd ? (it.j - it.k - 1) * op.tiles_m : 0);
+      gemm_tile<64, 64, 2, 2, STAGES>(op, local, smem);
+    }
+    __syncthreads();
+    if (threadIdx.x == 0) {
+      if (it.kind != ChainItem::POTRF)
+        for (int s = 0; s < 2 * STAGES; s++) mbar_inval(bars + s);
+      __threadfence();
+      st_release(tc + chain_tile(it.i, it.j), it.k + 1);
+    }
+  }
+}
+
+}
diff --git a/scilmm_b200/csrc/chol.cu b/scilmm_b200/csrc/chol.cu
--- a/scilmm_b200/csrc/chol.cu
+++ b/scilmm_b200/csrc/chol.cu
@@ -5,6 +5,7 @@
 #include <memory>
 #include <vector>
 
+#include "chain_block.cuh"
 #include "common.h"
 #include "dense_tiles.cuh"
 #include "dense_tiles_tma.cuh"
@@ -214,7 +215,8 @@
 struct Launch {
   enum Kind { POTRF, GEMM_BIG, GEMM_SMALL, PULL_MAT, PULL_VEC, PULL_MAT_BIG, INIT_W, REDUCE, EV_RECORD, EV_WAIT,
               SKINNY_F1, SKINNY_F2 ,
-              GEMM_TMA  } kind;
+              GEMM_TMA ,
+              CHAIN  } kind;
   int64_t off;
   int32_t count;
   int32_t grid;
@@ -257,6 +259,10 @@
   std::vector<Launch> launches;
   std::vector<GemmOp> gemm;
   std::vector<PotrfOp> potrf;
+  std::vector<ChainOp> chain;
+  ChainOp* d_chain = nullptr;
+  int64_t ctr_size = 0;
+  int* d_ctr = nullptr;
   std::vector<PullItem> pull;
   std::vector<PullEntry> pull_entries;
   PullEntry* d_pull_entries = nullptr;
@@ -293,6 +299,8 @@
     d_reduce = dev_upload(reduce.data(), reduce.size());
     d_gemm = dev_upload(gemm.data(), gemm.size());
     d_potrf = dev_upload(potrf.data(), potrf.size());
+    d_chain = dev_upload(chain.data(), chain.size());
+    if (ctr_size > 0) d_ctr = dev_alloc<int>(ctr_size);
     d_pull = dev_upload(pull.data(), pull.size());
     d_tile_op = dev_upload(tile_op.data(), tile_op.size());
     d_tmaps = dev_upload(tmaps.data(), tmaps.size());
@@ -303,11 +311,13 @@
     dev_free(d_gemm); dev_free(d_potrf); dev_free(d_pull); dev_free(d_ws); dev_free(d_ws2); dev_free(d_reduce); dev_free(d_tile_op); dev_free(d_pull_entries);
     d_ws2 = nullptr;
     dev_free(d_tmaps); d_tmaps = nullptr;
+    dev_free(d_chain); d_chain = nullptr;
+    dev_free(d_ctr); d_ctr = nullptr;
     d_tile_op = nullptr; d_pull_entries = nullptr;
     d_gemm = nullptr; d_potrf = nullptr; d_pull = nullptr; d_ws = nullptr; d_reduce = nullptr;
   }
   size_t device_bytes() const {
-    return gemm.size() * sizeof(GemmOp) + potrf.size() * sizeof(PotrfOp) + pull.size() * sizeof(PullItem) +
+    return gemm.size() * sizeof(GemmOp) + potrf.size() * sizeof(PotrfOp) + chain.size() * sizeof(ChainOp) + ctr_size * 4 + pull.size() * sizeof(PullItem) +
            reduce.size() * sizeof(ReduceOp) + (size_t)(ws_size + ws2_size) * 8 + tile_op.size() * 4 + pull_entries.size() * sizeof(PullEntry);
   }
 };
@@ -318,6 +328,7 @@
   int skinny_mt = 0;
   int ws_id = 0;
   std::vector<PotrfOp> potrf;
+  std::vector<ChainOp> chain;
   std::vector<ReduceOp> reduces;
   int64_t ws_used = 0;
   bool allow_split = true;
@@ -409,6 +420,35 @@
   }
   void flush(Schedule& sch, int stream = 0) {
     const size_t first_launch = sch.launches.size();
+    if (!chain.empty()) {
+      int items = 0;
+      double cf = 0;
+      Launch L{Launch::CHAIN, (int64_t)sch.chain.size(), (int32_t)chain.size(), 0, 0, 0.0};
+      L.aux_off = sch.ctr_size++;
+      for (ChainOp& c : chain) {
+        const int nib = chain_nib(c.w);
+        c.item_start = items;
+        c.ctr_off = (int32_t)sch.ctr_size;
+        sch.ctr_size += nib * (nib + 1) / 2;
+        items += chain_items(c.w);
+        for (int k = 0; k < nib; k++) {
+          const double nb = std::min(NBI, c.w - k * NBI), r = c.w - (k + 1) * NBI;
+          cf += 2.0 * nb * nb * nb / 3.0;
+          sch.flops += nb * nb * nb / 3.0;
+          if (r > 0) {
+            const double f = 2.0 * NBI * NBI * r + 2.0 * NBI * (r * r - r * (r - 1) / 2.0);
+            cf += f;
+            sch.flops += f;
+          }
+        }
+      }
+      if ((int64_t)sch.ctr_size > 0x7fffffff) throw std::runtime_error("chain counter area too large");
+      L.grid = std::min(items, CHAIN_CTAS);
+      L.tile_off = items;
+      L.flops = cf;
+      sch.launches.push_back(L);
+      sch.chain.insert(sch.chain.end(), chain.begin(), chain.end());
+    }
     if (!potrf.empty()) {
       double pf = 0;
       for (const PotrfOp& o : potrf) pf += 2.0 * o.nb * o.nb * o.nb / 3.0;
@@ -496,10 +536,10 @@
       if (ws_id) sch.ws2_size = std::max(sch.ws2_size, ws_used); else sch.ws_size = std::max(sch.ws_size, ws_used);
     }
     for (size_t q = first_launch; q < sch.launches.size(); q++) sch.launches[q].stream = stream;
-    big.clear(); small.clear(); tma.clear(); sk1.clear(); sk2.clear(); potrf.clear(); reduces.clear();
+    big.clear(); small.clear(); tma.clear(); sk1.clear(); sk2.clear(); potrf.clear(); chain.clear(); reduces.clear();
     ws_used = 0;
   }
-  bool empty() const { return big.empty() && small.empty() && tma.empty() && sk1.empty() && sk2.empty() && potrf.empty(); }
+  bool empty() const { return big.empty() && small.empty() && tma.empty() && sk1.empty() && sk2.empty() && potrf.empty() && chain.empty(); }
 };
 
 static GemmOp make_op(double* C, int64_t c_si, int64_t c_sj, const double* A, int64_t a_si, int64_t a_sk,
@@ -564,6 +604,7 @@
   bool timeline = false;
   std::vector<cudaEvent_t> tl_events;
   std::vector<cudaEvent_t> tl_launch;
+  std::vector<cudaEvent_t> tl_launch_start;
   int tl_count = 0;
   double prof_ms[16] = {};
   double prof_flops[16] = {};
@@ -587,6 +628,7 @@
   CUDA_OK(cudaFuncSetAttribute(gemm_tiles_kernel<128, 128, 2, 4, BIG_STAGES>, cudaFuncAttributeMaxDynamicSharedMemorySize, BIG_SMEM));
   CUDA_OK(cudaFuncSetAttribute(gemm_tiles_kernel<64, 64, 2, 2, SMALL_STAGES>, cudaFuncAttributeMaxDynamicSharedMemorySize, SMALL_SMEM));
   CUDA_OK(cudaFuncSetAttribute(potrf_inv_kernel_v4, cudaFuncAttributeMaxDynamicSharedMemorySize, POTRF4_SMEM));
+  CUDA_OK(cudaFuncSetAttribute(wide_chain_kernel, cudaFuncAttributeMaxDynamicSharedMemorySize, CHAIN_SMEM));
   CUDA_OK(cudaFuncSetAttribute(gemm_tiles_tma_kernel, cudaFuncAttributeMaxDynamicSharedMemorySize, TMA_SMEM));
 #define SKD_ATTR(NMT)                                                                                                         \
   CUDA_OK(cudaFuncSetAttribute(skinny_f2_dmma_kernel<NMT>, cudaFuncAttributeMaxDynamicSharedMemorySize, SkDmma<NMT>::SMEM));   \
@@ -649,6 +691,10 @@
 #undef SKD_CASE
       break;
     }
+    case Launch::CHAIN:
+      wide_chain_kernel<<<L.grid, 256, CHAIN_SMEM, st>>>(sch.d_chain + L.off, L.count, (int)L.tile_off, sch.d_ctr + L.aux_off,
+                                                         sch.d_ctr, h->d_info);
+      break;
     case Launch::INIT_W:
       init_identity_kernel<<<L.count, 256, 0, st>>>(h->d_wblocks, h->W);
       break;
@@ -661,18 +707,20 @@
 
 static void issue_schedule(slmm_chol* h, const Schedule& sch, double* X, double* const* vec_arena,
                            const int64_t* d_vptr, int nrhs, bool two, cudaStream_t one,
-                           std::vector<cudaEvent_t>* per_launch = nullptr) {
+                           std::vector<cudaEvent_t>* per_launch = nullptr, std::vector<cudaEvent_t>* per_launch_start = nullptr) {
   const DevSym ds = h->devsym();
   size_t nk = 0;
+  auto record = [&](std::vector<cudaEvent_t>* v, cudaStream_t st) {
+    if (nk >= v->size()) { cudaEvent_t e; CUDA_OK(cudaEventCreate(&e)); v->push_back(e); }
+    CUDA_OK(cudaEventRecord((*v)[nk], st));
+  };
   for (const Launch& L : sch.launches) {
     cudaStream_t st = two ? (L.stream ? h->s_bulk : h->s_main) : one;
     if (L.kind == Launch::EV_RECORD) { if (two) CUDA_OK(cudaEventRecord(h->events[L.count], st)); continue; }
     if (L.kind == Launch::EV_WAIT) { if (two) CUDA_OK(cudaStreamWaitEvent(st, h->events[L.count], 0)); continue; }
+    if (per_launch_start) record(per_launch_start, st);
     launch_one(h, sch, L, ds, X, vec_arena, d_vptr, nrhs, st);
-    if (per_launch) {
-      if (nk >= per_launch->size()) { cudaEvent_t e; CUDA_OK(cudaEventCreate(&e)); per_launch->push_back(e); }
-      CUDA_OK(cudaEventRecord((*per_launch)[nk], st));
-    }
+    if (per_launch) record(per_launch, st);
     nk++;
   }
 }
@@ -731,7 +779,7 @@
       CUDA_OK(cudaEventRecord(h->tl_events[0], 0));
       CUDA_OK(cudaStreamWaitEvent(h->s_main, h->tl_events[0], 0));
       CUDA_OK(cudaStreamWaitEvent(h->s_bulk, h->tl_events[0], 0));
-      issue_schedule(h, sch, X, vec_arena, d_vptr, nrhs, true, nullptr, &h->tl_launch);
+      issue_schedule(h, sch, X, vec_arena, d_vptr, nrhs, true, nullptr, &h->tl_launch, &h->tl_launch_start);
       CUDA_OK(cudaEventRecord(h->ev_join, h->s_bulk));
       CUDA_OK(cudaStreamWaitEvent(h->s_main, h->ev_join, 0));
       CUDA_OK(cudaEventRecord(h->tl_events[1], h->s_main));
@@ -871,7 +919,7 @@
 }
 
 struct FStep {
-  enum Kind { POTRF, TRSM, UPD, WINV1, WINV2, CPANEL, OUTER, SCHUR } kind;
+  enum Kind { POTRF, TRSM, UPD, CHAIN, WINV1, WINV2, CPANEL, OUTER, SCHUR } kind;
   int a, b;
 };
 
@@ -903,11 +951,7 @@
       } else {
         for (int ob = 0; ob < num_outer(ns); ob++) {
           const int o0 = ob * NBO, o1 = std::min(ns, o0 + NBO), w = o1 - o0;
-          for (int c0 = o0; c0 < o1; c0 += NBI) {
-            const int ib = c0 / NBI;
-            pr.push_back({FStep::POTRF, ib, 0});
-            if (std::min(o1, c0 + NBI) < o1) { pr.push_back({FStep::TRSM, ib, 0}); pr.push_back({FStep::UPD, ib, 0}); }
-          }
+          pr.push_back({FStep::CHAIN, ob, 0});
           for (int m = NBI; m < w; m *= 2) { pr.push_back({FStep::WINV1, ob, m}); pr.push_back({FStep::WINV2, ob, m}); }
           if (ms > o1)
             for (int j = (w + 127) / 128 - 1; j >= 0; j--) pr.push_back({FStep::CPANEL, ob, j});
@@ -925,19 +969,21 @@
         if (st.kind == FStep::CPANEL || st.kind == FStep::SCHUR) needs_below = true;
         const int s = S.level_sn[S.level_ptr[d] + q];
         const int f = S.sn_first[s], ns = S.sn_first[s + 1] - f, ms = S.sn_nrow[s], rs = ms - ns;
-        const bool wide = ns > NBO;
         double* P = h->Lx + S.sn_lptr[s];
         const int64_t ld = panel_ld(ms);
-        if (st.kind == FStep::POTRF || st.kind == FStep::TRSM || st.kind == FStep::UPD) {
+        if (st.kind == FStep::CHAIN) {
+          const OuterBlock wb = outer_block(h, s, st.a);
+          ChainOp c;
+          memset(&c, 0, sizeof(c));
+          c.P = P + wb.o0 + (int64_t)wb.o0 * ld;
+          c.winv = wb.winv;
+          c.ld = (int32_t)ld; c.w = wb.nbo; c.ldw = wb.ldw; c.colbase = f + wb.o0;
+          pb.chain.push_back(c);
+        } else if (st.kind == FStep::POTRF || st.kind == FStep::TRSM || st.kind == FStep::UPD) {
           const int ib = st.a, c0 = ib * NBI, c1 = std::min(ns, c0 + NBI), nb = c1 - c0;
-          const int ob = c0 / NBO, ob0 = ob * NBO, ob_end = std::min(ns, ob0 + NBO);
           double* inv = h->inv + h->invptr[s] + (int64_t)ib * NBI * NBI;
-          int64_t inv_ld = NBI;
-          if (wide) {
-            const OuterBlock wb = outer_block(h, s, ob);
-            if (wb.nbo > NBI) { inv = wb.winv + (c0 - ob0) + (int64_t)(c0 - ob0) * wb.ldw; inv_ld = wb.ldw; }
-          }
-          const int row_end = wide ? ob_end : ms;
+          const int64_t inv_ld = NBI;
+          const int row_end = ms;
           if (st.kind == FStep::POTRF) {
             pb.potrf.push_back({P + c0 + c0 * ld, inv, (int32_t)ld, nb, f + c0, (int32_t)inv_ld});
             sch.flops += (double)nb * nb * nb / 3.0;
@@ -945,7 +991,7 @@
             pb.add(make_op(P + c1 + c0 * ld, 1, ld, P + c1 + c0 * ld, 1, ld, inv, 1, inv_ld, row_end - c1, nb, nb, 0));
           } else {
             pb.add(make_op(P + c1 + c1 * ld, 1, ld, P + c1 + c0 * ld, 1, ld, P + c1 + c0 * ld, 1, ld, row_end - c1,
-                           ob_end - c1, nb, GF_LOWER | GF_ACCUM | GF_NEG));
+                           ns - c1, nb, GF_LOWER | GF_ACCUM | GF_NEG));
           }
         } else if (st.kind == FStep::WINV1 || st.kind == FStep::WINV2) {
           const OuterBlock wb = outer_block(h, s, st.a);
@@ -1226,6 +1272,28 @@
 
 const char* slmm_last_error(void) { return slmm::last_error().c_str(); }
 int slmm_version(void) { return 100; }
+
+int slmm_chain_order_check(int32_t w) {
+  SLMM_TRY
+  if (w < 1 || w > NBO) throw std::invalid_argument("width outside 1..1024");
+  const int nib = chain_nib(w), n = chain_items(w);
+  std::vector<int> ctr(nib * (nib + 1) / 2, 0);
+  for (int t = 0; t < n; t++) {
+    const ChainItem it = chain_item(w, t);
+    const int k = it.k, i = it.i, j = it.j;
+    bool ok = k >= 0 && k < nib && i < nib && j <= i;
+    if (ok && it.kind == ChainItem::POTRF) ok = i == k && j == k && ctr[chain_tile(k, k)] == k;
+    else if (ok && it.kind == ChainItem::TRSM) ok = i > k && j == k && ctr[chain_tile(k, k)] == k + 1 && ctr[chain_tile(i, k)] == k;
+    else if (ok) ok = j > k && ctr[chain_tile(i, k)] == k + 1 && ctr[chain_tile(j, k)] == k + 1 && ctr[chain_tile(i, j)] == k;
+    if (!ok) throw std::runtime_error("chain item " + std::to_string(t) + " of width " + std::to_string(w) + " is out of order");
+    ctr[chain_tile(i, j)] = k + 1;
+  }
+  for (int i = 0; i < nib; i++)
+    for (int j = 0; j <= i; j++)
+      if (ctr[chain_tile(i, j)] != j + 1) throw std::runtime_error("chain of width " + std::to_string(w) + " leaves a tile unfinished");
+  return SLMM_OK;
+  SLMM_CATCH
+}
 int slmm_device_count(int* out) {
   int c = 0;
   cudaError_t e = cudaGetDeviceCount(&c);
@@ -1328,6 +1396,7 @@
   for (cudaEvent_t e : h->events) cudaEventDestroy(e);
   for (cudaEvent_t e : h->tl_events) cudaEventDestroy(e);
   for (cudaEvent_t e : h->tl_launch) cudaEventDestroy(e);
+  for (cudaEvent_t e : h->tl_launch_start) cudaEventDestroy(e);
   if (h->ev_fork) cudaEventDestroy(h->ev_fork);
   if (h->ev_join) cudaEventDestroy(h->ev_join);
   if (h->s_main) cudaStreamDestroy(h->s_main);
@@ -1460,6 +1529,7 @@
   if (!h) throw std::invalid_argument("null handle");
   const int big = 0x7fffffff;
   CUDA_OK(cudaMemcpyAsync(h->d_info, &big, sizeof(int), cudaMemcpyHostToDevice, 0));
+  if (h->fact.ctr_size > 0) CUDA_OK(cudaMemsetAsync(h->fact.d_ctr, 0, h->fact.ctr_size * sizeof(int), 0));
   run_schedule(h, h->fact, nullptr, nullptr, nullptr, 0);
   int info = 0;
   CUDA_OK(cudaMemcpy(&info, h->d_info, sizeof(int), cudaMemcpyDeviceToHost));
@@ -1633,8 +1703,8 @@
   SLMM_CATCH
 }
 
-int slmm_chol_get_launch_timeline(slmm_chol_t* h, int32_t max_n, int32_t* n_out, float* end_ms, int32_t* stream,
-                                  int32_t* kind, int32_t* grid, double* flops) {
+int slmm_chol_get_launch_timeline(slmm_chol_t* h, int32_t max_n, int32_t* n_out, float* start_ms, float* end_ms,
+                                  int32_t* stream, int32_t* kind, int32_t* grid, double* flops) {
   SLMM_TRY
   if (!h || !n_out) throw std::invalid_argument("null argument");
   std::vector<const Launch*> ks;
@@ -1642,6 +1712,7 @@
   const int n = (int)std::min(ks.size(), h->tl_launch.size());
   *n_out = n;
   for (int q = 0; q < n && q < max_n; q++) {
+    if (start_ms) { float v = 0.f; CUDA_OK(cudaEventElapsedTime(&v, h->tl_events[0], h->tl_launch_start[q])); start_ms[q] = v; }
     if (end_ms) { float v = 0.f; CUDA_OK(cudaEventElapsedTime(&v, h->tl_events[0], h->tl_launch[q])); end_ms[q] = v; }
     if (stream) stream[q] = ks[q]->stream;
     if (kind) kind[q] = (int)ks[q]->kind;
diff --git a/scilmm_b200/csrc/dense_tiles.cuh b/scilmm_b200/csrc/dense_tiles.cuh
--- a/scilmm_b200/csrc/dense_tiles.cuh
+++ b/scilmm_b200/csrc/dense_tiles.cuh
@@ -110,8 +110,7 @@
 }
 
 template <int TM, int TN, int NWM, int NWN, int STAGES>
-__global__ void __launch_bounds__(32 * (NWM * NWN + NPW), 1) gemm_tiles_kernel(const GemmOp* __restrict__ ops,
-                                                                                const int32_t* __restrict__ tile_op) {
+__device__ __forceinline__ void gemm_tile(const GemmOp& op, int local, double* smem) {
   constexpr int NCW = NWM * NWN;
   constexpr int KS = 16;
   constexpr int WM = TM / NWM, WN = TN / NWN;
@@ -119,15 +118,11 @@
   constexpr int LDA = TM + 4, LDB = TN + 4;
   constexpr bool REBALANCE = (NCW == 8);
   static_assert(TM % 32 == 0 && TN % 32 == 0 && NCW % 4 == 0, "producer mapping / warpgroup layout");
-  extern __shared__ double smem[];
   double* As = smem;
   double* Bs = smem + STAGES * KS * LDA;
   uint64_t* full_bar = reinterpret_cast<uint64_t*>(Bs + STAGES * KS * LDB);
   uint64_t* empty_bar = full_bar + STAGES;
 
-  const int tile = blockIdx.x;
-  const GemmOp& op = ops[tile_op[tile]];
-  const int local = tile - op.tile_start;
   const int tiles_m = op.tiles_m;
   const int tm0 = (local % tiles_m) * TM, tn0 = (local / tiles_m) * TN;
   const int flags = op.flags;
@@ -252,6 +247,15 @@
   }
 }
 
+template <int TM, int TN, int NWM, int NWN, int STAGES>
+__global__ void __launch_bounds__(32 * (NWM * NWN + NPW), 1) gemm_tiles_kernel(const GemmOp* __restrict__ ops,
+                                                                                const int32_t* __restrict__ tile_op) {
+  extern __shared__ double smem[];
+  const int tile = blockIdx.x;
+  const GemmOp& op = ops[tile_op[tile]];
+  gemm_tile<TM, TN, NWM, NWN, STAGES>(op, tile - op.tile_start, smem);
+}
+
 __global__ void __launch_bounds__(256) splitk_reduce_kernel(const ReduceOp* __restrict__ ops, int nops) {
   int lo = 0, hi = nops - 1;
   const int blk = blockIdx.x;
diff --git a/scilmm_b200/csrc/potrf_block.cuh b/scilmm_b200/csrc/potrf_block.cuh
--- a/scilmm_b200/csrc/potrf_block.cuh
+++ b/scilmm_b200/csrc/potrf_block.cuh
@@ -19,14 +19,13 @@
   for (int k = 0; k < K; k += 4) dmma884(c0, c1, a[g * lda + k + t], b[g * ldb + k + t]);
 }
 
-__global__ void __launch_bounds__(256) potrf_inv_kernel_v4(const PotrfOp* __restrict__ ops, int* __restrict__ info) {
-  extern __shared__ double pb_smem[];
+template <bool NC>
+__device__ __forceinline__ void potrf_inv_block(const PotrfOp op, int* __restrict__ info, double* pb_smem) {
   double (*A)[PLD] = reinterpret_cast<double (*)[PLD]>(pb_smem);
   double (*X)[PLD] = reinterpret_cast<double (*)[PLD]>(pb_smem + NBI * PLD);
   double (*T)[PLD] = reinterpret_cast<double (*)[PLD]>(pb_smem + 2 * NBI * PLD);
   __shared__ int fail;
   PDBG(0)
-  const PotrfOp op = ops[blockIdx.x];
   const int nb = op.nb, tid = threadIdx.x, lane = tid & 31, warp = tid >> 5;
   const int g = lane >> 2, t = lane & 3;
   if (tid == 0) fail = 0;
@@ -36,7 +35,7 @@
     for (int u = 0; u < NBI * NBI / 256; u++) {
       const int q = tid + 256 * u, i = q % NBI, j = q / NBI;
       v[u] = (i == j) ? 1.0 : 0.0;
-      if (i < nb && j < nb) v[u] = (i >= j) ? __ldg(op.blk + i + (int64_t)j * op.ld) : 0.0;
+      if (i < nb && j < nb) v[u] = (i >= j) ? (NC ? __ldg(op.blk + i + (int64_t)j * op.ld) : op.blk[i + (int64_t)j * op.ld]) : 0.0;
     }
 #pragma unroll
     for (int u = 0; u < NBI * NBI / 256; u++) {
@@ -160,4 +159,9 @@
   PDBG(4)
 }
 
+__global__ void __launch_bounds__(256) potrf_inv_kernel_v4(const PotrfOp* __restrict__ ops, int* __restrict__ info) {
+  extern __shared__ double pb_smem[];
+  potrf_inv_block<true>(ops[blockIdx.x], info, pb_smem);
 }
+
+}
diff --git a/scilmm_b200/engine.py b/scilmm_b200/engine.py
--- a/scilmm_b200/engine.py
+++ b/scilmm_b200/engine.py
@@ -528,19 +528,19 @@
 
     def launch_timeline(self):
         n = C.c_int32(0)
-        check(lib().slmm_chol_get_launch_timeline(self._h, 0, C.byref(n), None, None, None, None, None))
-        end, fl = np.zeros(n.value, np.float32), np.zeros(n.value)
+        check(lib().slmm_chol_get_launch_timeline(self._h, 0, C.byref(n), None, None, None, None, None, None))
+        start, end, fl = np.zeros(n.value, np.float32), np.zeros(n.value, np.float32), np.zeros(n.value)
         st, kind, grid = (np.zeros(n.value, np.int32) for _ in range(3))
-        check(lib().slmm_chol_get_launch_timeline(self._h, n.value, C.byref(n), np_ptr(end), np_ptr(st), np_ptr(kind),
-                                                  np_ptr(grid), np_ptr(fl)))
-        return end, st, kind, grid, fl
+        check(lib().slmm_chol_get_launch_timeline(self._h, n.value, C.byref(n), np_ptr(start), np_ptr(end), np_ptr(st),
+                                                  np_ptr(kind), np_ptr(grid), np_ptr(fl)))
+        return start, end, st, kind, grid, fl
 
     def profile(self):
-        ms, fl, n = np.zeros(13), np.zeros(13), np.zeros(13, dtype=np.int64)
-        check(lib().slmm_chol_get_profile_ex(self._h, 13, np_ptr(ms), np_ptr(fl), np_ptr(n)))
+        ms, fl, n = np.zeros(14), np.zeros(14), np.zeros(14, dtype=np.int64)
+        check(lib().slmm_chol_get_profile_ex(self._h, 14, np_ptr(ms), np_ptr(fl), np_ptr(n)))
         names = ["potrf_inv", "gemm_big", "gemm_small", "extend_add", "rhs_pull", "extend_add_big", "init_w",
-                 "splitk_reduce", "_ev_record", "_ev_wait", "skinny_f1", "skinny_f2", "gemm_tma"]
-        return {names[k]: dict(ms=float(ms[k]), flops=float(fl[k]), launches=int(n[k])) for k in range(13)
+                 "splitk_reduce", "_ev_record", "_ev_wait", "skinny_f1", "skinny_f2", "gemm_tma", "chain"]
+        return {names[k]: dict(ms=float(ms[k]), flops=float(fl[k]), launches=int(n[k])) for k in range(14)
                 if not names[k].startswith("_")}
 
     def launch_profile(self):
```

Result: no change. 0.1931, median of 6 (-0.8%).
